# FangjinhuaWang/PatchmatchNet

Hardware: AMD Instinct MI355X
Metric: depth-maps/sec at 1600x1200 N=5 src views (higher is better)
Workload: dtype f32

## Files before the change

### include/pmn_hip.h

```cpp
#ifndef PMN_HIP_H
#define PMN_HIP_H

#include <stdint.h>

#ifdef __cplusplus
extern "C" {
#endif

#define PMN_ABI_VERSION 25
#define PMN_MLP_FLOATS 340
#define PMN_MAX_DEPTH 64
#define PMN_MAX_NEIGHBORS 17
#define PMN_MAX_FUSE_SRC 32
#define PMN_TSDF_MAX_VIEWS 16
#define PMN_TSDF_MARK_SPAN 8
#define PMN_RASTER_MAX_DIM 16384
#define PMN_RASTER_MAX_BOX 64
#define PMN_SPLAT_MAX_RADIUS 32

#define PMN_OK 0
#define PMN_ERR_ARG (-1)
#define PMN_ERR_SHAPE (-2)
#define PMN_ERR_LAUNCH (-3)

int pmn_abi_version(void);

const char *pmn_error_string(int code);

int pmn_nchw_to_nhwc(const float *in, float *out, int B, int C, int h, int w, void *stream);

int pmn_feature_weight(const float *ref_nhwc, const float *eval_offsets, const int *eval_table_host,
                       const float *mlp, int B, int C, int G, int K, int h, int w,
                       float *out_feature_weight, void *stream);

int pmn_init_hypotheses(const float *noise, const float *depth, int depth_shift, const float *depth_min,
                        const float *depth_max, int num_sample, float interval_scale, const float *propa_offsets,
                        const int *propa_table_host, int K, int B, int h, int w, float *depth_sample,
                        float *xnorm, void *stream);

int pmn_warp_correlate(const float *ref_nhwc, const float *src_nhwc, const float *rel_proj,
                       const float *depth_sample, const float *view_weights_in, int vw_shift,
                       const float *similarity_mlp, const float *pixelwise_mlp, int B, int N, int C,
                       int G, int D, int h, int w, int hs, int ws, float *cost_out, float *view_weights_out,
                       int *vw_argmax_out, float *similarity_out, void *stream);

int pmn_warp_correlate_views(const float *ref_nhwc, const void *src_view_table, const float *rel_proj,
                             const float *depth_sample, const float *view_weights_in, int vw_shift,
                             const float *similarity_mlp, const float *pixelwise_mlp, int B, int N, int C,
                             int G, int D, int h, int w, int hs, int ws, float *cost_out, float *view_weights_out,
                             int *vw_argmax_out, float *similarity_out, void *stream);

int pmn_aggregate_regress(const float *cost, const float *depth_sample, const float *xnorm,
                          const float *feature_weight, const float *eval_offsets, const int *eval_table_host,
                          int K, float interval_scale, int is_inverse, int B, int D, int h, int w,
                          float *score_out, float *depth_out, void *stream);

int pmn_confidence(const float *score, int B, int D, int h, int w, int H, int W, float *confidence_out,
                   int *depth_index_out, void *stream);

int pmn_conv2d(const float *in, const float *weights, const float *shift, const float *up, float *out, int N, int H,
               int W, int cin, int cout, int K, int stride, int pad, int dil, int relu, int in_nchw, int out_nchw,
               int up_h, int up_w, void *stream);

int pmn_fpn_tail(const float *x, const float *up, const float *w_in, const float *b_in, const float *w_out, float *out,
                 int N, int H, int W, int cin, int cmid, int cout, void *stream);

int pmn_conv2d_mfma(const float *in, const float *weights, const float *shift, float *out, float *out_b, int N, int H, int W,
                    int cin, int cout, int ca, int K, int stride, int pad, int dil, int relu, int planar, void *stream);


int pmn_conv2d_f16s(const float *in, const void *weights, const float *shift, float *out, int N, int H, int W, int cin, int cout,
                    int k, int stride, int relu, void *stream);

int pmn_conv2d_f16s_pair(const float *in, const void *weights_a, const float *shift_a, const void *weights_b, const float *shift_b,
                         float *out, int N, int H, int W, int channels, int relu, void *stream);

int pmn_offset_heads_f16s(const float *in, const void *weights, const float *shift, float *out_a, float *out_b, int N, int H, int W,
                          int cin, int cout, int ca, int dil, void *stream);

int pmn_fpn_level(const float *x, const float *u, const float *w, const float *b, float *out_a, float *out_b, int N, int H,
                  int W, int cin, int cout, int ca, void *stream);

int pmn_deconv3x3s2(const float *in, const float *weights, const float *shift, float *out, int N, int Hi, int Wi, int cin,
                    int cout, int relu, void *stream);

int pmn_refine_front(const float *img, const float *t2, const float *w0, const float *s0, const float *wd, const float *sd,
                     float *x16, int B, int H, int W, void *stream);
int pmn_refine_tail(const float *x16, const float *w3, const float *s3, const float *wr, const float *dnorm,
                    const float *depth_min, const float *depth_max, float *out, int B, int H, int W, void *stream);

int pmn_refine_fused(const float *img, const float *t2, const float *w0, const float *s0, const float *wd, const float *sd,
                     const void *w3a, const float *s3, const float *wr, const float *dnorm, const float *depth_min,
                     const float *depth_max, float *out, int B, int H, int W, void *stream);

int pmn_stage_projections(const float *intrinsics, const float *extrinsics, int B, int V, int nstages, float scale0,
                          float *rel, void *stream);

int pmn_stem(const float *img, const float *w0, const float *s0, const float *w1, const float *s1, float *out, int N, int H,
             int W, void *stream);

int pmn_stem_f16s(const float *img, const float *w0, const float *s0, const void *w1a, const float *s1, float *out, int N, int H,
                  int W, void *stream);

int pmn_stem_f16s_views(const float *const *img_table, int views, const float *w0, const float *s0, const void *w1a,
                        const float *s1, float *out, int B, int H, int W, void *stream);

int pmn_differentiable_warping(const float *src_nchw, const float *rel_proj, const float *depth, int B, int C,
                               int D, int h, int w, int hs, int ws, float *warped, void *stream);

int pmn_fuse_view(const float *maps, long long slot_stride, int ref_slot, const int *src_slots_host,
                  const int *src_hw_host, int n_src, const float *mats, int H, int W, float geo_pixel_thres, float geo_depth_thres, int geo_mask_thres,
                  float photo_thres, unsigned char *masks, float *xyz, double *depth_avg, int *geo_sum, void *stream);

int pmn_pack_points(const unsigned char *final_mask, const float *xyz, const void *image_hwc, int image_is_float, int H, int W,
                    unsigned char *records, long long capacity_points, long long *cursor, int *view_count, long long *scratch,
                    void *stream);

int pmn_pack_points_normals(const unsigned char *final_mask, const float *xyz, const float *normals_chw, const float *rotation,
                            int rotation_stride, const void *image_hwc, int image_is_float, int H, int W, unsigned char *records,
                            long long capacity_points, long long *cursor, int *view_count, long long *scratch, void *stream);

int pmn_depth_normals(const float *depth, int H, int W, const float *intrinsics_host, int radius, float rel_thres,
                      float *normals_out, void *stream);

int pmn_normalize_depth(const float *depth, const float *depth_min, const float *depth_max, int B, int n, float *out,
                        void *stream);

int pmn_check_f16_domain(const float *x, long long n, int *flag, void *stream);

int pmn_plan_create(void **plan_out);
int pmn_plan_begin(void *plan);
int pmn_plan_end(void *plan);
int pmn_plan_count(const void *plan);
const char *pmn_plan_kernel_name(const void *plan, int index);
int pmn_plan_launch(const void *plan, void *stream);
int pmn_plan_destroy(void *plan);

int pmn_view_scores(const double *cam_centers, const double *xyz, const long long *obs_ptr, const int *obs_pt,
                    const long long *trk_ptr, const int *trk_img, int N, int P, long long n_obs, long long n_trk,
                    double theta0, double sigma1, double sigma2, double *score, void *stream);

#define PMN_METRICS_MAX_STAGES 4
#define PMN_METRICS_MAX_ITERS 5
#define PMN_METRICS_MAX_THRESHOLDS 8
#define PMN_METRICS_COUNT 0
#define PMN_METRICS_ABS 4
#define PMN_METRICS_THR 8
#define PMN_METRICS_SL1 16
#define PMN_METRICS_ROW 36
#define PMN_METRICS_PIXELS_PER_BLOCK 4096
#define PMN_METRICS_MAX_BLOCKS 128
#define PMN_METRICS_BLOCKS(H, W)                                                                                                     \
    ((int)((((long long)(H) * (W) + PMN_METRICS_PIXELS_PER_BLOCK - 1) / PMN_METRICS_PIXELS_PER_BLOCK) > PMN_METRICS_MAX_BLOCKS        \
               ? PMN_METRICS_MAX_BLOCKS                                                                                               \
               : (((long long)(H) * (W) + PMN_METRICS_PIXELS_PER_BLOCK - 1) / PMN_METRICS_PIXELS_PER_BLOCK)))
#define PMN_METRICS_SCRATCH(B, H, W) ((long long)(B) * PMN_METRICS_BLOCKS(H, W) * PMN_METRICS_ROW)
int pmn_depth_metrics(const float *depth_gt, const float *depth_min, const float *const *maps_host, const int *iters_host,
                      const int *hw_host, int stages, const float *thresholds_host, int n_thresholds, int B, int H, int W,
                      double *scratch, long long scratch_doubles, double *rows, void *stream);

int pmn_nn_distance(const float *to_xyz, const long long *to_keys, long long n_to, const double *origin_host, double cell,
                    const int *dims_host, const float *query, const int *order, long long n_from, double max_dist, double *dist,
                    int *index, void *stream);
int pmn_reduce_round(const float *xyz, const long long *keys, long long n, const double *origin_host, double cell,
                     const int *dims_host, double dst, const int *rank, unsigned char *state, unsigned int *counter, void *stream);

int pmn_tsdf_integrate(float *tsdf, float *weight, float *rgb, float *cweight, const int *dims_host, const float *origin_host,
                       float voxel, float trunc, const float *maps, long long slot_stride, const int *slots_host,
                       const int *hw_host, const void *const *masks_host, const void *const *images_host, const float *cams_host,
                       int n_views, void *stream);
int pmn_mt_count(const float *tsdf, const float *weight, const int *dims_host, float min_weight, unsigned char *vertex_mask,
                 unsigned char *cell_triangles, void *stream);
int pmn_mt_emit(const float *tsdf, const float *weight, const float *rgb, const float *cweight, const int *dims_host,
                const float *origin_host, float voxel, float min_weight, const unsigned char *vertex_mask,
                const unsigned char *cell_triangles, const int *vertex_scan, const int *triangle_scan, float *vertices,
                unsigned char *colors, float *normals, int *faces, void *stream);

int pmn_tsdf_mark_blocks(unsigned char *flags, int *overflow, const int *dims_host, const float *origin_host, float voxel, float trunc,
                         const float *maps, long long slot_stride, const int *slots_host, const int *hw_host,
                         const void *const *masks_host, const float *inv_cams_host, int n_views, void *stream);
int pmn_tsdf_integrate_blocks(float *tsdf, float *weight, float *rgb, float *cweight, const int *blocks, int n_blocks,
                              const int *dims_host, const float *origin_host, float voxel, float trunc, const float *maps,
                              long long slot_stride, const int *slots_host, const int *hw_host, const void *const *masks_host,
                              const void *const *images_host, const float *cams_host, int n_views, void *stream);
int pmn_mt_count_blocks(const float *tsdf, const float *weight, const int *table, const int *blocks, int n_blocks,
                        const int *dims_host, float min_weight, unsigned char *vertex_mask, unsigned char *cell_triangles, void *stream);
int pmn_mt_emit_blocks(const float *tsdf, const float *weight, const float *rgb, const float *cweight, const int *table,
                       const int *blocks, int n_blocks, const int *dims_host, const float *origin_host, float voxel, float min_weight,
                       const unsigned char *vertex_mask, const unsigned char *cell_triangles, const int *vertex_scan,
                       const int *triangle_scan, float *vertices, unsigned char *colors, float *normals, int *faces, void *stream);

int pmn_raster_triangles(const float *vertices, int n_vertices, const int *faces, int n_faces, const float *cam_host, int h, int w,
                         long long max_box, unsigned long long *keys, int *counters, int *worklist, void *stream);
int pmn_splat_points(const float *points, long long n_points, const float *cam_host, int h, int w, float radius_px, float radius_world,
                     unsigned long long *keys, int *counters, void *stream);
int pmn_raster_resolve(const unsigned long long *keys, int h, int w, const float *cam_host, const float *vertices, long long n_vertices,
                       const int *faces, long long n_faces, const unsigned char *colors, const float *normals, int shade, float *depth,
                       int *index, unsigned char *rgb, float *normal, void *stream);

#define PMN_ICP_SUMS 17
#define PMN_ICP_LIMBS 5
#define PMN_ICP_BLOCK_POINTS 256
#define PMN_ICP_BLOCKS(n) (((long long)(n) + PMN_ICP_BLOCK_POINTS - 1) / PMN_ICP_BLOCK_POINTS)
#define PMN_ICP_SCRATCH(n) (PMN_ICP_BLOCKS(n) * PMN_ICP_SUMS * PMN_ICP_LIMBS)
#define PMN_VOXEL_LONG_RUN 256
#define PMN_VOXEL_MAX_CHANNELS 8
#define PMN_CROP_MAX_VERTICES 4096
int pmn_icp_accumulate(const float *to_xyz, const long long *to_keys, long long n_to, const double *origin_host, double cell,
                       const int *dims_host, const float *src, const int *order, long long n, const double *pose_host,
                       const double *centre_host, double max_dist, double *scratch, long long scratch_doubles, double *sums,
                       void *stream);
int pmn_voxel_mean(const float *xyz, const float *attr, int channels, long long n, const long long *starts, long long m, float *out_xyz,
                   float *out_attr, void *stream);
int pmn_crop_prism(const float *xyz, long long n, const double *polygon, int k, int axis, double axis_min, double axis_max,
                   const double *pose_host, unsigned char *mask, void *stream);

int pmn_mesh_components(const int *faces, int n_faces, int n_vertices, int *label, int *invalid, void *stream);
int pmn_mesh_face_samples(const float *vertices, int n_vertices, const int *faces, int n_faces, double density, unsigned long long seed,
                          int *counts, int *invalid, void *stream);
int pmn_mesh_sample(const float *vertices, int n_vertices, const int *faces, int n_faces, const unsigned char *colors,
                    const long long *sample_scan, long long n_samples, unsigned long long seed, float *points, int *face,
                    unsigned char *out_colors, void *stream);

#ifdef __cplusplus
}
#endif
#endif
```

### patchmatchnet_amd/_lib.py

```python
from __future__ import annotations

import ctypes
import os
import subprocess
from typing import Optional

_CSRC = os.path.join(os.path.dirname(os.path.abspath(__file__)), "csrc")
LIB_PATH = os.path.join(_CSRC, "libpmn_hip.so")
ABI_VERSION = 25
MLP_FLOATS = 340
MAX_DEPTH = 64
MAX_NEIGHBORS = 17
MAX_FUSE_SRC = 32
TSDF_MAX_VIEWS = 16
TSDF_MARK_SPAN = 8
RASTER_MAX_DIM = 16384
RASTER_MAX_BOX = 64
SPLAT_MAX_RADIUS = 32
ICP_SUMS = 17
ICP_LIMBS = 5
ICP_BLOCK_POINTS = 256
VOXEL_LONG_RUN = 256
VOXEL_MAX_CHANNELS = 8
CROP_MAX_VERTICES = 4096

_fp = ctypes.c_void_p
_ip = ctypes.c_void_p
_hp = ctypes.c_void_p
_i = ctypes.c_int
_f = ctypes.c_float
_s = ctypes.c_void_p

SIGNATURES = {
    "pmn_abi_version": [],
    "pmn_error_string": [_i],
    "pmn_nchw_to_nhwc": [_fp, _fp, _i, _i, _i, _i, _s],
    "pmn_feature_weight": [_fp, _fp, _hp, _fp, _i, _i, _i, _i, _i, _i, _fp, _s],
    "pmn_init_hypotheses": [_fp, _fp, _i, _fp, _fp, _i, _f, _fp, _hp, _i, _i, _i, _i, _fp, _fp, _s],
    "pmn_warp_correlate": [_fp, _fp, _fp, _fp, _fp, _i, _fp, _fp, _i, _i, _i, _i, _i, _i, _i, _i, _i, _fp, _fp, _ip,
                           _fp, _s],
    "pmn_warp_correlate_views": [_fp, _fp, _fp, _fp, _fp, _i, _fp, _fp, _i, _i, _i, _i, _i, _i, _i, _i, _i, _fp, _fp, _ip,
                                 _fp, _s],
    "pmn_aggregate_regress": [_fp, _fp, _fp, _fp, _fp, _hp, _i, _f, _i, _i, _i, _i, _i, _fp, _fp, _s],
    "pmn_confidence": [_fp, _i, _i, _i, _i, _i, _i, _fp, _ip, _s],
    "pmn_conv2d": [_fp, _fp, _fp, _fp, _fp] + [_i] * 14 + [_s],
    "pmn_fpn_tail": [_fp] * 6 + [_i] * 6 + [_s],
    "pmn_fpn_level": [_fp] * 6 + [_i] * 6 + [_s],
    "pmn_conv2d_f16s": [_fp] * 4 + [_i] * 8 + [_s],
    "pmn_offset_heads_f16s": [_fp] * 5 + [_i] * 7 + [_s],
    "pmn_conv2d_f16s_pair": [_fp] * 6 + [_i] * 5 + [_s],
    "pmn_refine_front": [_fp] * 7 + [_i] * 3 + [_s],
    "pmn_refine_tail": [_fp] * 8 + [_i] * 3 + [_s],
    "pmn_refine_fused": [_fp] * 13 + [_i] * 3 + [_s],
    "pmn_conv2d_mfma": [_fp] * 5 + [_i] * 12 + [_s],
    "pmn_deconv3x3s2": [_fp] * 4 + [_i] * 6 + [_s],
    "pmn_stage_projections": [_fp, _fp, _i, _i, _i, _f, _fp, _s],
    "pmn_stem": [_fp] * 6 + [_i] * 3 + [_s],
    "pmn_stem_f16s": [_fp] * 6 + [_i] * 3 + [_s],
    "pmn_stem_f16s_views": [_fp, _i] + [_fp] * 5 + [_i] * 3 + [_s],
    "pmn_differentiable_warping": [_fp, _fp, _fp, _i, _i, _i, _i, _i, _i, _i, _fp, _s],
    "pmn_fuse_view": [_fp, ctypes.c_longlong, _i, _hp, _hp, _i, _fp, _i, _i, _f, _f, _i, _f, _fp, _fp, _fp, _ip, _s],
    "pmn_pack_points": [_fp, _fp, _fp, _i, _i, _i, _fp, ctypes.c_longlong, _fp, _ip, _fp, _s],
    "pmn_pack_points_normals": [_fp, _fp, _fp, _fp, _i, _fp, _i, _i, _i, _fp, ctypes.c_longlong, _fp, _ip, _fp, _s],
    "pmn_depth_normals": [_fp, _i, _i, _hp, _i, _f, _fp, _s],
    "pmn_normalize_depth": [_fp, _fp, _fp, _i, _i, _fp, _s],
    "pmn_check_f16_domain": [_fp, ctypes.c_longlong, _ip, _s],
    "pmn_plan_create": [ctypes.POINTER(ctypes.c_void_p)],
    "pmn_plan_begin": [_hp],
    "pmn_plan_end": [_hp],
    "pmn_plan_count": [_hp],
    "pmn_plan_kernel_name": [_hp, _i],
    "pmn_plan_launch": [_hp, _s],
    "pmn_plan_destroy": [_hp],
    "pmn_view_scores": [_fp] * 6 + [_i, _i, ctypes.c_longlong, ctypes.c_longlong] + [ctypes.c_double] * 3 + [_fp, _s],
    "pmn_depth_metrics": [_fp, _fp, _hp, _hp, _hp, _i, _hp, _i, _i, _i, _i, _fp, ctypes.c_longlong, _fp, _s],
    "pmn_nn_distance": [_fp, _ip, ctypes.c_longlong, _hp, ctypes.c_double, _hp, _fp, _ip, ctypes.c_longlong, ctypes.c_double, _fp, _ip,
                        _s],
    "pmn_reduce_round": [_fp, _ip, ctypes.c_longlong, _hp, ctypes.c_double, _hp, ctypes.c_double, _ip, _ip, _ip, _s],
    "pmn_tsdf_integrate": [_fp] * 4 + [_hp, _hp, _f, _f, _fp, ctypes.c_longlong] + [_hp] * 5 + [_i, _s],
    "pmn_mt_count": [_fp, _fp, _hp, _f, _ip, _ip, _s],
    "pmn_mt_emit": [_fp] * 4 + [_hp, _hp, _f, _f] + [_ip] * 4 + [_fp, _ip, _fp, _ip, _s],
    "pmn_tsdf_mark_blocks": [_ip, _ip, _hp, _hp, _f, _f, _fp, ctypes.c_longlong] + [_hp] * 4 + [_i, _s],
    "pmn_tsdf_integrate_blocks": [_fp] * 4 + [_ip, _i, _hp, _hp, _f, _f, _fp, ctypes.c_longlong] + [_hp] * 5 + [_i, _s],
    "pmn_mt_count_blocks": [_fp, _fp, _ip, _ip, _i, _hp, _f, _ip, _ip, _s],
    "pmn_mt_emit_blocks": [_fp] * 4 + [_ip, _ip, _i, _hp, _hp, _f, _f] + [_ip] * 4 + [_fp, _ip, _fp, _ip, _s],
    "pmn_raster_triangles": [_fp, _i, _ip, _i, _hp, _i, _i, ctypes.c_longlong, _ip, _ip, _ip, _s],
    "pmn_splat_points": [_fp, ctypes.c_longlong, _hp, _i, _i, _f, _f, _ip, _ip, _s],
    "pmn_raster_resolve": [_ip, _i, _i, _hp, _fp, ctypes.c_longlong, _ip, ctypes.c_longlong, _ip, _fp, _i, _fp, _ip, _ip, _fp, _s],
    "pmn_icp_accumulate": [_fp, _ip, ctypes.c_longlong, _hp, ctypes.c_double, _hp, _fp, _ip, ctypes.c_longlong, _hp, _hp, ctypes.c_double,
                           _fp, ctypes.c_longlong, _fp, _s],
    "pmn_voxel_mean": [_fp, _fp, _i, ctypes.c_longlong, _ip, ctypes.c_longlong, _fp, _fp, _s],
    "pmn_crop_prism": [_fp, ctypes.c_longlong, _fp, _i, _i, ctypes.c_double, ctypes.c_double, _hp, _ip, _s],
    "pmn_mesh_components": [_ip, _i, _i, _ip, _ip, _s],
    "pmn_mesh_face_samples": [_fp, _i, _ip, _i, ctypes.c_double, ctypes.c_ulonglong, _ip, _ip, _s],
    "pmn_mesh_sample": [_fp, _i, _ip, _i, _ip, _ip, ctypes.c_longlong, ctypes.c_ulonglong, _fp, _ip, _ip, _s],
}

METRICS_MAX_STAGES = 4
METRICS_MAX_ITERS = 5
METRICS_MAX_THRESHOLDS = 8
METRICS_COUNT, METRICS_ABS, METRICS_THR, METRICS_SL1 = 0, 4, 8, 16
METRICS_ROW = 36
METRICS_PIXELS_PER_BLOCK = 4096
METRICS_MAX_BLOCKS = 128


def metrics_scratch(B: int, H: int, W: int) -> int:
    return B * min(METRICS_MAX_BLOCKS, -(-H * W // METRICS_PIXELS_PER_BLOCK)) * METRICS_ROW

def icp_scratch(n: int) -> int:
    return -(-n // ICP_BLOCK_POINTS) * ICP_SUMS * ICP_LIMBS


EXPERIMENTAL_SIGNATURES = {"pmn_set_tuning": [_i, _i],
                           "pmn_conv3x3_wino": [_fp] * 4 + [_i] * 5 + [_s],
                           "pmn_conv5x5s2_wino": [_fp] * 4 + [_i] * 6 + [_s]}
EXPERIMENTAL_LIB_PATH = os.path.join(_CSRC, "libpmn_hip_experimental.so")


def experimental() -> bool:
    return os.environ.get("PMN_EXPERIMENTAL", "") == "1"


_LIB: Optional[ctypes.CDLL] = None


class PmnError(RuntimeError):
    pass


def build(force: bool = False, verbose: bool = False) -> str:
    args = ["make", "-C", _CSRC, "-j4"] + (["-B"] if force else []) + (["EXPERIMENTAL=1"] if experimental() else [])
    if not verbose:
        args.insert(1, "-s")
    subprocess.check_call(args)
    return LIB_PATH


def lib() -> ctypes.CDLL:
    global _LIB
    if _LIB is None:
        path, sigs = LIB_PATH, SIGNATURES
        if experimental():
            path, sigs = EXPERIMENTAL_LIB_PATH, {**SIGNATURES, **EXPERIMENTAL_SIGNATURES}
        if not os.path.isfile(path):
            raise PmnError(f"{path} not found: build it with `python -c 'import __graft_entry__ as g; g.build()'` "
                           f"or `make -C patchmatchnet_amd/csrc` -- patchmatchnet_amd has no fallback path")
        L = (ctypes.CDLL if os.environ.get("PMN_CTYPES", "") == "cdll" else ctypes.PyDLL)(path)
        for name, argtypes in sigs.items():
            try:
                fn = getattr(L, name)
            except AttributeError as e:
                raise PmnError(f"libpmn_hip.so does not export {name}") from e
            fn.argtypes = argtypes
            fn.restype = ctypes.c_char_p if name in ("pmn_error_string", "pmn_plan_kernel_name") else ctypes.c_int
        if L.pmn_abi_version() != ABI_VERSION:
            raise PmnError(f"libpmn_hip.so ABI {L.pmn_abi_version()} != expected {ABI_VERSION}: rebuild")
        _LIB = L
    return _LIB


def check(code: int, what: str) -> None:
    if code != 0:
        raise PmnError(f"{what} failed: {lib().pmn_error_string(code).decode()} (code {code})")
```

### patchmatchnet_amd/csrc/plan.hip

```cpp
#include <hip/hip_runtime.h>

#include <cstring>
#include <mutex>
#include <new>
#include <vector>

#include "pmn_common.hpp"

struct PmnPlanEntry {
    const void* func;
    dim3 grid, block;
    size_t lds;
    int nargs;
    size_t first_arg;
};

struct PmnPlan {
    uint32_t magic;
    bool recording, poisoned, sealed;
    int device;
    std::vector<PmnPlanEntry> entries;
    std::vector<size_t> arg_offsets;
    std::vector<unsigned char> blob;
    std::vector<void*> argv;
};

static const uint32_t PMN_PLAN_MAGIC = 0x504d4e50u;

thread_local PmnPlan* pmn_tls_plan = nullptr;

static PmnPlan* as_plan(void* p) {
    PmnPlan* plan = static_cast<PmnPlan*>(p);
    return (plan && plan->magic == PMN_PLAN_MAGIC) ? plan : nullptr;
}

int pmn_plan_append(PmnPlan* plan, const void* func, dim3 grid, dim3 block, size_t lds, int nargs, void* const* args,
                    const size_t* sizes, const size_t* aligns) {
    if (!plan || plan->poisoned) return PMN_ERR_ARG;
    try {
        PmnPlanEntry e{func, grid, block, lds, nargs, plan->arg_offsets.size()};
        for (int i = 0; i < nargs; ++i) {
            const size_t al = aligns[i] ? aligns[i] : 1;
            size_t off = (plan->blob.size() + al - 1) / al * al;
            plan->blob.resize(off + sizes[i]);
            std::memcpy(plan->blob.data() + off, args[i], sizes[i]);
            plan->arg_offsets.push_back(off);
        }
        plan->entries.push_back(e);
    } catch (const std::bad_alloc&) {
        plan->poisoned = true;
        return PMN_ERR_ARG;
    }
    return PMN_OK;
}

extern "C" int pmn_plan_create(void** plan_out) {
    if (!plan_out) return PMN_ERR_ARG;
    PmnPlan* plan = new (std::nothrow) PmnPlan();
    if (!plan) return PMN_ERR_ARG;
    plan->magic = PMN_PLAN_MAGIC;
    plan->recording = plan->poisoned = plan->sealed = false;
    plan->device = -1;
    *plan_out = plan;
    return PMN_OK;
}

extern "C" int pmn_plan_begin(void* p) {
    PmnPlan* plan = as_plan(p);
    if (!plan || plan->sealed || plan->recording || pmn_tls_plan != nullptr) return PMN_ERR_ARG;
    if (hipGetDevice(&plan->device) != hipSuccess) plan->device = -1;
    plan->recording = true;
    pmn_tls_plan = plan;
    return PMN_OK;
}

extern "C" int pmn_plan_end(void* p) {
    PmnPlan* plan = as_plan(p);
    if (!plan || !plan->recording || pmn_tls_plan != plan) return PMN_ERR_ARG;
    pmn_tls_plan = nullptr;
    plan->recording = false;
    if (plan->poisoned) return PMN_ERR_ARG;
    try {
        plan->argv.resize(plan->arg_offsets.size());
    } catch (const std::bad_alloc&) {
        plan->poisoned = true;
        return PMN_ERR_ARG;
    }
    for (size_t i = 0; i < plan->arg_offsets.size(); ++i) plan->argv[i] = plan->blob.data() + plan->arg_offsets[i];
    plan->sealed = true;
    return PMN_OK;
}

extern "C" int pmn_plan_count(const void* p) {
    const PmnPlan* plan = as_plan(const_cast<void*>(p));
    if (!plan) return PMN_ERR_ARG;
    return (int)plan->entries.size();
}

extern "C" const char* pmn_plan_kernel_name(const void* p, int index) {
    const PmnPlan* plan = as_plan(const_cast<void*>(p));
    if (!plan || index < 0 || index >= (int)plan->entries.size()) return nullptr;
    return hipKernelNameRefByPtr(plan->entries[index].func, nullptr);
}

extern "C" int pmn_plan_launch(const void* p, void* stream) {
    const PmnPlan* plan = as_plan(const_cast<void*>(p));
    if (!plan || !plan->sealed) return PMN_ERR_ARG;
    if (pmn_tls_plan != nullptr) return PMN_ERR_ARG;
    hipStream_t st = (hipStream_t)stream;
    void* const* argv = plan->argv.data();
    for (const PmnPlanEntry& e : plan->entries) {
        if (hipLaunchKernel(e.func, e.grid, e.block, const_cast<void**>(argv + e.first_arg), e.lds, st) != hipSuccess) {
            (void)hipGetLastError();
            return PMN_ERR_LAUNCH;
        }
    }
    return PMN_OK;
}

extern "C" int pmn_plan_destroy(void* p) {
    PmnPlan* plan = as_plan(p);
    if (!plan) return PMN_ERR_ARG;
    if (pmn_tls_plan == plan) pmn_tls_plan = nullptr;
    plan->magic = 0;
    delete plan;
    return PMN_OK;
}
```

### patchmatchnet_amd/graph.py

```python
from __future__ import annotations

from typing import Dict, List, Optional, Sequence, Tuple

import torch

from ._lib import PmnError


class GraphedForward:

    def __init__(self, model, max_graphs: int = 8, inputs_in_place: bool = False) -> None:
        self.model, self.max_graphs, self.inputs_in_place = model, max_graphs, inputs_in_place
        self.cache: Dict[Tuple, Tuple] = {}
        self.replays = self.captures = self.evictions = 0

    @staticmethod
    def _alias_pattern(images: Sequence[torch.Tensor]) -> Tuple[int, ...]:
        first: Dict[int, int] = {}
        return tuple(first.setdefault(im.data_ptr(), i) for i, im in enumerate(images))

    @classmethod
    def _signature(cls, images: Sequence[torch.Tensor], intrinsics: torch.Tensor, features) -> Tuple:
        feat = None if features is None else tuple(tuple((s, tuple(t.shape)) for s, t in sorted(f.items())) for f in features)
        return (tuple(tuple(i.shape) for i in images), cls._alias_pattern(images), tuple(intrinsics.shape), feat,
                features is not None and cls._table_ok_cached(features))

    _TABLE_OK: Dict[Tuple, bool] = {}

    @classmethod
    def _table_ok_cached(cls, features) -> bool:
        try:
            key = tuple((s, tuple(t.shape), tuple(t.stride()), t.dtype, t.is_cuda) for f in features for s, t in sorted(f.items()))
        except (AttributeError, TypeError):
            return cls._table_ok(features)
        hit = cls._TABLE_OK.get(key)
        if hit is None:
            if len(cls._TABLE_OK) > 64:
                cls._TABLE_OK.clear()
            hit = cls._TABLE_OK[key] = cls._table_ok(features)
        return hit

    def _images_in_place(self, features) -> bool:
        feature = getattr(self.model, "feature", None)
        if not (self.inputs_in_place and features is None and getattr(self.model, "hip_feature_net", False)
                and feature is not None and feature.f16_split):
            return False
        return "conv1_f16s" in feature._packed()

    def _capture(self, images, intrinsics, extrinsics, depth_min, depth_max, features):
        dev = intrinsics.device
        pattern = self._alias_pattern(images)
        in_place = self._images_in_place(features)
        bufs = [torch.empty_like(im) if pattern[i] == i and not (in_place and i) else None for i, im in enumerate(images)]
        static = dict(images=[bufs[pattern[i]] for i in range(len(images))], intrinsics=torch.empty_like(intrinsics),
                      extrinsics=torch.empty_like(extrinsics), depth_min=torch.empty_like(depth_min),
                      depth_max=torch.empty_like(depth_max),
                      noise=torch.empty((images[0].shape[0], 48, images[0].shape[2] // 8, images[0].shape[3] // 8),
                                        dtype=torch.float32, device=dev),
                      features=None, features_nhwc=None)
        if in_place:
            from . import ops
            static["images"] = [bufs[0]] * len(images)
            static["image_bufs"] = bufs
            static["table_all"] = torch.zeros(len(images), dtype=torch.int64, device=dev)
            static["image_table"] = ops.SourceTable(static["table_all"], (len(images),) + tuple(images[0].shape))
            static["table_host"] = []
        if features is not None and self._table_ok(features):
            from . import ops
            B = images[0].shape[0]
            stages = sorted(features[0])
            ref = {s: torch.empty((B,) + tuple(features[0][s].shape[2:]) + (features[0][s].shape[1],), dtype=torch.float32, device=dev)
                   for s in stages}
            static["ref_nhwc"] = ref
            n_src = len(features) - 1
            static["table_all"] = torch.zeros(len(stages) * n_src, dtype=torch.int64, device=dev)
            static["tables"] = {s: ops.SourceTable(static["table_all"][i * n_src:(i + 1) * n_src],
                                                   (n_src, B) + tuple(features[1][s].shape[2:]) + (features[1][s].shape[1],))
                                for i, s in enumerate(stages)}
            static["features"] = [{s: ref[s].permute(0, 3, 1, 2) for s in stages} for _ in range(len(features))]
            static["table_host"] = []
        elif features is not None:
            B = images[0].shape[0]
            stages = sorted(features[0])
            nhwc = {s: torch.empty((len(features) * B,) + tuple(features[0][s].shape[2:]) + (features[0][s].shape[1],),
                                   dtype=torch.float32, device=dev) for s in stages}
            static["features_nhwc"] = nhwc
            static["features"] = [{s: nhwc[s][v * B:(v + 1) * B].permute(0, 3, 1, 2) for s in stages} for v in range(len(features))]
        self._fill(static, images, intrinsics, extrinsics, depth_min, depth_max, features)

        def run():
            return self.model(list(static["images"]), static["intrinsics"], static["extrinsics"], static["depth_min"],
                              static["depth_max"], features=static["features"], features_nhwc=static["features_nhwc"],
                              noise=static["noise"], source_tables=static.get("tables"), ref_nhwc_maps=static.get("ref_nhwc"),
                              image_table=static.get("image_table"))

        rng = torch.cuda.get_rng_state(dev)
        self._draw(static)
        try:
            handle, out = self._record(run, dev)
        finally:
            torch.cuda.set_rng_state(rng, dev)
        return handle, static, out

    def _record(self, run, dev):
        side = torch.cuda.Stream(dev)
        side.wait_stream(torch.cuda.current_stream(dev))
        with torch.cuda.stream(side):
            run()
        torch.cuda.current_stream(dev).wait_stream(side)
        graph = torch.cuda.CUDAGraph()
        with torch.cuda.graph(graph, capture_error_mode="thread_local"):
            depth, confidence, _ = run()
        return graph, (depth, confidence)

    def _replay(self, handle, dev) -> None:
        handle.replay()

    @staticmethod
    def _table_ok(features) -> bool:
        try:
            for s in features[0]:
                shapes = {tuple(f[s].shape) for f in features}
                if len(shapes) != 1:
                    return False
                for f in features:
                    t = f[s]
                    if not (t.is_cuda and t.dtype == torch.float32 and t.permute(0, 2, 3, 1).is_contiguous()):
                        return False
            return len(features) >= 2
        except (AttributeError, KeyError, TypeError):
            return False

    @staticmethod
    def _draw(static) -> None:
        torch.rand(size=tuple(static["noise"].shape), out=static["noise"])

    @staticmethod
    def _stage_addresses(static, addrs) -> None:
        ring = static["table_host"]
        k = static["turn"] = (static.get("turn", -1) + 1) % 8
        if k >= len(ring):
            host = torch.empty(static["table_all"].numel(), dtype=torch.int64).pin_memory()
            ring.append([host, host.numpy(), None])
        host, host_np, ev = ring[k]
        if ev is not None:
            ev.synchronize()
        host_np[:] = addrs
        static["table_all"].copy_(host, non_blocking=True)
        ev = torch.cuda.Event()
        ev.record(torch.cuda.current_stream(static["intrinsics"].device))
        ring[k][2] = ev

    @classmethod
    def _fill(cls, static, images, intrinsics, extrinsics, depth_min, depth_max, features) -> None:
        if "image_table" in static:
            from . import ops
            bufs, addrs, held = static["image_bufs"], [], []
            for i, im in enumerate(images):
                if i == 0 or im.device != static["intrinsics"].device or not ops.SourceTable.image_in_place(im):
                    if bufs[i] is None:
                        bufs[i] = torch.empty(tuple(images[0].shape), dtype=torch.float32, device=static["intrinsics"].device)
                    if bufs[i].data_ptr() != im.data_ptr():
                        bufs[i].copy_(im, non_blocking=True)
                    addrs.append(bufs[i].data_ptr())
                else:
                    im.record_stream(torch.cuda.current_stream(im.device))
                    held.append(im)
                    addrs.append(im.data_ptr())
            static["held_images"] = held
            cls._stage_addresses(static, addrs)
        else:
            done = set()
            for dst, src in zip(static["images"], images):
                if dst.data_ptr() not in done and dst.data_ptr() != src.data_ptr():
                    dst.copy_(src, non_blocking=True)
                done.add(dst.data_ptr())
        static["intrinsics"].copy_(intrinsics, non_blocking=True)
        static["extrinsics"].copy_(extrinsics, non_blocking=True)
        static["depth_min"].copy_(depth_min, non_blocking=True)
        static["depth_max"].copy_(depth_max, non_blocking=True)
        if features is not None and "tables" in static:
            for s, t in features[0].items():
                static["features"][0][s].copy_(t, non_blocking=True)
            cls._stage_addresses(static, [features[1 + v][s].data_ptr() for s in sorted(static["tables"]) for v in range(len(features) - 1)])
        elif features is not None:
            for dst, src in zip(static["features"], features):
                for s, t in src.items():
                    dst[s].copy_(t, non_blocking=True)

    def __call__(self, images: List[torch.Tensor], intrinsics: torch.Tensor, extrinsics: torch.Tensor,
                 depth_min: torch.Tensor, depth_max: torch.Tensor, features: Optional[List[Dict[int, torch.Tensor]]] = None):
        if not intrinsics.is_cuda:
            raise PmnError("GraphedForward replays HIP graphs: the inputs must be on a ROCm device")
        h, w = images[0].shape[-2:]
        if h % 8 or w % 8 or any(tuple(i.shape) != tuple(images[0].shape) for i in images):
            depth, confidence, _ = self.model(images, intrinsics, extrinsics, depth_min, depth_max, features=features)
            return depth, confidence
        key = self._signature(images, intrinsics, features)
        entry = self.cache.pop(key, None)
        if entry is None:
            if len(self.cache) >= self.max_graphs:
                self.cache.pop(next(iter(self.cache)))
                self.evictions += 1
            entry = self._capture(images, intrinsics, extrinsics, depth_min, depth_max, features)
            self.captures += 1
        self.cache[key] = entry
        graph, static, out = entry
        self._fill(static, images, intrinsics, extrinsics, depth_min, depth_max, features)
        self._draw(static)
        self._replay(graph, intrinsics.device)
        self.replays += 1
        return out


class _LibraryLaunchesOnly(torch.utils._python_dispatch.TorchDispatchMode):

    _ALLOC = ("aten.empty.", "aten.empty_strided.", "aten.empty_like.", "aten.new_empty.", "aten.new_empty_strided.", "aten.detach.",
              "aten.alias.", "aten.lift_fresh.", "aten._unsafe_view.", "aten.reshape.", "aten.view.", "aten.sym_size.",
              "aten.sym_stride.", "aten.sym_numel.", "aten.sym_storage_offset.", "aten.is_contiguous.", "aten.size.", "aten.stride.",
              "aten.numel.", "aten.dim.", "aten.is_pinned.", "prim.device.", "prim.dtype.", "prim.layout.", "aten.record_stream.")

    def __torch_dispatch__(self, func, types, args=(), kwargs=None):
        if not (getattr(func, "is_view", False) or (str(func) + ".").startswith(self._ALLOC)):
            raise PmnError(f"PlannedForward: the forward dispatched {func} while it was being recorded -- an operator outside "
                           "libpmn_hip.so cannot be part of a launch plan (it would run once, on uninitialised data, and never "
                           "again); this input signature has to run eagerly or through a path that only calls the library")
        return func(*args, **(kwargs or {}))


class PlannedForward(GraphedForward):

    def __init__(self, model, max_graphs: int = 8, inputs_in_place: bool = False) -> None:
        super().__init__(model, max_graphs=max_graphs, inputs_in_place=inputs_in_place)

    def _record(self, run, dev):
        import ctypes
        from . import _lib
        L = _lib.lib()
        run()
        with torch.cuda.device(dev):
            pool = torch.cuda.MemPool()
            plan = ctypes.c_void_p()
            _lib.check(L.pmn_plan_create(ctypes.byref(plan)), "pmn_plan_create")
            handle = _Plan(plan, pool)
            with torch.cuda.use_mem_pool(pool, device=dev):
                _lib.check(L.pmn_plan_begin(plan), "pmn_plan_begin")
                try:
                    with _LibraryLaunchesOnly():
                        depth, confidence, _ = run()
                finally:
                    rc = L.pmn_plan_end(plan)
                _lib.check(rc, "pmn_plan_end")
        handle.count = L.pmn_plan_count(plan)
        if handle.count <= 0:
            raise PmnError("PlannedForward: the recording pass recorded no launch")
        return handle, (depth, confidence)

    def _replay(self, handle, dev) -> None:
        from . import _lib
        with torch.cuda.device(dev):
            _lib.check(_lib.lib().pmn_plan_launch(handle.plan, torch.cuda.current_stream(dev).cuda_stream), "pmn_plan_launch")


class PlannedValidationForward(PlannedForward):

    def __init__(self, model, thresholds: Sequence[float], max_graphs: int = 8) -> None:
        super().__init__(model, max_graphs=max_graphs)
        self.thresholds = tuple(float(t) for t in thresholds)
        self._truth: Dict[Tuple, Tuple[torch.Tensor, torch.Tensor]] = {}
        self._current: Optional[Tuple[torch.Tensor, torch.Tensor]] = None

    def __call__(self, images: List[torch.Tensor], intrinsics: torch.Tensor, extrinsics: torch.Tensor,
                 depth_min: torch.Tensor, depth_max: torch.Tensor, depth_gt: torch.Tensor):
        h, w = images[0].shape[-2:]
        if h % 8 or w % 8:
            raise PmnError(f"PlannedValidationForward: {h}x{w} images -- the stage maps are down-samplings of the ground truth only "
                           "when height and width are multiples of 8")
        key = (tuple(depth_gt.shape), depth_gt.device)
        bufs = self._truth.get(key)
        if bufs is None:
            bufs = self._truth[key] = (torch.empty(tuple(depth_gt.shape), dtype=torch.float32, device=depth_gt.device),
                                       torch.empty(tuple(depth_min.shape), dtype=torch.float32, device=depth_gt.device))
        bufs[0].copy_(depth_gt, non_blocking=True)
        bufs[1].copy_(depth_min, non_blocking=True)
        self._current = bufs
        return super().__call__(images, intrinsics, extrinsics, depth_min, depth_max)

    def _record(self, run, dev):
        from . import ops
        depth_gt, depth_min = self._current
        held = {}

        def run_scored():
            depth, confidence, maps = run()
            held["rows"] = ops.depth_metrics(depth_gt, depth_min, maps, self.thresholds)
            return depth, confidence, maps

        handle, (depth, confidence) = super()._record(run_scored, dev)
        return handle, (depth, confidence, held["rows"])


class _Plan:

    def __init__(self, plan, pool) -> None:
        self.plan, self.pool, self.count = plan, pool, 0

    def kernel_names(self) -> List[str]:
        from . import _lib
        L = _lib.lib()
        return [(L.pmn_plan_kernel_name(self.plan, i) or b"?").decode() for i in range(self.count)]

    def __del__(self):
        try:
            from . import _lib
            if self.plan:
                _lib.lib().pmn_plan_destroy(self.plan)
                self.plan = None
        except Exception:
            pass
```

### patchmatchnet_amd/net.py

```python
from __future__ import annotations

from typing import Dict, List, Optional, Tuple

import warnings

import numpy as np
import torch
import torch.nn as nn
import torch.nn.functional as F

from . import _lib, ops, params
from ._lib import PmnError
from .module import ConvBnReLU
from .patchmatch import PatchMatch


class FeatureNet(nn.Module):

    def __init__(self) -> None:
        super().__init__()
        spec = [(3, 8, 3, 1, 1), (8, 8, 3, 1, 1), (8, 16, 5, 2, 2), (16, 16, 3, 1, 1), (16, 16, 3, 1, 1),
                (16, 32, 5, 2, 2), (32, 32, 3, 1, 1), (32, 32, 3, 1, 1), (32, 64, 5, 2, 2), (64, 64, 3, 1, 1),
                (64, 64, 3, 1, 1)]
        for i, (cin, cout, k, s, p) in enumerate(spec):
            setattr(self, f"conv{i}", ConvBnReLU(cin, cout, k, s, p))
        self.output1 = nn.Conv2d(64, 64, 1, bias=False)
        self.inner1 = nn.Conv2d(32, 64, 1, bias=True)
        self.inner2 = nn.Conv2d(16, 64, 1, bias=True)
        self.output2 = nn.Conv2d(64, 32, 1, bias=False)
        self.output3 = nn.Conv2d(64, 16, 1, bias=False)
        self.f16_split = True
        self.f16_domain_error: Optional[str] = None
        self.fold_fpn = True
        self.fuse_conv34 = True
        self.fpn8_valu = False
        self.layer_hook = None

    _SPEC = [(3, 1, 1), (3, 1, 1), (5, 2, 2), (3, 1, 1), (3, 1, 1), (5, 2, 2), (3, 1, 1), (3, 1, 1), (5, 2, 2), (3, 1, 1),
             (3, 1, 1)]

    def _packed(self):
        srcs = [p for p in self.parameters()] + [b for b in self.buffers() if b.dtype.is_floating_point]
        key = params.versions(srcs)
        if getattr(self, "_pack_key", None) != key:
            dev = self.output1.weight.device
            pk = {}
            f16_ok, self.f16_domain_error = True, None
            for i in range(11):
                m = getattr(self, f"conv{i}")
                w, s = params.pack_conv(m.conv.weight, bn=(m.bn.weight, m.bn.bias, m.bn.running_mean, m.bn.running_var),
                                        eps=m.bn.eps)
                pk[f"conv{i}"] = (torch.from_numpy(w).to(dev), torch.from_numpy(s).to(dev))
                cv = m.conv
                if (cv.kernel_size[0], cv.stride[0], cv.in_channels, cv.out_channels) in ops.F16S_SHAPES and f16_ok:
                    try:
                        w, s = params.pack_conv_f16s(cv.weight, bn=(m.bn.weight, m.bn.bias, m.bn.running_mean, m.bn.running_var),
                                                     eps=m.bn.eps)
                        pk[f"conv{i}_f16s"] = (torch.from_numpy(w).to(dev), torch.from_numpy(s).to(dev))
                    except params.F16DomainError as e:
                        f16_ok, self.f16_domain_error = False, f"conv{i}: {e}"
            m1 = self.conv1
            try:
                w, s = params.pack_stem_conv1_f16s(m1.conv.weight, bn=(m1.bn.weight, m1.bn.bias, m1.bn.running_mean, m1.bn.running_var),
                                                  eps=m1.bn.eps)
                pk["conv1_f16s"] = (torch.from_numpy(w).to(dev), torch.from_numpy(s).to(dev))
            except params.F16DomainError as e:
                f16_ok, self.f16_domain_error = False, f"conv1: {e}"
            if not f16_ok:
                for k in [k for k in pk if k.endswith("_f16s")]:
                    del pk[k]
                warnings.warn("FeatureNet: " + self.f16_domain_error + " -- using the fp32 kernels (pmn_stem / pmn_conv2d) instead of "
                              "the fp16-split matrix-core kernels", RuntimeWarning, stacklevel=2)
            for name in ("output1", "inner1", "inner2", "output2", "output3"):
                m = getattr(self, name)
                w, s = params.pack_conv(m.weight, bias=m.bias)
                pk[name] = (torch.from_numpy(w).to(dev), torch.from_numpy(s).to(dev))
            fold = params.fold_fpn(self.output1.weight, self.inner1.weight, self.inner1.bias, self.inner2.weight,
                                   self.inner2.bias, self.output2.weight, self.output3.weight)
            for lvl, (w, b) in fold.items():
                pk[f"fpn{lvl}"] = (torch.from_numpy(w).to(dev), torch.from_numpy(b).to(dev))
            w8 = torch.from_numpy(np.ascontiguousarray(fold[8][0].T))[:, :, None, None]
            w, s = params.pack_conv_mfma(w8, bias=torch.from_numpy(fold[8][1]))
            pk["fpn8_mfma"] = (torch.from_numpy(w).to(dev), torch.from_numpy(s).to(dev))
            self._pack, self._pack_key = pk, key
        return self._pack

    def forward_hip(self, x, image_table: Optional["ops.SourceTable"] = None) -> Dict[int, torch.Tensor]:
        pk = self._packed()
        imgs = list(x) if isinstance(x, (list, tuple)) else [x]
        B, _, H, W = imgs[0].shape
        in_place = image_table is not None
        if in_place and not (self.f16_split and "conv1_f16s" in pk):
            raise PmnError("image_table: only the fp16-split stem (FeatureNet.f16_split, weights inside its domain) reads images in place")
        if in_place:
            t = ops.stem_f16s_views(image_table, *pk["conv0"], *pk["conv1_f16s"])
        else:
            t = torch.empty((B * len(imgs), H, W, 8), dtype=torch.float32, device=imgs[0].device)
        for i, im in enumerate(() if in_place else imgs):
            if self.f16_split and "conv1_f16s" in pk:
                ops.stem_f16s(im.contiguous(), *pk["conv0"], *pk["conv1_f16s"], out=t[i * B:(i + 1) * B])
            else:
                ops.stem(im.contiguous(), *pk["conv0"], *pk["conv1"], out=t[i * B:(i + 1) * B])
        feats = {}
        for i, (k, s, p) in enumerate(self._SPEC):
            if i < 2:
                continue
            if i == 4 and self.f16_split and self.fuse_conv34 and "conv3_f16s" in pk and "conv4_f16s" in pk:
                continue
            if i == 3 and self.f16_split and self.fuse_conv34 and "conv3_f16s" in pk and "conv4_f16s" in pk:
                t = ops.conv2d_f16s_pair(t, *pk["conv3_f16s"], *pk["conv4_f16s"], relu=True)
                feats[4] = t
            elif self.f16_split and f"conv{i}_f16s" in pk:
                t = ops.conv2d_f16s(t, *pk[f"conv{i}_f16s"], k, s, relu=True)
            elif self.layer_hook is not None and (hooked := self.layer_hook(i, t)) is not None:
                t = hooked
            else:
                w, sh = pk[f"conv{i}"]
                t = ops.conv2d(t, w, sh, getattr(self, f"conv{i}").conv.out_channels, k, s, p, relu=True)
            if i in (4, 7, 10):
                feats[i] = t
        half, quarter, eighth = feats[4], feats[7], feats[10]
        if self.fold_fpn:
            if self.fpn8_valu:
                f3, u8 = ops.fpn_level(eighth, None, *pk["fpn8"], ca=64)
            else:
                f3, u8 = ops.pointwise_split_mfma(eighth, *pk["fpn8_mfma"], cout=112, ca=64)
            f2, u4 = ops.fpn_level(quarter, u8, *pk["fpn4"], ca=32)
            f1, _ = ops.fpn_level(half, u4, *pk["fpn2"], ca=16)
            return {3: f3, 2: f2, 1: f1}
        out = {3: ops.conv2d(eighth, *pk["output1"], 64, 1)}
        top = ops.conv2d(quarter, *pk["inner1"], 64, 1, up=eighth)
        out[2] = ops.conv2d(top, *pk["output2"], 32, 1)
        out[1] = ops.fpn_tail(half, top, pk["inner2"][0], pk["inner2"][1], pk["output3"][0])
        return out

    def forward(self, x: torch.Tensor) -> Dict[int, torch.Tensor]:
        half = self.conv4(self.conv3(self.conv2(self.conv1(self.conv0(x)))))
        quarter = self.conv7(self.conv6(self.conv5(half)))
        eighth = self.conv10(self.conv9(self.conv8(quarter)))
        out: Dict[int, torch.Tensor] = {3: self.output1(eighth)}
        top = F.interpolate(eighth, scale_factor=2.0, mode="bilinear", align_corners=False) + self.inner1(quarter)
        out[2] = self.output2(top)
        top = F.interpolate(top, scale_factor=2.0, mode="bilinear", align_corners=False) + self.inner2(half)
        out[1] = self.output3(top)
        return out


class Refinement(nn.Module):

    def __init__(self) -> None:
        super().__init__()
        self.conv0 = ConvBnReLU(in_channels=3, out_channels=8)
        self.conv1 = ConvBnReLU(in_channels=1, out_channels=8)
        self.conv2 = ConvBnReLU(in_channels=8, out_channels=8)
        self.deconv = nn.ConvTranspose2d(8, 8, kernel_size=3, padding=1, output_padding=1, stride=2, bias=False)
        self.bn = nn.BatchNorm2d(8)
        self.conv3 = ConvBnReLU(in_channels=16, out_channels=8)
        self.res = nn.Conv2d(8, 1, kernel_size=3, padding=1, bias=False)
        self.f16_split = True
        self.f16_domain_error: Optional[str] = None
        self.research = dict(layers=False)

    def _packed(self):
        srcs = [p for p in self.parameters()] + [b for b in self.buffers() if b.dtype.is_floating_point]
        key = params.versions(srcs)
        if getattr(self, "_pack_key", None) != key:
            dev = self.res.weight.device

            def bn_of(m):
                return (m.weight, m.bias, m.running_mean, m.running_var)

            pk = {}
            for name in ("conv0", "conv1", "conv2", "conv3"):
                m = getattr(self, name)
                w, s = params.pack_conv(m.conv.weight, bn=bn_of(m.bn), eps=m.bn.eps)
                pk[name] = (torch.from_numpy(w).to(dev), torch.from_numpy(s).to(dev))
            w, s = params.pack_deconv(self.deconv.weight, bn=bn_of(self.bn), eps=self.bn.eps)
            pk["deconv"] = (torch.from_numpy(w).to(dev), torch.from_numpy(s).to(dev))
            w, s = params.pack_conv(self.res.weight)
            pk["res"] = (torch.from_numpy(w).to(dev), torch.from_numpy(s).to(dev))
            pk["tail"] = tuple(torch.from_numpy(a).to(dev) for a in params.pack_refine_tail(
                self.conv3.conv.weight, bn_of(self.conv3.bn), self.res.weight, eps=self.conv3.bn.eps))
            self.f16_domain_error = None
            try:
                w, s = params.pack_refine_conv3_f16s(self.conv3.conv.weight, bn_of(self.conv3.bn), eps=self.conv3.bn.eps)
                pk["conv3_f16s"] = (torch.from_numpy(w).to(dev), torch.from_numpy(s).to(dev))
            except params.F16DomainError as e:
                self.f16_domain_error = f"conv3: {e}"
                warnings.warn("Refinement: " + self.f16_domain_error + " -- using the fp32 kernels (pmn_refine_front / pmn_refine_tail)",
                              RuntimeWarning, stacklevel=2)
            self._pack, self._pack_key = pk, key
        return self._pack

    def forward_hip(self, img: torch.Tensor, depth_0: torch.Tensor, depth_min: torch.Tensor, depth_max: torch.Tensor
                    ) -> torch.Tensor:
        pk = self._packed()
        b = depth_min.size()[0]
        if not self.research["layers"]:
            d = ops.normalize_depth(depth_0, depth_min, depth_max)
        else:
            lo = depth_min.view(b, 1, 1, 1)
            span = (depth_max - depth_min).view(b, 1, 1, 1)
            d = ((depth_0 - lo) / span).contiguous()
        t = ops.conv2d(d, *pk["conv1"], 8, 3, 1, 1, relu=True, in_nchw=True)
        t = ops.conv2d(t, *pk["conv2"], 8, 3, 1, 1, relu=True)
        if not self.research["layers"]:
            if self.f16_split and "conv3_f16s" in pk:
                return ops.refine_fused(img.contiguous(), t, *pk["conv0"], *pk["deconv"], *pk["conv3_f16s"], pk["tail"][2], d,
                                        depth_min.float().contiguous(), depth_max.float().contiguous())
            x16 = ops.refine_front(img.contiguous(), t, *pk["conv0"], *pk["deconv"])
            return ops.refine_tail(x16, *pk["tail"], d, depth_min.float().contiguous(), depth_max.float().contiguous())
        img_feat = ops.conv2d(img.contiguous(), *pk["conv0"], 8, 3, 1, 1, relu=True, in_nchw=True)
        up = ops.deconv3x3s2(t, *pk["deconv"], relu=True)
        t = ops.conv2d(torch.cat((up, img_feat), dim=3), *pk["conv3"], 8, 3, 1, 1, relu=True)
        res = ops.conv2d(t, *pk["res"], 1, 3, 1, 1, out_nchw=True)
        d = F.interpolate(d, scale_factor=2.0, mode="nearest") + res
        return d * span + lo

    def forward(self, img: torch.Tensor, depth_0: torch.Tensor, depth_min: torch.Tensor, depth_max: torch.Tensor
                ) -> torch.Tensor:
        b = depth_min.size()[0]
        lo = depth_min.view(b, 1, 1, 1)
        span = (depth_max - depth_min).view(b, 1, 1, 1)
        d = (depth_0 - lo) / span
        img_feat = self.conv0(img)
        up = F.relu(self.bn(self.deconv(self.conv2(self.conv1(d)))), inplace=True)
        res = self.res(self.conv3(torch.cat((up, img_feat), dim=1)))
        d = F.interpolate(d, scale_factor=2.0, mode="nearest") + res
        return d * span + lo


class PatchmatchNet(nn.Module):

    def __init__(self, patchmatch_interval_scale: List[float], propagation_range: List[int],
                 patchmatch_iteration: List[int], patchmatch_num_sample: List[int], propagate_neighbors: List[int],
                 evaluate_neighbors: List[int]) -> None:
        super().__init__()
        self.stages = 4
        self.feature = FeatureNet()
        self.patchmatch_num_sample = patchmatch_num_sample
        num_features = [16, 32, 64]
        self.propagate_neighbors = propagate_neighbors
        self.evaluate_neighbors = evaluate_neighbors
        self.G = [4, 8, 8]
        for i in range(self.stages - 1):
            setattr(self, f"patchmatch_{i + 1}", PatchMatch(
                propagation_out_range=propagation_range[i], patchmatch_iteration=patchmatch_iteration[i],
                patchmatch_num_sample=patchmatch_num_sample[i], patchmatch_interval_scale=patchmatch_interval_scale[i],
                num_feature=num_features[i], G=self.G[i], propagate_neighbors=self.propagate_neighbors[i],
                evaluate_neighbors=evaluate_neighbors[i], stage=i + 1))
        self.upsample_net = Refinement()
        self.batch_feature_extraction = True
        self.hip_feature_net = True
        self.hip_projections = True

    def load_state_dict(self, state_dict, strict: bool = True, **kw):
        if any(k.startswith("module.") for k in state_dict):
            state_dict = {(k[len("module."):] if k.startswith("module.") else k): v for k, v in state_dict.items()}
        return super().load_state_dict(state_dict, strict=strict, **kw)

    @staticmethod
    def scripted_module_config(archive) -> Dict[str, list]:
        stages = [getattr(archive, f"patchmatch_{i}") for i in (1, 2, 3)]
        return dict(patchmatch_interval_scale=[float(s.patchmatch_interval_scale) for s in stages],
                    propagation_range=[int(s.dilation) for s in stages],
                    patchmatch_iteration=[int(s.patchmatch_iteration) for s in stages],
                    patchmatch_num_sample=[int(x) for x in archive.patchmatch_num_sample],
                    propagate_neighbors=[int(s.propagate_neighbors) for s in stages],
                    evaluate_neighbors=[int(s.evaluate_neighbors) for s in stages])

    @classmethod
    def from_scripted_module(cls, path: str) -> "PatchmatchNet":
        archive = torch.jit.load(path, map_location="cpu")
        model = cls(**cls.scripted_module_config(archive))
        model.load_state_dict({k: v.detach().clone() for k, v in archive.state_dict().items()}, strict=True)
        return model

    def extract_features(self, images: List[torch.Tensor], stacked: Optional[dict] = None,
                         image_table: Optional["ops.SourceTable"] = None) -> List[Dict[int, torch.Tensor]]:
        same = all(im.shape == images[0].shape for im in images)
        B = images[0].shape[0]
        if image_table is not None and not (self.hip_feature_net and same and images[0].is_cuda and self.feature.f16_split):
            raise PmnError("image_table needs the HIP FeatureNet (f16_split) and same-size images on a ROCm device")
        if self.hip_feature_net and same and images[0].is_cuda:
            f = self.feature.forward_hip(images, image_table=image_table)
            if stacked is not None:
                stacked.update({("nhwc", s): t for s, t in f.items()})
            return [{s: t[i * B:(i + 1) * B].permute(0, 3, 1, 2) for s, t in f.items()} for i in range(len(images))]
        if self.hip_feature_net and images[0].is_cuda:
            outs = [self.feature.forward_hip(im) for im in images]
            return [{s: t.permute(0, 3, 1, 2) for s, t in f.items()} for f in outs]
        if self.batch_feature_extraction and same and len(images) > 1:
            f = self.feature(torch.cat(images, dim=0))
            if stacked is not None:
                stacked.update(f)
            return [{s: t[i * B:(i + 1) * B] for s, t in f.items()} for i in range(len(images))]
        return [self.feature(im) for im in images]

    def forward(self, images: List[torch.Tensor], intrinsics: torch.Tensor, extrinsics: torch.Tensor,
                depth_min: torch.Tensor, depth_max: torch.Tensor, noise: Optional[torch.Tensor] = None,
                features: Optional[List[Dict[int, torch.Tensor]]] = None, debug: Optional[dict] = None,
                features_nhwc: Optional[Dict[int, torch.Tensor]] = None, source_tables: Optional[Dict[int, "ops.SourceTable"]] = None,
                ref_nhwc_maps: Optional[Dict[int, torch.Tensor]] = None, image_table: Optional["ops.SourceTable"] = None
                ) -> Tuple[torch.Tensor, torch.Tensor, Dict[int, List[torch.Tensor]]]:
        assert len(images) == intrinsics.size()[1], "Different number of images and intrinsic matrices"
        assert len(images) == extrinsics.size()[1], "Different number of images and extrinsic matrices"
        if self.training:
            raise PmnError("patchmatchnet_amd.PatchmatchNet is inference-only: call .eval() (the HIP kernels have no "
                           "backward pass)")
        images, intrinsics, orig_height, orig_width = adjust_image_dims(images, intrinsics)
        ref_image = images[0]
        _, _, ref_height, ref_width = ref_image.size()

        stacked: Dict[int, torch.Tensor] = {}
        if features is None:
            features = self.extract_features(images, stacked, image_table)
        elif features_nhwc is not None:
            stacked.update({("nhwc", st): t for st, t in features_nhwc.items()})
        ref_feature, src_features = features[0], features[1:]
        batch = ref_image.shape[0]

        depth_min = depth_min.float()
        depth_max = depth_max.float()
        device = intrinsics.device
        depth = torch.empty(0, device=device)
        score = torch.empty(0, device=device)
        view_weights = torch.empty(0, device=device)
        depth_patchmatch: Dict[int, List[torch.Tensor]] = {}

        scale = 0.125
        depth_shift, vw_shift = 0, 0
        rel_all = ops.stage_projections(intrinsics, extrinsics, self.stages - 1, scale) if self.hip_projections else None
        for stage in range(self.stages - 1, 0, -1):
            if rel_all is None:
                intrinsics_l = intrinsics.clone()
                intrinsics_l[:, :, :2] *= scale
                proj = extrinsics.clone()
                proj[:, :, :3, :4] = torch.matmul(intrinsics_l, extrinsics[:, :, :3, :4])
                proj_l = torch.unbind(proj, 1)
                ref_proj, src_proj = proj_l[0], proj_l[1:]
            else:
                ref_proj, src_proj = extrinsics[:, 0], [extrinsics[:, i] for i in range(1, extrinsics.shape[1])]
            scale *= 2.0

            dbg = [] if debug is not None else None
            pm: PatchMatch = getattr(self, f"patchmatch_{stage}")
            ref_nhwc = src_nhwc = None
            if ("nhwc", stage) in stacked:
                allv = stacked[("nhwc", stage)]
            elif stage in stacked:
                allv = ops.nchw_to_nhwc(stacked[stage].contiguous())
            else:
                allv = None
            if source_tables is not None:
                ref_nhwc, src_nhwc = ref_nhwc_maps[stage], source_tables[stage]
            elif allv is not None:
                ref_nhwc = allv[:batch]
                src_nhwc = allv[batch:].view(len(src_features), batch, *allv.shape[1:])
            depths, score, view_weights = pm(
                ref_feature=ref_feature[stage], src_features=[f[stage] for f in src_features], ref_proj=ref_proj,
                src_projs=list(src_proj), depth_min=depth_min, depth_max=depth_max, depth=depth,
                view_weights=view_weights, depth_shift=depth_shift, vw_shift=vw_shift,
                noise=noise if stage == self.stages - 1 else None, debug=dbg, ref_nhwc=ref_nhwc, src_nhwc=src_nhwc,
                rel_proj=None if rel_all is None else rel_all[self.stages - 1 - stage])
            if debug is not None:
                debug[stage] = dbg
            depth_patchmatch[stage] = depths
            depth = depths[-1].detach()
            if stage > 1:
                depth_shift = 1
                vw_shift = vw_shift + 1 if view_weights.shape[-1] != depths[-1].shape[-1] else 1

        if self.hip_feature_net and ref_image.is_cuda:
            depth = self.upsample_net.forward_hip(ref_image, depth, depth_min, depth_max)
        else:
            depth = self.upsample_net(ref_image, depth, depth_min, depth_max)
        if ref_width != orig_width or ref_height != orig_height:
            depth = F.interpolate(depth, size=[orig_height, orig_width], mode="bilinear", align_corners=False)
        depth_patchmatch[0] = [depth]

        confidence, _ = ops.confidence(score.contiguous(), orig_height, orig_width)
        return depth, confidence, depth_patchmatch


def adjust_image_dims(images: List[torch.Tensor], intrinsics: torch.Tensor
                      ) -> Tuple[List[torch.Tensor], torch.Tensor, int, int]:
    _, _, ref_height, ref_width = images[0].size()
    for i in range(len(images)):
        _, _, height, width = images[i].size()
        new_height = int(round(height / 8)) * 8
        new_width = int(round(width / 8)) * 8
        if new_width != width or new_height != height:
            intrinsics[:, i, 0] *= new_width / width
            intrinsics[:, i, 1] *= new_height / height
            images[i] = F.interpolate(images[i], size=[new_height, new_width], mode="bilinear", align_corners=False)
    return images, intrinsics, ref_height, ref_width
```

### patchmatchnet_amd/ops.py

```python
from __future__ import annotations

import ctypes
from typing import List, Optional, Sequence, Tuple

import numpy as np
import torch

from . import _lib
from ._lib import PmnError, check


_TIMING = None
_TIMING_ON = True


def enable_kernel_timing() -> None:
    global _TIMING, _TIMING_ON
    _TIMING, _TIMING_ON = [], True


def pause_kernel_timing(paused: bool) -> None:
    global _TIMING_ON
    _TIMING_ON = not paused


def disable_kernel_timing():
    global _TIMING
    rec, _TIMING = _TIMING, None
    if not rec:
        return []
    torch.cuda.synchronize()
    return [(s.elapsed_time(e), nbytes, tag) for s, e, nbytes, tag in rec]


TUNE_WINDOW_BYTES, TUNE_FLAGS, TUNE_WINDOW_BYTES_PIXELWISE, TUNE_ABLATE = 0, 1, 2, 3
TUNE_LANE_WINDOW_BYTES, TUNE_LANE_ABLATE, TUNE_LANE_WAVES_PER_SIMD = 4, 5, 6
TUNE_TILE_WINDOW_BYTES = 10
FLAG_WINDOWED, FLAG_NO_ROTATION, FLAG_STREAM_PIXELWISE, FLAG_STREAM_VIEWS, FLAG_WIN_V1, FLAG_TILE, FLAG_MFMA = 1, 2, 4, 8, 16, 32, 64
DEFAULT_FLAGS = 0


def set_tuning(key: int, value: int) -> None:
    if not _lib.experimental():
        raise PmnError("pmn_set_tuning exists only in libpmn_hip_experimental.so: build with `make -C patchmatchnet_amd/csrc "
                       "EXPERIMENTAL=1` and run with PMN_EXPERIMENTAL=1")
    check(_lib.lib().pmn_set_tuning(int(key), int(value)), "pmn_set_tuning")


import os as _os

F16_DOMAIN_CHECK = _os.environ.get("PMN_CHECK_F16_DOMAIN", "") == "1"
_F16_FLAGS = {}


def _f16_domain_probe(*tensors: Optional[torch.Tensor]) -> None:
    if not F16_DOMAIN_CHECK:
        return
    for t in tensors:
        if t is None or not t.is_cuda or t.numel() == 0:
            continue
        flag = _F16_FLAGS.get(t.device)
        if flag is None:
            flag = _F16_FLAGS[t.device] = torch.zeros(1, dtype=torch.int32, device=t.device)
        with torch.cuda.device(t.device):
            check(_lib.lib().pmn_check_f16_domain(t.data_ptr(), t.numel(), flag.data_ptr(), _stream(t)), "pmn_check_f16_domain")


def f16_domain_check(reset: bool = True) -> None:
    bad = [str(d) for d, f in _F16_FLAGS.items() if int(f.item()) != 0]
    if reset:
        for f in _F16_FLAGS.values():
            f.zero_()
    if bad:
        raise PmnError("an activation outside the fp16-split kernels' domain (|x| >= 65504 or not finite) reached pmn_*_f16s on " +
                       ", ".join(bad) + ": the outputs contain inf / NaN where an fp32 convolution is finite -- set f16_split = False on "
                       "FeatureNet / Refinement / PatchMatch for this checkpoint or input range (include/pmn_hip.h)")


def _dev(t: torch.Tensor, name: str) -> torch.Tensor:
    if not isinstance(t, torch.Tensor):
        raise PmnError(f"{name}: expected a torch.Tensor")
    if not t.is_cuda:
        raise PmnError(f"{name}: tensor is on {t.device}; patchmatchnet_amd runs only on a ROCm GPU (no CPU fallback)")
    if t.dtype != torch.float32:
        raise PmnError(f"{name}: expected float32, got {t.dtype}")
    if not t.is_contiguous():
        raise PmnError(f"{name}: tensor must be contiguous")
    return t


def _dlast(t: torch.Tensor, name: str) -> torch.Tensor:
    if not isinstance(t, torch.Tensor) or not t.is_cuda or t.dtype != torch.float32:
        raise PmnError(f"{name}: expected a float32 tensor on a ROCm GPU (no CPU fallback)")
    if t.permute(0, 2, 3, 1).is_contiguous():
        return t
    return t.permute(0, 2, 3, 1).contiguous().permute(0, 3, 1, 2)


def _dev_as(t: torch.Tensor, name: str, dtype: torch.dtype) -> torch.Tensor:
    if not isinstance(t, torch.Tensor) or not t.is_cuda:
        raise PmnError(f"{name}: expected a tensor on a ROCm GPU (no CPU fallback)")
    if t.dtype != dtype or not t.is_contiguous():
        raise PmnError(f"{name}: expected a contiguous {dtype} tensor")
    return t


def _ptr(t: Optional[torch.Tensor]) -> Optional[int]:
    return None if t is None else t.data_ptr()


def _stream(t: torch.Tensor) -> int:
    return torch.cuda.current_stream(t.device).cuda_stream


def _host_f32(a: np.ndarray, n: int, name: str):
    a = np.ascontiguousarray(a, np.float32)
    if a.size != n:
        raise PmnError(f"{name}: expected {n} floats, got {a.size}")
    return a, a.ctypes.data_as(ctypes.c_void_p)


def _host_i32(a: np.ndarray, n: int, name: str):
    a = np.ascontiguousarray(a, np.int32)
    if a.size != n:
        raise PmnError(f"{name}: expected {n} ints, got {a.size}")
    return a, a.ctypes.data_as(ctypes.c_void_p)


def nchw_to_nhwc(x: torch.Tensor, out: Optional[torch.Tensor] = None) -> torch.Tensor:
    if out is None and isinstance(x, torch.Tensor) and x.is_cuda and x.dtype == torch.float32 and not x.is_contiguous():
        v = x.permute(0, 2, 3, 1)
        if v.is_contiguous():
            return v
        x = x.contiguous()
    _dev(x, "x")
    B, C, h, w = x.shape
    if out is None:
        out = torch.empty((B, h, w, C), dtype=torch.float32, device=x.device)
    else:
        _dev(out, "out")
        if tuple(out.shape) != (B, h, w, C):
            raise PmnError("nchw_to_nhwc: bad output shape")
    with torch.cuda.device(x.device):
        check(_lib.lib().pmn_nchw_to_nhwc(x.data_ptr(), out.data_ptr(), B, C, h, w, _stream(x)), "pmn_nchw_to_nhwc")
    return out


def stack_sources_nhwc(src_features: Sequence[torch.Tensor]) -> torch.Tensor:
    buf, sizes = stack_sources_padded(src_features)
    if any(sz != sizes[0] for sz in sizes):
        raise PmnError("all source feature maps of one stage must share a shape (stack_sources_padded handles mixed sizes)")
    return buf


def stack_sources_padded(src_features: Sequence[torch.Tensor]):
    if len(src_features) == 0:
        raise PmnError("at least one source view is required")
    B, C = src_features[0].shape[:2]
    sizes = [(int(f.shape[2]), int(f.shape[3])) for f in src_features]
    if any(tuple(f.shape[:2]) != (B, C) for f in src_features):
        raise PmnError("source feature maps of one stage must share batch size and channels")
    hs, ws = max(h for h, _ in sizes), max(w for _, w in sizes)
    mixed = any(sz != (hs, ws) for sz in sizes)
    alloc = torch.zeros if mixed else torch.empty
    buf = alloc((len(src_features), B, hs, ws, C), dtype=torch.float32, device=src_features[0].device)
    for i, f in enumerate(src_features):
        v = f.permute(0, 2, 3, 1)
        if sizes[i] != (hs, ws):
            _dev(f.contiguous(), "src_feature")
            buf[i][:, :sizes[i][0], :sizes[i][1], :].copy_(v)
        elif f.is_cuda and f.dtype == torch.float32 and v.is_contiguous():
            buf[i].copy_(v)
        else:
            nchw_to_nhwc(f.contiguous(), buf[i])
    return buf, sizes


def rescale_projection_rows(rel_proj: torch.Tensor, sizes, padded_hw) -> torch.Tensor:
    HS, WS = padded_hw
    if all(sz == (HS, WS) for sz in sizes):
        return rel_proj
    out = rel_proj.clone()
    for v, (h_v, w_v) in enumerate(sizes):
        if (h_v, w_v) != (HS, WS):
            out[:, v, 0, :] *= (w_v - 1) / (WS - 1)
            out[:, v, 1, :] *= (h_v - 1) / (HS - 1)
    return out.contiguous()


def _mlp_dev(t: torch.Tensor, name: str) -> torch.Tensor:
    _dev(t, name)
    if t.numel() != _lib.MLP_FLOATS:
        raise PmnError(f"{name}: expected a packed MLP block of {_lib.MLP_FLOATS} floats")
    return t


def feature_weight(ref_nhwc: torch.Tensor, eval_offsets: torch.Tensor, table: np.ndarray, mlp: torch.Tensor,
                   G: int) -> torch.Tensor:
    _dev(ref_nhwc, "ref_nhwc")
    _dev(eval_offsets, "eval_offsets")
    B, h, w, C = ref_nhwc.shape
    K = eval_offsets.shape[1] // 2
    if tuple(eval_offsets.shape) != (B, 2 * K, h, w):
        raise PmnError("feature_weight: eval_offsets must be [B,2K,h,w]")
    tab, tab_p = _host_i32(table, 2 * K, "table")
    _mlp_dev(mlp, "mlp")
    out = torch.empty((B, K, h, w), dtype=torch.float32, device=ref_nhwc.device)
    with torch.cuda.device(ref_nhwc.device):
        check(_lib.lib().pmn_feature_weight(ref_nhwc.data_ptr(), eval_offsets.data_ptr(), tab_p, mlp.data_ptr(), B, C, G,
                                            K, h, w,
                                            out.data_ptr(), _stream(out)), "pmn_feature_weight")
    return out


def init_hypotheses(noise: Optional[torch.Tensor], depth: Optional[torch.Tensor], depth_shift: int,
                    depth_min: torch.Tensor, depth_max: torch.Tensor, num_sample: int, interval_scale: float,
                    propa_offsets: Optional[torch.Tensor], table: Optional[np.ndarray], h: int, w: int
                    ) -> Tuple[torch.Tensor, torch.Tensor]:
    _dev(depth_min, "depth_min")
    _dev(depth_max, "depth_max")
    B = depth_min.shape[0]
    dev = depth_min.device
    if noise is not None:
        _dev(noise, "noise")
        if tuple(noise.shape) != (B, 48, h, w):
            raise PmnError("init_hypotheses: noise must be [B,48,h,w]")
        D0 = 48
    else:
        if depth is None:
            raise PmnError("init_hypotheses: need noise or depth")
        _dev(depth, "depth")
        if tuple(depth.shape) != (B, 1, h >> depth_shift, w >> depth_shift):
            raise PmnError(f"init_hypotheses: depth must be [B,1,{h >> depth_shift},{w >> depth_shift}], "
                           f"got {tuple(depth.shape)}")
        D0 = num_sample
    K = 0
    tab_p = None
    tab = None
    if propa_offsets is not None:
        _dev(propa_offsets, "propa_offsets")
        K = propa_offsets.shape[1] // 2
        if tuple(propa_offsets.shape) != (B, 2 * K, h, w):
            raise PmnError("init_hypotheses: propa_offsets must be [B,2K,h,w]")
        tab, tab_p = _host_i32(table, 2 * K, "table")
    D = D0 + K
    ds = torch.empty((B, D, h, w), dtype=torch.float32, device=dev)
    xn = torch.empty((B, h, w, D), dtype=torch.float32, device=dev).permute(0, 3, 1, 2)
    with torch.cuda.device(dev):
        check(_lib.lib().pmn_init_hypotheses(_ptr(noise), _ptr(depth) if noise is None else None, depth_shift,
                                             depth_min.data_ptr(), depth_max.data_ptr(), num_sample,
                                             float(interval_scale), _ptr(propa_offsets), tab_p, K, B, h, w,
                                             ds.data_ptr(), xn.data_ptr(), _stream(ds)), "pmn_init_hypotheses")
    del tab
    return ds, xn


class SourceTable:

    def __init__(self, table: torch.Tensor, shape) -> None:
        if table.dtype != torch.int64 or not table.is_cuda or table.numel() != int(shape[0]):
            raise PmnError("SourceTable: int64 device tensor with one address per source view")
        self.table, self.shape, self.device = table, tuple(int(x) for x in shape), table.device

    @staticmethod
    def image_in_place(im: torch.Tensor) -> bool:
        return bool(im.is_cuda and im.dtype == torch.float32 and im.is_contiguous() and im.data_ptr() % 16 == 0)

    @staticmethod
    def addresses(maps) -> list:
        out = []
        for m in maps:
            if not (m.is_cuda and m.dtype == torch.float32 and m.is_contiguous()):
                raise PmnError("SourceTable: dense float32 channels-last device maps")
            out.append(m.data_ptr())
        return out


def warp_correlate(ref_nhwc: torch.Tensor, src_nhwc, rel_proj: torch.Tensor, depth_sample: torch.Tensor,
                   view_weights: Optional[torch.Tensor], vw_shift: int, similarity_mlp: torch.Tensor,
                   pixelwise_mlp: Optional[torch.Tensor], G: int, want_similarity: bool = False,
                   want_argmax: bool = False):
    _dev(ref_nhwc, "ref_nhwc")
    table = src_nhwc if isinstance(src_nhwc, SourceTable) else None
    if table is None:
        _dev(src_nhwc, "src_nhwc")
    _dev(rel_proj, "rel_proj")
    _dev(depth_sample, "depth_sample")
    B, h, w, C = ref_nhwc.shape
    N, Bs, hs, ws, Cs = src_nhwc.shape
    D = depth_sample.shape[1]
    if Bs != B or Cs != C or tuple(depth_sample.shape) != (B, D, h, w) or tuple(rel_proj.shape) != (B, N, 4, 4):
        raise PmnError("warp_correlate: inconsistent shapes")
    dev = ref_nhwc.device
    sim_p = _mlp_dev(similarity_mlp, "similarity_mlp").data_ptr()
    pix_p, vw_out, argmax = None, None, None
    if view_weights is not None:
        _dev(view_weights, "view_weights")
        if tuple(view_weights.shape) != (B, N, h >> vw_shift, w >> vw_shift):
            raise PmnError("Patchmatch Evaluation: Different number of images and view weights")
    else:
        if pixelwise_mlp is None:
            raise PmnError("warp_correlate: pixelwise_mlp required when view_weights is None")
        pix_p = _mlp_dev(pixelwise_mlp, "pixelwise_mlp").data_ptr()
        vw_out = torch.empty((B, N, h, w), dtype=torch.float32, device=dev)
        if want_argmax:
            argmax = torch.empty((B, N, h, w), dtype=torch.int32, device=dev)
    cost = torch.empty((B, h, w, D), dtype=torch.float32, device=dev).permute(0, 3, 1, 2)
    sim = torch.empty((B, G, D, h, w), dtype=torch.float32, device=dev) if want_similarity else None
    with torch.cuda.device(dev):
        if _TIMING is not None and _TIMING_ON:
            ev0, ev1 = torch.cuda.Event(enable_timing=True), torch.cuda.Event(enable_timing=True)
            ev0.record()
        fn = _lib.lib().pmn_warp_correlate if table is None else _lib.lib().pmn_warp_correlate_views
        check(fn(ref_nhwc.data_ptr(), (src_nhwc if table is None else table.table).data_ptr(), rel_proj.data_ptr(),
                 depth_sample.data_ptr(), _ptr(view_weights), vw_shift, sim_p, pix_p, B, N, C,
                 G, D, h, w, hs, ws, cost.data_ptr(), _ptr(vw_out), _ptr(argmax), _ptr(sim),
                 _stream(cost)), "pmn_warp_correlate")
        if _TIMING is not None and _TIMING_ON:
            ev1.record()
            _TIMING.append((ev0, ev1, 4 * B * h * w * ((1 + N) * C + D + N + G * D),
                            f"C{C}_D{D}_{h}x{w}_N{N}_{'vw' if view_weights is not None else 'pixelwise'}"))
    return cost, (view_weights if view_weights is not None else vw_out), argmax, sim


def aggregate_regress(cost: torch.Tensor, depth_sample: torch.Tensor, xnorm: torch.Tensor, feature_weight_: torch.Tensor,
                      eval_offsets: torch.Tensor, table: np.ndarray, interval_scale: float, is_inverse: bool
                      ) -> Tuple[torch.Tensor, torch.Tensor]:
    for n, t in (("depth_sample", depth_sample), ("feature_weight", feature_weight_), ("eval_offsets", eval_offsets)):
        _dev(t, n)
    cost, xnorm = _dlast(cost, "cost"), _dlast(xnorm, "xnorm")
    B, D, h, w = cost.shape
    K = feature_weight_.shape[1]
    if tuple(depth_sample.shape) != (B, D, h, w) or tuple(xnorm.shape) != (B, D, h, w) or \
            tuple(feature_weight_.shape) != (B, K, h, w) or tuple(eval_offsets.shape) != (B, 2 * K, h, w):
        raise PmnError("aggregate_regress: inconsistent shapes")
    tab, tab_p = _host_i32(table, 2 * K, "table")
    score = torch.empty((B, D, h, w), dtype=torch.float32, device=cost.device)
    depth = torch.empty((B, h, w), dtype=torch.float32, device=cost.device)
    with torch.cuda.device(cost.device):
        check(_lib.lib().pmn_aggregate_regress(cost.data_ptr(), depth_sample.data_ptr(), xnorm.data_ptr(),
                                               feature_weight_.data_ptr(), eval_offsets.data_ptr(), tab_p, K,
                                               float(interval_scale), 1 if is_inverse else 0, B, D, h, w,
                                               score.data_ptr(), depth.data_ptr(), _stream(cost)),
              "pmn_aggregate_regress")
    return score, depth


def confidence(score: torch.Tensor, H: int, W: int, want_index: bool = False):
    _dev(score, "score")
    B, D, h, w = score.shape
    conf = torch.empty((B, H, W), dtype=torch.float32, device=score.device)
    idx = torch.empty((B, h, w), dtype=torch.int32, device=score.device) if want_index else None
    with torch.cuda.device(score.device):
        check(_lib.lib().pmn_confidence(score.data_ptr(), B, D, h, w, H, W, conf.data_ptr(), _ptr(idx), _stream(score)),
              "pmn_confidence")
    return conf, idx


def relative_projection(src_projs: Sequence[torch.Tensor], ref_proj: torch.Tensor) -> torch.Tensor:
    inv = torch.inverse(ref_proj)
    return torch.matmul(torch.stack(list(src_projs), dim=1), inv.unsqueeze(1)).contiguous()


def differentiable_warping(src_fea: torch.Tensor, src_proj: torch.Tensor, ref_proj: torch.Tensor,
                           depth_samples: torch.Tensor) -> torch.Tensor:
    src_fea = _dev(src_fea.contiguous(), "src_fea")
    depth_samples = _dev(depth_samples.contiguous(), "depth_samples")
    B, C, hs, ws = src_fea.shape
    _, D, h, w = depth_samples.shape
    proj = torch.matmul(src_proj, torch.inverse(ref_proj)).contiguous()
    _dev(proj, "proj")
    out = torch.empty((B, C, D, h, w), dtype=torch.float32, device=src_fea.device)
    with torch.cuda.device(src_fea.device):
        check(_lib.lib().pmn_differentiable_warping(src_fea.data_ptr(), proj.data_ptr(), depth_samples.data_ptr(), B, C,
                                                    D, h, w, hs, ws, out.data_ptr(), _stream(out)),
              "pmn_differentiable_warping")
    return out


def stage_projections(intrinsics: torch.Tensor, extrinsics: torch.Tensor, nstages: int = 3, scale0: float = 0.125
                      ) -> torch.Tensor:
    intrinsics = _dev(intrinsics.float().contiguous(), "intrinsics")
    extrinsics = _dev(extrinsics.float().contiguous(), "extrinsics")
    B, V = intrinsics.shape[:2]
    rel = torch.empty((nstages, B, V - 1, 4, 4), dtype=torch.float32, device=intrinsics.device)
    with torch.cuda.device(rel.device):
        check(_lib.lib().pmn_stage_projections(intrinsics.data_ptr(), extrinsics.data_ptr(), B, V, nstages, float(scale0),
                                               rel.data_ptr(), _stream(rel)), "pmn_stage_projections")
    return rel


def normalize_depth(depth: torch.Tensor, depth_min: torch.Tensor, depth_max: torch.Tensor) -> torch.Tensor:
    depth = _dev(depth.contiguous(), "depth")
    lo, hi = _dev(depth_min.float().contiguous(), "depth_min"), _dev(depth_max.float().contiguous(), "depth_max")
    B = depth.shape[0]
    if lo.numel() != B or hi.numel() != B:
        raise PmnError("normalize_depth: depth_min / depth_max must hold one value per batch element")
    out = torch.empty_like(depth)
    with torch.cuda.device(depth.device):
        check(_lib.lib().pmn_normalize_depth(depth.data_ptr(), lo.data_ptr(), hi.data_ptr(), B, depth.numel() // B, out.data_ptr(),
                                             _stream(out)), "pmn_normalize_depth")
    return out


def conv2d(x: torch.Tensor, weights: torch.Tensor, shift: torch.Tensor, cout: int, K: int, stride: int = 1, pad: int = 0,
           dil: int = 1, relu: bool = False, up: Optional[torch.Tensor] = None, in_nchw: bool = False,
           out_nchw: bool = False, out: Optional[torch.Tensor] = None) -> torch.Tensor:
    _dev(x, "x")
    _dev(weights, "weights")
    _dev(shift, "shift")
    if in_nchw:
        N, cin, H, W = x.shape
    else:
        N, H, W, cin = x.shape
    if tuple(weights.shape[:3]) != (K, K, cin) or shift.numel() != weights.shape[3]:
        raise PmnError("conv2d: packed weights do not match the input")
    Ho = (H + 2 * pad - dil * (K - 1) - 1) // stride + 1
    Wo = (W + 2 * pad - dil * (K - 1) - 1) // stride + 1
    shape = (N, cout, Ho, Wo) if out_nchw else (N, Ho, Wo, cout)
    if out is None:
        out = torch.empty(shape, dtype=torch.float32, device=x.device)
    else:
        _dev(out, "out")
        if tuple(out.shape) != shape:
            raise PmnError("conv2d: bad `out` shape")
    up_h = up_w = 0
    if up is not None:
        _dev(up, "up")
        if tuple(up.shape) != (N, Ho // 2, Wo // 2, cout) or Ho % 2 or Wo % 2:
            raise PmnError("conv2d: `up` must be [N,Ho/2,Wo/2,cout]")
        up_h, up_w = up.shape[1], up.shape[2]
    with torch.cuda.device(x.device):
        check(_lib.lib().pmn_conv2d(x.data_ptr(), weights.data_ptr(), shift.data_ptr(), _ptr(up), out.data_ptr(), N, H, W,
                                    cin, cout, K, stride, pad, dil, 1 if relu else 0, 1 if in_nchw else 0,
                                    1 if out_nchw else 0, up_h, up_w, _stream(x)), "pmn_conv2d")
    return out


def fpn_tail(x: torch.Tensor, up: torch.Tensor, w_in: torch.Tensor, b_in: torch.Tensor, w_out: torch.Tensor) -> torch.Tensor:
    for n_, t_ in (("x", x), ("up", up), ("w_in", w_in), ("b_in", b_in), ("w_out", w_out)):
        _dev(t_, n_)
    N, H, W, cin = x.shape
    cmid, cout = up.shape[3], w_out.shape[3]
    if tuple(up.shape) != (N, H // 2, W // 2, cmid) or tuple(w_in.shape) != (1, 1, cin, cmid) or \
            tuple(w_out.shape) != (1, 1, cmid, cout):
        raise PmnError("fpn_tail: inconsistent shapes")
    out = torch.empty((N, H, W, cout), dtype=torch.float32, device=x.device)
    with torch.cuda.device(x.device):
        check(_lib.lib().pmn_fpn_tail(x.data_ptr(), up.data_ptr(), w_in.data_ptr(), b_in.data_ptr(), w_out.data_ptr(),
                                      out.data_ptr(), N, H, W, cin, cmid, cout, _stream(x)), "pmn_fpn_tail")
    return out


MFMA_CONV_SHAPES = {(64, 64, 3, 1), (32, 32, 3, 1), (32, 64, 5, 2), (16, 32, 5, 2)}
MFMA_HEAD_SHAPES = {(64, 2), (32, 4), (16, 6)}


def conv2d_mfma(x: torch.Tensor, weights: torch.Tensor, shift: torch.Tensor, K: int, stride: int = 1, pad: int = 0,
                relu: bool = True) -> torch.Tensor:
    for n_, t_ in (("x", x), ("weights", weights), ("shift", shift)):
        _dev(t_, n_)
    N, H, W, cin = x.shape
    cout = shift.shape[0]
    if tuple(weights.shape) != (K * K, cin // 8, cout // 32, 64, 4):
        raise PmnError("conv2d_mfma: weights are not in pack_conv_mfma layout for this input")
    Ho, Wo = (H + 2 * pad - K) // stride + 1, (W + 2 * pad - K) // stride + 1
    out = torch.empty((N, Ho, Wo, cout), dtype=torch.float32, device=x.device)
    with torch.cuda.device(x.device):
        check(_lib.lib().pmn_conv2d_mfma(x.data_ptr(), weights.data_ptr(), shift.data_ptr(), out.data_ptr(), None, N, H, W,
                                         cin, cout, cout, K, stride, pad, 1, 1 if relu else 0, 0, _stream(x)),
              "pmn_conv2d_mfma")
    return out


def conv3x3_wino(x: torch.Tensor, weights: torch.Tensor, shift: torch.Tensor, relu: bool = True) -> torch.Tensor:
    if not _lib.experimental():
        raise PmnError("conv3x3_wino: research build only (make -C patchmatchnet_amd/csrc EXPERIMENTAL=1, PMN_EXPERIMENTAL=1)")
    for n_, t_ in (("x", x), ("weights", weights), ("shift", shift)):
        _dev(t_, n_)
    N, H, W, C = x.shape
    if tuple(weights.shape) != (C // 16, 16, C // 16, 64, 4) or tuple(shift.shape) != (C,):
        raise PmnError("conv3x3_wino: weights are not in pack_conv_wino layout for this input")
    out = torch.empty((N, H, W, C), dtype=torch.float32, device=x.device)
    with torch.cuda.device(x.device):
        check(_lib.lib().pmn_conv3x3_wino(x.data_ptr(), weights.data_ptr(), shift.data_ptr(), out.data_ptr(), N, H, W, C,
                                          1 if relu else 0, _stream(x)), "pmn_conv3x3_wino")
    return out


def conv5x5s2_wino(x: torch.Tensor, weights: torch.Tensor, shift: torch.Tensor, relu: bool = True) -> torch.Tensor:
    if not _lib.experimental():
        raise PmnError("conv5x5s2_wino: research build only (make -C patchmatchnet_amd/csrc EXPERIMENTAL=1, PMN_EXPERIMENTAL=1)")
    for n_, t_ in (("x", x), ("weights", weights), ("shift", shift)):
        _dev(t_, n_)
    N, H, W, cin = x.shape
    cout = shift.shape[0]
    if tuple(weights.shape) != (cin // 8, 49, cout // 16, 64, 2):
        raise PmnError("conv5x5s2_wino: weights are not in pack_conv5x5s2_wino layout for this input")
    out = torch.empty((N, (H - 1) // 2 + 1, (W - 1) // 2 + 1, cout), dtype=torch.float32, device=x.device)
    with torch.cuda.device(x.device):
        check(_lib.lib().pmn_conv5x5s2_wino(x.data_ptr(), weights.data_ptr(), shift.data_ptr(), out.data_ptr(), N, H, W, cin,
                                            cout, 1 if relu else 0, _stream(x)), "pmn_conv5x5s2_wino")
    return out


F16S_SHAPES = {(3, 1, 16, 16), (3, 1, 32, 32), (3, 1, 64, 64), (5, 2, 8, 16), (5, 2, 16, 32), (5, 2, 32, 64)}


def conv2d_f16s(x: torch.Tensor, weights: torch.Tensor, shift: torch.Tensor, k: int, stride: int, relu: bool = True) -> torch.Tensor:
    _dev(x, "x")
    _f16_domain_probe(x)
    _dev(shift, "shift")
    if not isinstance(weights, torch.Tensor) or not weights.is_cuda or weights.dtype != torch.float16 or not weights.is_contiguous():
        raise PmnError("conv2d_f16s: weights must be a contiguous float16 tensor on a ROCm GPU (params.pack_conv_f16s)")
    N, H, W, cin = x.shape
    cout = shift.shape[0]
    if (k, stride, cin, cout) not in F16S_SHAPES:
        raise PmnError(f"conv2d_f16s: unsupported layer (k={k}, stride={stride}, cin={cin}, cout={cout})")
    from . import params as _params
    cc = _params.f16s_chunk(cin, k)
    if tuple(weights.shape) != (cin // cc, (k * k * (cc // 8) + 3) // 4, cout // 16, 2, 64, 8):
        raise PmnError("conv2d_f16s: weights are not in pack_conv_f16s layout for this input")
    out = torch.empty((N, (H - 1) // stride + 1, (W - 1) // stride + 1, cout), dtype=torch.float32, device=x.device)
    with torch.cuda.device(x.device):
        check(_lib.lib().pmn_conv2d_f16s(x.data_ptr(), weights.data_ptr(), shift.data_ptr(), out.data_ptr(), N, H, W, cin, cout, k,
                                         stride, 1 if relu else 0, _stream(x)), "pmn_conv2d_f16s")
    return out


def conv2d_f16s_pair(x: torch.Tensor, weights_a: torch.Tensor, shift_a: torch.Tensor, weights_b: torch.Tensor, shift_b: torch.Tensor,
                     relu: bool = True) -> torch.Tensor:
    _dev(x, "x")
    _f16_domain_probe(x)
    N, H, W, C = x.shape
    for w_, s_ in ((weights_a, shift_a), (weights_b, shift_b)):
        _dev(s_, "shift")
        if not isinstance(w_, torch.Tensor) or not w_.is_cuda or w_.dtype != torch.float16 or not w_.is_contiguous() or \
                tuple(w_.shape) != (1, 5, 1, 2, 64, 8) or s_.numel() != 16:
            raise PmnError("conv2d_f16s_pair: weights must be params.pack_conv_f16s of a (3, 1, 16, 16) layer on a ROCm GPU")
    if C != 16:
        raise PmnError("conv2d_f16s_pair: 16-channel layers only")
    out = torch.empty((N, H, W, 16), dtype=torch.float32, device=x.device)
    with torch.cuda.device(x.device):
        check(_lib.lib().pmn_conv2d_f16s_pair(x.data_ptr(), weights_a.data_ptr(), shift_a.data_ptr(), weights_b.data_ptr(), shift_b.data_ptr(),
                                              out.data_ptr(), N, H, W, 16, 1 if relu else 0, _stream(x)), "pmn_conv2d_f16s_pair")
    return out


def pointwise_split_mfma(x: torch.Tensor, weights: torch.Tensor, shift: torch.Tensor, cout: int, ca: int):
    for n_, t_ in (("x", x), ("weights", weights), ("shift", shift)):
        _dev(t_, n_)
    N, H, W, cin = x.shape
    coutp = shift.shape[0]
    if tuple(weights.shape) != (1, cin // 8, coutp // 32, 64, 4) or not 0 < ca < cout <= coutp:
        raise PmnError("pointwise_split_mfma: weights are not in pack_conv_mfma layout for this input")
    out_a = torch.empty((N, H, W, ca), dtype=torch.float32, device=x.device)
    out_b = torch.empty((N, H, W, cout - ca), dtype=torch.float32, device=x.device)
    with torch.cuda.device(x.device):
        check(_lib.lib().pmn_conv2d_mfma(x.data_ptr(), weights.data_ptr(), shift.data_ptr(), out_a.data_ptr(), out_b.data_ptr(),
                                         N, H, W, cin, cout, ca, 1, 1, 0, 1, 0, 0, _stream(x)), "pmn_conv2d_mfma")
    return out_a, out_b


def offset_heads_mfma(x: torch.Tensor, weights: torch.Tensor, shift: torch.Tensor, cout: int, ca: int, dil: int):
    for n_, t_ in (("x", x), ("weights", weights), ("shift", shift)):
        _dev(t_, n_)
    N, H, W, cin = x.shape
    coutp = shift.shape[0]
    if tuple(weights.shape) != (9, cin // 8, coutp // 32, 64, 4) or not 0 < ca <= cout <= coutp:
        raise PmnError("offset_heads_mfma: weights are not in pack_conv_mfma layout for this input")
    out_a = torch.empty((N, ca, H, W), dtype=torch.float32, device=x.device)
    out_b = torch.empty((N, cout - ca, H, W), dtype=torch.float32, device=x.device) if ca < cout else None
    with torch.cuda.device(x.device):
        check(_lib.lib().pmn_conv2d_mfma(x.data_ptr(), weights.data_ptr(), shift.data_ptr(), out_a.data_ptr(), _ptr(out_b), N,
                                         H, W, cin, cout, ca, 3, 1, dil, dil, 0, 1, _stream(x)), "pmn_conv2d_mfma")
    return out_a, out_b


F16S_HEAD_SHAPES = {(64, 2), (32, 4), (16, 6)}


def offset_heads_f16s(x: torch.Tensor, weights: torch.Tensor, shift: torch.Tensor, cout: int, ca: int, dil: int):
    _dev(x, "x")
    _f16_domain_probe(x)
    _dev(shift, "shift")
    N, H, W, cin = x.shape
    coutp = shift.shape[0]
    if not isinstance(weights, torch.Tensor) or not weights.is_cuda or weights.dtype != torch.float16 or not weights.is_contiguous() \
            or tuple(weights.shape) != (cin // 16, (9 * 2 + 3) // 4, coutp // 16, 2, 64, 8) or not 0 < ca <= cout <= coutp \
            or coutp != (cout + 15) // 16 * 16:
        raise PmnError("offset_heads_f16s: weights are not in pack_offset_heads_f16s layout for this input")
    out_a = torch.empty((N, ca, H, W), dtype=torch.float32, device=x.device)
    out_b = torch.empty((N, cout - ca, H, W), dtype=torch.float32, device=x.device) if ca < cout else None
    with torch.cuda.device(x.device):
        check(_lib.lib().pmn_offset_heads_f16s(x.data_ptr(), weights.data_ptr(), shift.data_ptr(), out_a.data_ptr(), _ptr(out_b), N,
                                               H, W, cin, cout, ca, dil, _stream(x)), "pmn_offset_heads_f16s")
    return out_a, out_b


def fpn_level(x: torch.Tensor, u: Optional[torch.Tensor], w: torch.Tensor, b: torch.Tensor, ca: int):
    for n_, t_ in (("x", x), ("w", w), ("b", b)):
        _dev(t_, n_)
    N, H, W, cin = x.shape
    cout = w.shape[1]
    if tuple(w.shape) != (cin, cout) or tuple(b.shape) != (cout,) or not 0 < ca <= cout:
        raise PmnError("fpn_level: inconsistent shapes")
    if u is not None:
        _dev(u, "u")
        if tuple(u.shape) != (N, H // 2, W // 2, cout) or H % 2 or W % 2:
            raise PmnError("fpn_level: `u` must be [N,H/2,W/2,cout]")
    out_a = torch.empty((N, H, W, ca), dtype=torch.float32, device=x.device)
    out_b = torch.empty((N, H, W, cout - ca), dtype=torch.float32, device=x.device) if ca < cout else None
    with torch.cuda.device(x.device):
        check(_lib.lib().pmn_fpn_level(x.data_ptr(), _ptr(u), w.data_ptr(), b.data_ptr(), out_a.data_ptr(), _ptr(out_b),
                                       N, H, W, cin, cout, ca, _stream(x)), "pmn_fpn_level")
    return out_a, out_b


def refine_front(img: torch.Tensor, t2: torch.Tensor, w0: torch.Tensor, s0: torch.Tensor, wd: torch.Tensor,
                 sd: torch.Tensor) -> torch.Tensor:
    for n_, t_ in (("img", img), ("t2", t2), ("w0", w0), ("s0", s0), ("wd", wd), ("sd", sd)):
        _dev(t_, n_)
    B, c, H, W = img.shape
    if c != 3 or H % 2 or W % 2 or tuple(t2.shape) != (B, H // 2, W // 2, 8) or tuple(w0.shape) != (3, 3, 3, 8) or \
            tuple(wd.shape) != (3, 3, 8, 8):
        raise PmnError("refine_front: inconsistent shapes")
    out = torch.empty((B, H, W, 16), dtype=torch.float32, device=img.device)
    with torch.cuda.device(img.device):
        check(_lib.lib().pmn_refine_front(img.data_ptr(), t2.data_ptr(), w0.data_ptr(), s0.data_ptr(), wd.data_ptr(),
                                          sd.data_ptr(), out.data_ptr(), B, H, W, _stream(img)), "pmn_refine_front")
    return out


def refine_tail(x16: torch.Tensor, w3: torch.Tensor, s3: torch.Tensor, wr: torch.Tensor, dnorm: torch.Tensor,
                depth_min: torch.Tensor, depth_max: torch.Tensor) -> torch.Tensor:
    for n_, t_ in (("x16", x16), ("w3", w3), ("s3", s3), ("wr", wr), ("dnorm", dnorm), ("depth_min", depth_min),
                   ("depth_max", depth_max)):
        _dev(t_, n_)
    B, H, W, c = x16.shape
    if c != 16 or H % 2 or W % 2 or tuple(dnorm.shape) != (B, 1, H // 2, W // 2) or tuple(w3.shape) != (2, 3, 3, 16, 4) or \
            tuple(wr.shape) != (3, 3, 8) or depth_min.numel() != B or depth_max.numel() != B:
        raise PmnError("refine_tail: inconsistent shapes")
    out = torch.empty((B, 1, H, W), dtype=torch.float32, device=x16.device)
    with torch.cuda.device(x16.device):
        check(_lib.lib().pmn_refine_tail(x16.data_ptr(), w3.data_ptr(), s3.data_ptr(), wr.data_ptr(), dnorm.data_ptr(),
                                         depth_min.data_ptr(), depth_max.data_ptr(), out.data_ptr(), B, H, W, _stream(x16)),
              "pmn_refine_tail")
    return out


def refine_fused(img: torch.Tensor, t2: torch.Tensor, w0: torch.Tensor, s0: torch.Tensor, wd: torch.Tensor, sd: torch.Tensor,
                 w3a: torch.Tensor, s3: torch.Tensor, wr: torch.Tensor, dnorm: torch.Tensor, depth_min: torch.Tensor,
                 depth_max: torch.Tensor) -> torch.Tensor:
    for n_, t_ in (("img", img), ("t2", t2), ("w0", w0), ("s0", s0), ("wd", wd), ("sd", sd), ("s3", s3), ("wr", wr), ("dnorm", dnorm),
                   ("depth_min", depth_min), ("depth_max", depth_max)):
        _dev(t_, n_)
    if not isinstance(w3a, torch.Tensor) or not w3a.is_cuda or w3a.dtype != torch.float16 or tuple(w3a.shape) != (5, 2, 64, 8) \
            or not w3a.is_contiguous():
        raise PmnError("refine_fused: w3a must be the float16 [5,2,64,8] tensor of params.pack_refine_conv3_f16s on a ROCm GPU")
    B, c, H, W = img.shape
    if c != 3 or H % 2 or W % 2 or tuple(t2.shape) != (B, H // 2, W // 2, 8) or tuple(dnorm.shape) != (B, 1, H // 2, W // 2) or \
            tuple(w0.shape) != (3, 3, 3, 8) or tuple(wd.shape) != (3, 3, 8, 8) or tuple(wr.shape) != (3, 3, 8) or s3.numel() != 8 or \
            depth_min.numel() != B or depth_max.numel() != B:
        raise PmnError("refine_fused: inconsistent shapes")
    _f16_domain_probe(img, t2)
    out = torch.empty((B, 1, H, W), dtype=torch.float32, device=img.device)
    with torch.cuda.device(img.device):
        check(_lib.lib().pmn_refine_fused(img.data_ptr(), t2.data_ptr(), w0.data_ptr(), s0.data_ptr(), wd.data_ptr(), sd.data_ptr(),
                                          w3a.data_ptr(), s3.data_ptr(), wr.data_ptr(), dnorm.data_ptr(), depth_min.data_ptr(),
                                          depth_max.data_ptr(), out.data_ptr(), B, H, W, _stream(img)), "pmn_refine_fused")
    return out


def deconv3x3s2(x: torch.Tensor, weights: torch.Tensor, shift: torch.Tensor, relu: bool = True) -> torch.Tensor:
    _dev(x, "x")
    _dev(weights, "weights")
    _dev(shift, "shift")
    N, Hi, Wi, cin = x.shape
    cout = weights.shape[3]
    out = torch.empty((N, 2 * Hi, 2 * Wi, cout), dtype=torch.float32, device=x.device)
    with torch.cuda.device(x.device):
        check(_lib.lib().pmn_deconv3x3s2(x.data_ptr(), weights.data_ptr(), shift.data_ptr(), out.data_ptr(), N, Hi, Wi, cin,
                                         cout, 1 if relu else 0, _stream(x)), "pmn_deconv3x3s2")
    return out


def stem(img: torch.Tensor, w0: torch.Tensor, s0: torch.Tensor, w1: torch.Tensor, s1: torch.Tensor,
         out: Optional[torch.Tensor] = None) -> torch.Tensor:
    for n_, t_ in (("img", img), ("w0", w0), ("s0", s0), ("w1", w1), ("s1", s1)):
        _dev(t_, n_)
    N, c, H, W = img.shape
    if c != 3 or tuple(w0.shape) != (3, 3, 3, 8) or tuple(w1.shape) != (3, 3, 8, 8):
        raise PmnError("stem: expects a 3-channel image and 3->8->8 weights")
    if out is None:
        out = torch.empty((N, H, W, 8), dtype=torch.float32, device=img.device)
    else:
        _dev(out, "out")
        if tuple(out.shape) != (N, H, W, 8):
            raise PmnError("stem: bad `out` shape")
    with torch.cuda.device(img.device):
        check(_lib.lib().pmn_stem(img.data_ptr(), w0.data_ptr(), s0.data_ptr(), w1.data_ptr(), s1.data_ptr(), out.data_ptr(),
                                  N, H, W, _stream(img)), "pmn_stem")
    return out


def stem_f16s(img: torch.Tensor, w0: torch.Tensor, s0: torch.Tensor, w1a: torch.Tensor, s1: torch.Tensor,
              out: Optional[torch.Tensor] = None) -> torch.Tensor:
    for n_, t_ in (("img", img), ("w0", w0), ("s0", s0), ("s1", s1)):
        _dev(t_, n_)
    if not isinstance(w1a, torch.Tensor) or not w1a.is_cuda or w1a.dtype != torch.float16 or tuple(w1a.shape) != (3, 2, 64, 8) \
            or not w1a.is_contiguous():
        raise PmnError("stem_f16s: w1a must be the float16 [3,2,64,8] tensor of params.pack_stem_conv1_f16s on a ROCm GPU")
    N, c, H, W = img.shape
    if c != 3 or tuple(w0.shape) != (3, 3, 3, 8):
        raise PmnError("stem_f16s: expects a 3-channel image and 3->8 conv0 weights")
    _f16_domain_probe(img)
    if out is None:
        out = torch.empty((N, H, W, 8), dtype=torch.float32, device=img.device)
    else:
        _dev(out, "out")
        if tuple(out.shape) != (N, H, W, 8):
            raise PmnError("stem_f16s: bad `out` shape")
    with torch.cuda.device(img.device):
        check(_lib.lib().pmn_stem_f16s(img.data_ptr(), w0.data_ptr(), s0.data_ptr(), w1a.data_ptr(), s1.data_ptr(), out.data_ptr(),
                                       N, H, W, _stream(img)), "pmn_stem_f16s")
    return out


def stem_f16s_views(images: "SourceTable", w0: torch.Tensor, s0: torch.Tensor, w1a: torch.Tensor, s1: torch.Tensor) -> torch.Tensor:
    for n_, t_ in (("w0", w0), ("s0", s0), ("s1", s1)):
        _dev(t_, n_)
    if not isinstance(images, SourceTable) or len(images.shape) != 5 or images.shape[2] != 3:
        raise PmnError("stem_f16s_views: a SourceTable of shape (views, B, 3, H, W)")
    if not isinstance(w1a, torch.Tensor) or not w1a.is_cuda or w1a.dtype != torch.float16 or tuple(w1a.shape) != (3, 2, 64, 8) \
            or not w1a.is_contiguous() or tuple(w0.shape) != (3, 3, 3, 8):
        raise PmnError("stem_f16s_views: 3->8 conv0 weights and the float16 [3,2,64,8] tensor of params.pack_stem_conv1_f16s")
    V, B, _, H, W = images.shape
    out = torch.empty((V * B, H, W, 8), dtype=torch.float32, device=images.device)
    with torch.cuda.device(images.device):
        check(_lib.lib().pmn_stem_f16s_views(images.table.data_ptr(), V, w0.data_ptr(), s0.data_ptr(), w1a.data_ptr(), s1.data_ptr(),
                                             out.data_ptr(), B, H, W, _stream(out)), "pmn_stem_f16s_views")
    return out


def fuse_view(maps: torch.Tensor, ref_slot: int, src_slots: Sequence[int], mats: torch.Tensor, geo_pixel_thres: float,
              geo_depth_thres: float, geo_mask_thres: int, photo_thres: float, want_depth_avg: bool = False,
              want_geo_sum: bool = False, sizes: Optional[Sequence[Tuple[int, int]]] = None):
    _dev(maps, "maps")
    _dev(mats, "mats")
    if sizes is None:
        if maps.dim() != 4 or maps.shape[1] != 2:
            raise PmnError("fuse_view: maps must be [V,2,H,W] (or [V,F] flat slots with sizes=)")
        V, _, H, W = maps.shape
        stride = 2 * H * W
        sizes = [(H, W)] * V
    else:
        if maps.dim() != 2 or len(sizes) != maps.shape[0]:
            raise PmnError("fuse_view: with sizes= maps must be [V,F] flat slots and sizes must have V entries")
        V, stride = maps.shape
        if any(h < 1 or w < 1 or 2 * h * w > stride for h, w in sizes):
            raise PmnError("fuse_view: a view's maps do not fit its slot")
    n = len(src_slots)
    if n > _lib.MAX_FUSE_SRC:
        raise PmnError(f"fuse_view: at most {_lib.MAX_FUSE_SRC} source views per reference view")
    if not 0 <= ref_slot < V or any(not 0 <= s < V for s in src_slots):
        raise PmnError("fuse_view: slot out of range")
    if mats.numel() != 48 + 64 * n:
        raise PmnError("fuse_view: mats must hold 48 + 64 * n_src floats (fusion.camera_block)")
    H, W = sizes[ref_slot]
    slots, slots_p = _host_i32(np.asarray(list(src_slots) if n else [0], np.int32), max(n, 1), "src_slots")
    hw, hw_p = _host_i32(np.asarray([x for s in src_slots for x in sizes[s]] if n else [0, 0], np.int32), max(2 * n, 2), "src_hw")
    masks = torch.empty((3, H, W), dtype=torch.uint8, device=maps.device)
    xyz = torch.empty((H, W, 3), dtype=torch.float32, device=maps.device)
    davg = torch.empty((H, W), dtype=torch.float64, device=maps.device) if want_depth_avg else None
    gsum = torch.empty((H, W), dtype=torch.int32, device=maps.device) if want_geo_sum else None
    with torch.cuda.device(maps.device):
        check(_lib.lib().pmn_fuse_view(maps.data_ptr(), int(stride), int(ref_slot), slots_p, hw_p, n, mats.data_ptr(), H, W,
                                       float(geo_pixel_thres), float(geo_depth_thres), int(geo_mask_thres), float(photo_thres),
                                       masks.data_ptr(), xyz.data_ptr(), _ptr(davg), _ptr(gsum), _stream(maps)),
              "pmn_fuse_view")
    del slots, hw
    return masks, xyz, davg, gsum


def depth_normals(depth: torch.Tensor, intrinsics, radius: int = 2, rel_thres: float = 0.01) -> torch.Tensor:
    _dev(depth, "depth")
    if depth.dim() not in (2, 3) or depth.numel() == 0:
        raise PmnError("depth_normals: depth must be [H,W] or [B,H,W], H, W >= 1")
    if isinstance(radius, bool) or not isinstance(radius, (int, np.integer)) or not 1 <= int(radius) <= 3:
        raise PmnError("depth_normals: radius must be 1, 2 or 3")
    with np.errstate(over="ignore"):
        rel_thres = float(np.float32(rel_thres))
    if not (np.isfinite(rel_thres) and rel_thres > 0.0):
        raise PmnError("depth_normals: rel_thres must be a positive finite float32")
    K = np.ascontiguousarray((intrinsics.detach().cpu().numpy() if isinstance(intrinsics, torch.Tensor) else np.asarray(intrinsics)),
                             np.float32)
    batched = depth.dim() == 3
    B = depth.shape[0] if batched else 1
    if tuple(K.shape) != ((B, 3, 3) if batched else (3, 3)):
        raise PmnError("depth_normals: intrinsics must be [3,3] for a [H,W] map, [B,3,3] for [B,H,W] maps")
    if not np.isfinite(K).all():
        raise PmnError("depth_normals: intrinsics must be finite")
    K = K.reshape(B, 9)
    H, W = depth.shape[-2:]
    out = torch.empty((B, 3, H, W), dtype=torch.float32, device=depth.device)
    with torch.cuda.device(depth.device):
        for b in range(B):
            k, k_p = _host_f32(K[b], 9, "intrinsics")
            check(_lib.lib().pmn_depth_normals((depth[b] if batched else depth).data_ptr(), H, W, k_p, int(radius), rel_thres,
                                               out[b].data_ptr(), _stream(depth)), "pmn_depth_normals")
            del k
    return out if batched else out[0]



def _colour_planes(tsdf, rgb, cweight, what, layout):
    if (rgb is None) != (cweight is None):
        raise PmnError(f"{what}: rgb and cweight come together or not at all")
    if rgb is not None:
        _dev(rgb, "rgb")
        _dev(cweight, "cweight")
        if tuple(rgb.shape) != (3,) + tuple(tsdf.shape) or cweight.shape != tsdf.shape or rgb.device != tsdf.device or \
                cweight.device != tsdf.device:
            raise PmnError(f"{what}: {layout}")


def _volume_planes(tsdf, weight, rgb, cweight, what):
    _dev(tsdf, "tsdf")
    _dev(weight, "weight")
    if tsdf.dim() != 3 or tsdf.numel() == 0 or weight.shape != tsdf.shape or weight.device != tsdf.device:
        raise PmnError(f"{what}: tsdf and weight must be [nz,ny,nx] planes of one volume on one device")
    _colour_planes(tsdf, rgb, cweight, what, "rgb must be [3,nz,ny,nx] and cweight [nz,ny,nx] on the volume's device")
    nz, ny, nx = tsdf.shape
    if nz > 65535 or tsdf.numel() > 2 ** 31 - 1:
        raise PmnError(f"{what}: a volume holds at most 2^31 - 1 samples and 65535 planes")
    return _host_i32(np.asarray([nx, ny, nz]), 3, "dims")


def _positive_f32(v, what):
    with np.errstate(over="ignore"):
        v = float(np.float32(v))
    if not (np.isfinite(v) and v > 0.0):
        raise PmnError(f"{what} must be a positive finite float32")
    return v


def _placement(origin, voxel, trunc, what):
    org, org_p = _host_f32(np.asarray(origin, np.float32), 3, "origin")
    if not np.isfinite(org).all():
        raise PmnError(f"{what}: origin must be finite")
    return org, org_p, _positive_f32(voxel, f"{what}: voxel"), None if trunc is None else _positive_f32(trunc, f"{what}: trunc")


def _view_args(maps, slots, sizes, cams, masks, images, dev, what):
    _dev(maps, "maps")
    if maps.dim() < 2 or maps.device != dev:
        raise PmnError(f"{what}: maps must be [S,...] slots on the volume's device")
    S, stride = maps.shape[0], maps[0].numel()
    V = len(slots)
    if not 1 <= V <= _lib.TSDF_MAX_VIEWS:
        raise PmnError(f"{what}: 1 .. {_lib.TSDF_MAX_VIEWS} views per launch, got {V}")
    if len(sizes) != V or any(not 0 <= int(s) < S for s in slots) or any(h < 1 or w < 1 or h * w > stride for h, w in sizes):
        raise PmnError(f"{what}: a slot is out of range or a view's depth map does not fit its slot")
    cam = np.ascontiguousarray(np.asarray(cams, np.float32).reshape(-1))
    if cam.size != 21 * V or not np.isfinite(cam).all():
        raise PmnError(f"{what}: cams must hold 21 finite floats per view (K, then the upper 3x4 of the extrinsic)")

    def table(items, shape_of, name):
        if items is None:
            return None, None
        if len(items) != V:
            raise PmnError(f"{what}: {name} must have one entry (a tensor or None) per view")
        arr = (ctypes.c_void_p * V)()
        for n, t in enumerate(items):
            if t is None:
                continue
            if not isinstance(t, torch.Tensor) or not t.is_cuda or t.device != dev or t.dtype != torch.uint8 or \
                    not t.is_contiguous() or tuple(t.shape) != shape_of(*sizes[n]):
                raise PmnError(f"{what}: {name}[{n}] must be a contiguous uint8 tensor {shape_of(*sizes[n])} on the volume's device "
                               f"(no CPU fallback)")
            arr[n] = t.data_ptr()
        return arr, ctypes.cast(arr, ctypes.c_void_p)

    m_arr, m_p = table(masks, lambda h, w: (h, w), "masks")
    i_arr, i_p = table(images, lambda h, w: (h, w, 3), "images")
    sl, sl_p = _host_i32(np.asarray(list(slots)), V, "slots")
    hw, hw_p = _host_i32(np.asarray([x for s in sizes for x in s]), 2 * V, "sizes")
    return V, int(stride), cam, (m_arr, i_arr, sl, hw), sl_p, hw_p, m_p, i_p


def tsdf_integrate(tsdf: torch.Tensor, weight: torch.Tensor, rgb: Optional[torch.Tensor], cweight: Optional[torch.Tensor], origin,
                   voxel: float, trunc: float, maps: torch.Tensor, slots: Sequence[int], sizes: Sequence[Tuple[int, int]], cams,
                   masks: Optional[Sequence[Optional[torch.Tensor]]] = None,
                   images: Optional[Sequence[Optional[torch.Tensor]]] = None) -> None:
    dims, dims_p = _volume_planes(tsdf, weight, rgb, cweight, "tsdf_integrate")
    org, org_p, voxel, trunc = _placement(origin, voxel, trunc, "tsdf_integrate")
    V, stride, cam, keep, sl_p, hw_p, m_p, i_p = _view_args(maps, slots, sizes, cams, masks, images, tsdf.device, "tsdf_integrate")
    with torch.cuda.device(tsdf.device):
        check(_lib.lib().pmn_tsdf_integrate(tsdf.data_ptr(), weight.data_ptr(), _ptr(rgb), _ptr(cweight), dims_p, org_p, voxel, trunc,
                                            maps.data_ptr(), stride, sl_p, hw_p, m_p, i_p, cam.ctypes.data_as(ctypes.c_void_p), V,
                                            _stream(tsdf)), "pmn_tsdf_integrate")
    del dims, org, keep


def _popcount_u8(m: torch.Tensor) -> torch.Tensor:
    m = m - ((m >> 1) & 0x55)
    m = (m & 0x33) + ((m >> 2) & 0x33)
    return (m + (m >> 4)) & 0x0F


def _mt_extract(what, tsdf, color, normals, count, emit):
    dev = tsdf.device
    vmask = torch.empty(tsdf.shape, dtype=torch.uint8, device=dev)
    ntri = torch.empty(tsdf.shape, dtype=torch.uint8, device=dev)
    with torch.cuda.device(dev):
        count(vmask, ntri)
        vcount = _popcount_u8(vmask)
        totals = torch.stack((vcount.sum(dtype=torch.int64), ntri.sum(dtype=torch.int64))).tolist()
        nv, nt = int(totals[0]), int(totals[1])
        if nv > 2 ** 31 - 1 or nt > 2 ** 31 - 1:
            raise PmnError(f"{what}: {nv} vertices / {nt} triangles do not fit int32 indices; use a larger voxel")
        vscan = torch.cumsum(vcount.reshape(-1), 0, dtype=torch.int32)
        tscan = torch.cumsum(ntri.reshape(-1), 0, dtype=torch.int32)
        del vcount
        vertices = torch.empty((nv, 3), dtype=torch.float32, device=dev)
        faces = torch.empty((nt, 3), dtype=torch.int32, device=dev)
        colors = torch.empty((nv, 3), dtype=torch.uint8, device=dev) if color else None
        nrm = torch.empty((nv, 3), dtype=torch.float32, device=dev) if normals else None
        if nv:
            emit(vmask, ntri, vscan, tscan, vertices, colors, nrm, faces)
    return vertices, faces, colors, nrm


def mt_extract(tsdf: torch.Tensor, weight: torch.Tensor, origin, voxel: float, min_weight: float = 1.0,
               rgb: Optional[torch.Tensor] = None, cweight: Optional[torch.Tensor] = None, normals: bool = True):
    dims, dims_p = _volume_planes(tsdf, weight, rgb, cweight, "mt_extract")
    org, org_p, voxel, _ = _placement(origin, voxel, None, "mt_extract")
    min_weight = float(np.float32(min_weight))
    if not np.isfinite(min_weight):
        raise PmnError("mt_extract: min_weight must be finite")
    L, planes, stream = _lib.lib(), (tsdf.data_ptr(), weight.data_ptr()), _stream(tsdf)

    def count(vmask, ntri):
        check(L.pmn_mt_count(*planes, dims_p, min_weight, vmask.data_ptr(), ntri.data_ptr(), stream), "pmn_mt_count")

    def emit(vmask, ntri, vscan, tscan, vertices, colors, nrm, faces):
        check(L.pmn_mt_emit(*planes, _ptr(rgb), _ptr(cweight), dims_p, org_p, voxel, min_weight, vmask.data_ptr(), ntri.data_ptr(),
                            vscan.data_ptr(), tscan.data_ptr(), vertices.data_ptr(), _ptr(colors), _ptr(nrm), faces.data_ptr(), stream),
              "pmn_mt_emit")

    out = _mt_extract("mt_extract", tsdf, rgb is not None, normals, count, emit)
    del dims, org
    return out



SPARSE_BLOCK = 8
SPARSE_MAX_AXIS = 2 ** 19
SPARSE_MAX_TABLE = 2 ** 28
SPARSE_MAX_BLOCKS = (2 ** 31 - 1) // SPARSE_BLOCK ** 3


def sparse_blocks(dims) -> Tuple[int, int, int]:
    nx, ny, nz = (int(d) for d in dims)
    nb = tuple(-(-n // SPARSE_BLOCK) for n in (nx, ny, nz))
    if min(nx, ny, nz) < 2 or max(nx, ny, nz) >= SPARSE_MAX_AXIS or nb[0] * nb[1] * nb[2] > SPARSE_MAX_TABLE:
        raise PmnError(f"sparse volume: dims {nx} x {ny} x {nz} must be 2 .. {SPARSE_MAX_AXIS - 1} per axis and at most "
                       f"{SPARSE_MAX_TABLE} blocks of {SPARSE_BLOCK}^3 samples")
    return nb


def _grid_args(dims, origin, voxel, trunc, what):
    nb = sparse_blocks(dims)
    d, d_p = _host_i32(np.asarray([int(x) for x in dims]), 3, "dims")
    org, org_p, voxel, trunc = _placement(origin, voxel, trunc, what)
    return nb, (d, org), d_p, org_p, voxel, trunc


def inverse_cameras(cams) -> np.ndarray:
    cams = np.asarray(cams, np.float32).reshape(-1, 21).astype(np.float64)
    out = np.empty((len(cams), 21), np.float32)
    for n, c in enumerate(cams):
        E = np.eye(4)
        E[:3] = c[9:].reshape(3, 4)
        try:
            with np.errstate(all="ignore"):
                out[n, :9] = np.linalg.inv(c[:9].reshape(3, 3)).reshape(9)
                out[n, 9:] = np.linalg.inv(E)[:3].reshape(12)
        except np.linalg.LinAlgError as e:
            raise PmnError(f"tsdf_mark_blocks: camera {n} is singular") from e
    if not np.isfinite(out).all():
        raise PmnError("tsdf_mark_blocks: a camera has no finite float32 inverse")
    return out


def tsdf_mark_blocks(flags: torch.Tensor, overflow: torch.Tensor, dims, origin, voxel: float, trunc: float, maps: torch.Tensor,
                     slots: Sequence[int], sizes: Sequence[Tuple[int, int]], cams,
                     masks: Optional[Sequence[Optional[torch.Tensor]]] = None) -> None:
    _dev_as(flags, "flags", torch.uint8)
    _dev_as(overflow, "overflow", torch.int32)
    nb, keep, dims_p, org_p, voxel, trunc = _grid_args(dims, origin, voxel, trunc, "tsdf_mark_blocks")
    if tuple(flags.shape) != nb[::-1]:
        raise PmnError(f"tsdf_mark_blocks: flags must be a contiguous uint8 tensor {nb[::-1]} (nbz, nby, nbx)")
    if overflow.numel() != 1 or overflow.device != flags.device:
        raise PmnError("tsdf_mark_blocks: overflow must be one int32 on the flags' device")
    V, stride, cam, keep2, sl_p, hw_p, m_p, _ = _view_args(maps, slots, sizes, cams, masks, None, flags.device, "tsdf_mark_blocks")
    inv = np.ascontiguousarray(inverse_cameras(cam).reshape(-1))
    with torch.cuda.device(flags.device):
        check(_lib.lib().pmn_tsdf_mark_blocks(flags.data_ptr(), overflow.data_ptr(), dims_p, org_p, voxel, trunc, maps.data_ptr(), stride,
                                              sl_p, hw_p, m_p, inv.ctypes.data_as(ctypes.c_void_p), V, _stream(flags)),
              "pmn_tsdf_mark_blocks")
    del keep, keep2


def _pool_planes(tsdf, weight, rgb, cweight, blocks, what):
    _dev(tsdf, "tsdf")
    _dev(weight, "weight")
    _dev_as(blocks, "blocks", torch.int32)
    B = tsdf.shape[0] if tsdf.dim() == 4 else 0
    shape = (B,) + (SPARSE_BLOCK,) * 3
    if not 1 <= B <= SPARSE_MAX_BLOCKS or tuple(tsdf.shape) != shape or tuple(weight.shape) != shape or weight.device != tsdf.device:
        raise PmnError(f"{what}: tsdf and weight must be [B,8,8,8] pool planes on one device, 1 <= B <= {SPARSE_MAX_BLOCKS}")
    _colour_planes(tsdf, rgb, cweight, what, "rgb must be [3,B,8,8,8] and cweight [B,8,8,8] on the pool's device")
    if tuple(blocks.shape) != (B,) or blocks.device != tsdf.device:
        raise PmnError(f"{what}: blocks must be a contiguous int32 [B] tensor on the pool's device")
    return B


def tsdf_integrate_blocks(tsdf: torch.Tensor, weight: torch.Tensor, rgb: Optional[torch.Tensor], cweight: Optional[torch.Tensor],
                          blocks: torch.Tensor, dims, origin, voxel: float, trunc: float, maps: torch.Tensor, slots: Sequence[int],
                          sizes: Sequence[Tuple[int, int]], cams, masks: Optional[Sequence[Optional[torch.Tensor]]] = None,
                          images: Optional[Sequence[Optional[torch.Tensor]]] = None) -> None:
    B = _pool_planes(tsdf, weight, rgb, cweight, blocks, "tsdf_integrate_blocks")
    nb, keep, dims_p, org_p, voxel, trunc = _grid_args(dims, origin, voxel, trunc, "tsdf_integrate_blocks")
    V, stride, cam, keep2, sl_p, hw_p, m_p, i_p = _view_args(maps, slots, sizes, cams, masks, images, tsdf.device, "tsdf_integrate_blocks")
    with torch.cuda.device(tsdf.device):
        check(_lib.lib().pmn_tsdf_integrate_blocks(tsdf.data_ptr(), weight.data_ptr(), _ptr(rgb), _ptr(cweight), blocks.data_ptr(), B,
                                                   dims_p, org_p, voxel, trunc, maps.data_ptr(), stride, sl_p, hw_p, m_p, i_p,
                                                   cam.ctypes.data_as(ctypes.c_void_p), V, _stream(tsdf)), "pmn_tsdf_integrate_blocks")
    del keep, keep2


def mt_extract_blocks(tsdf: torch.Tensor, weight: torch.Tensor, table: torch.Tensor, blocks: torch.Tensor, dims, origin, voxel: float,
                      min_weight: float = 1.0, rgb: Optional[torch.Tensor] = None, cweight: Optional[torch.Tensor] = None,
                      normals: bool = True):
    B = _pool_planes(tsdf, weight, rgb, cweight, blocks, "mt_extract_blocks")
    nb, keep, dims_p, org_p, voxel, _ = _grid_args(dims, origin, voxel, None, "mt_extract_blocks")
    _dev_as(table, "table", torch.int32)
    if tuple(table.shape) != nb[::-1] or table.device != tsdf.device:
        raise PmnError(f"mt_extract_blocks: table must be a contiguous int32 tensor {nb[::-1]} (nbz, nby, nbx) on the pool's device")
    min_weight = float(np.float32(min_weight))
    if not (np.isfinite(min_weight) and min_weight > 0):
        raise PmnError("mt_extract_blocks: min_weight must be positive and finite")
    L, planes, lists, stream = _lib.lib(), (tsdf.data_ptr(), weight.data_ptr()), (table.data_ptr(), blocks.data_ptr(), B), _stream(tsdf)

    def count(vmask, ntri):
        check(L.pmn_mt_count_blocks(*planes, *lists, dims_p, min_weight, vmask.data_ptr(), ntri.data_ptr(), stream), "pmn_mt_count_blocks")

    def emit(vmask, ntri, vscan, tscan, vertices, colors, nrm, faces):
        check(L.pmn_mt_emit_blocks(*planes, _ptr(rgb), _ptr(cweight), *lists, dims_p, org_p, voxel, min_weight, vmask.data_ptr(),
                                   ntri.data_ptr(), vscan.data_ptr(), tscan.data_ptr(), vertices.data_ptr(), _ptr(colors), _ptr(nrm),
                                   faces.data_ptr(), stream), "pmn_mt_emit_blocks")

    out = _mt_extract("mt_extract_blocks", tsdf, rgb is not None, normals, count, emit)
    del keep
    return out



def _raster_common(keys: torch.Tensor, counters: torch.Tensor, cam, what: str):
    if not isinstance(keys, torch.Tensor) or not keys.is_cuda:
        raise PmnError(f"{what}: keys must be a tensor on a ROCm GPU (no CPU fallback)")
    if keys.dtype != torch.int64 or keys.dim() != 2 or not keys.is_contiguous() or keys.numel() == 0:
        raise PmnError(f"{what}: keys must be a contiguous [h,w] int64 tensor (the uint64 keys' bits)")
    h, w = keys.shape
    if h > _lib.RASTER_MAX_DIM or w > _lib.RASTER_MAX_DIM:
        raise PmnError(f"{what}: a view is at most {_lib.RASTER_MAX_DIM} pixels per side")
    if not isinstance(counters, torch.Tensor) or counters.device != keys.device or counters.dtype != torch.int32 or \
            counters.numel() != 4 or not counters.is_contiguous():
        raise PmnError(f"{what}: counters must be 4 int32 on the keys' device")
    cam = np.ascontiguousarray(np.asarray(cam, np.float32).reshape(-1))
    if cam.size != 21 or not np.isfinite(cam).all():
        raise PmnError(f"{what}: cam must hold 21 finite floats (K, then the upper 3x4 of the extrinsic)")
    return h, w, cam


def _raster_array(t, dtype, keys, name, what, rows=None):
    if not isinstance(t, torch.Tensor) or not t.is_cuda or t.device != keys.device or t.dtype != dtype or t.dim() != 2 or \
            t.shape[1] != 3 or not t.is_contiguous() or t.shape[0] < 1 or (rows is not None and t.shape[0] != rows):
        raise PmnError(f"{what}: {name} must be a contiguous [{'n' if rows is None else rows},3] {dtype} tensor on the keys' device "
                       f"(no CPU fallback)")
    return t


def raster_triangles(vertices: torch.Tensor, faces: torch.Tensor, cam, keys: torch.Tensor, counters: torch.Tensor,
                     worklist: torch.Tensor, max_box: int = 0) -> None:
    h, w, cam = _raster_common(keys, counters, cam, "raster_triangles")
    _raster_array(vertices, torch.float32, keys, "vertices", "raster_triangles")
    _raster_array(faces, torch.int32, keys, "faces", "raster_triangles")
    if vertices.shape[0] > 2 ** 31 - 1 or faces.shape[0] > 2 ** 31 - 1:
        raise PmnError("raster_triangles: at most 2^31 - 1 vertices and faces")
    if not isinstance(worklist, torch.Tensor) or worklist.device != keys.device or worklist.dtype != torch.int32 or \
            not worklist.is_contiguous() or worklist.numel() < faces.shape[0]:
        raise PmnError("raster_triangles: worklist must hold one int32 per face on the keys' device")
    if int(max_box) < 0:
        raise PmnError("raster_triangles: max_box must be >= 0")
    with torch.cuda.device(keys.device):
        check(_lib.lib().pmn_raster_triangles(vertices.data_ptr(), vertices.shape[0], faces.data_ptr(), faces.shape[0],
                                              cam.ctypes.data_as(ctypes.c_void_p), h, w, int(max_box), keys.data_ptr(),
                                              counters.data_ptr(), worklist.data_ptr(), _stream(keys)), "pmn_raster_triangles")


def splat_points(points: torch.Tensor, cam, keys: torch.Tensor, counters: torch.Tensor, radius_px: float = 0.0,
                 radius_world: float = 0.0) -> None:
    h, w, cam = _raster_common(keys, counters, cam, "splat_points")
    _raster_array(points, torch.float32, keys, "points", "splat_points")
    if points.shape[0] > 2 ** 31 - 1:
        raise PmnError("splat_points: at most 2^31 - 1 points (the index plane is int32)")
    with np.errstate(over="ignore"):
        radius_px, radius_world = float(np.float32(radius_px)), float(np.float32(radius_world))
    if not (0.0 <= radius_px <= _lib.SPLAT_MAX_RADIUS) or not (np.isfinite(radius_world) and radius_world >= 0.0) or \
            (radius_px > 0.0 and radius_world > 0.0):
        raise PmnError(f"splat_points: radius_px must be 0 .. {_lib.SPLAT_MAX_RADIUS}, radius_world >= 0 and finite, and only one "
                       f"of them non-zero")
    with torch.cuda.device(keys.device):
        check(_lib.lib().pmn_splat_points(points.data_ptr(), points.shape[0], cam.ctypes.data_as(ctypes.c_void_p), h, w, radius_px,
                                          radius_world, keys.data_ptr(), counters.data_ptr(), _stream(keys)), "pmn_splat_points")


def raster_resolve(keys: torch.Tensor, cam, vertices: torch.Tensor, faces: Optional[torch.Tensor], depth: torch.Tensor,
                   index: torch.Tensor, colors: Optional[torch.Tensor] = None, normals: Optional[torch.Tensor] = None,
                   shade: bool = False, rgb: Optional[torch.Tensor] = None, normal: Optional[torch.Tensor] = None) -> None:
    if not isinstance(keys, torch.Tensor) or not keys.is_cuda or keys.dtype != torch.int64 or keys.dim() != 2 or \
            not keys.is_contiguous() or keys.numel() == 0:
        raise PmnError("raster_resolve: keys must be a contiguous [h,w] int64 tensor on a ROCm GPU (no CPU fallback)")
    h, w = keys.shape
    cam = np.ascontiguousarray(np.asarray(cam, np.float32).reshape(-1))
    if cam.size != 21 or not np.isfinite(cam).all():
        raise PmnError("raster_resolve: cam must hold 21 finite floats (K, then the upper 3x4 of the extrinsic)")
    _raster_array(vertices, torch.float32, keys, "vertices", "raster_resolve")
    nv = vertices.shape[0]
    if faces is not None:
        _raster_array(faces, torch.int32, keys, "faces", "raster_resolve")
    if colors is not None:
        _raster_array(colors, torch.uint8, keys, "colors", "raster_resolve", nv)
    if normals is not None:
        _raster_array(normals, torch.float32, keys, "normals", "raster_resolve", nv)

    def plane(t, dtype, shape, name):
        if not isinstance(t, torch.Tensor) or t.device != keys.device or t.dtype != dtype or tuple(t.shape) != shape or \
                not t.is_contiguous():
            raise PmnError(f"raster_resolve: {name} must be a contiguous {shape} {dtype} tensor on the keys' device")
        return t

    plane(depth, torch.float32, (h, w), "depth")
    plane(index, torch.int32, (h, w), "index")
    if rgb is not None:
        plane(rgb, torch.uint8, (h, w, 3), "rgb")
    if normal is not None:
        plane(normal, torch.float32, (h, w, 3), "normal")
    with torch.cuda.device(keys.device):
        check(_lib.lib().pmn_raster_resolve(keys.data_ptr(), h, w, cam.ctypes.data_as(ctypes.c_void_p), vertices.data_ptr(), nv,
                                            _ptr(faces), 0 if faces is None else faces.shape[0], _ptr(colors), _ptr(normals),
                                            1 if shade else 0, depth.data_ptr(), index.data_ptr(), _ptr(rgb), _ptr(normal),
                                            _stream(keys)), "pmn_raster_resolve")


class PointPacker:

    def __init__(self, capacity: int, device, max_views: int = 1024, normals: bool = False) -> None:
        self.capacity = int(capacity)
        self.normals = bool(normals)
        self.record_size = 27 if self.normals else 15
        self.records = torch.empty((self.record_size * self.capacity,), dtype=torch.uint8, device=device)
        self.cursor = torch.zeros((1,), dtype=torch.int64, device=device)
        self.view_counts = torch.zeros((max_views,), dtype=torch.int32, device=device)
        self.scratch = None
        self.n = 0

    def reset(self) -> None:
        self.cursor.zero_()
        self.n = 0

    def append(self, final_mask: torch.Tensor, xyz: torch.Tensor, image_hwc: torch.Tensor,
               normals_chw: Optional[torch.Tensor] = None, rotation: Optional[torch.Tensor] = None) -> None:
        _dev(xyz, "xyz")
        if self.normals != (normals_chw is not None) or self.normals != (rotation is not None):
            raise PmnError("pack_points: a packer built with normals=True takes normals_chw and rotation with every view, "
                           "one built without takes neither")
        for t, name in ((final_mask, "final_mask"), (image_hwc, "image_hwc")):
            if not isinstance(t, torch.Tensor) or t.device != self.records.device:
                raise PmnError(f"pack_points: {name} must be a tensor on {self.records.device} (no CPU fallback)")
        H, W = final_mask.shape
        if final_mask.dtype != torch.uint8 or not final_mask.is_contiguous():
            raise PmnError("pack_points: final_mask must be contiguous uint8 [H,W]")
        if tuple(xyz.shape) != (H, W, 3) or xyz.dtype != torch.float32 or not xyz.is_contiguous():
            raise PmnError("pack_points: xyz must be contiguous float32 [H,W,3]")
        if tuple(image_hwc.shape) != (H, W, 3) or image_hwc.dtype not in (torch.uint8, torch.float32) or not image_hwc.is_contiguous():
            raise PmnError("pack_points: image must be contiguous uint8 or float32 [H,W,3]")
        if self.n >= self.view_counts.numel():
            raise PmnError("pack_points: more views than the packer was sized for")
        nb = (H * W + 1023) // 1024
        if self.scratch is None or self.scratch.numel() < nb:
            self.scratch = torch.empty((nb,), dtype=torch.int64, device=self.records.device)
        if self.normals:
            for t, name in ((normals_chw, "normals_chw"), (rotation, "rotation")):
                if not isinstance(t, torch.Tensor) or t.device != self.records.device or t.dtype != torch.float32:
                    raise PmnError(f"pack_points: {name} must be a float32 tensor on {self.records.device} (no CPU fallback)")
            if tuple(normals_chw.shape) != (3, H, W) or not normals_chw.is_contiguous():
                raise PmnError("pack_points: normals_chw must be contiguous float32 [3,H,W]")
            if tuple(rotation.shape) not in ((3, 3), (4, 4)) or rotation.stride(1) != 1 or rotation.stride(0) < 3:
                raise PmnError("pack_points: rotation must be float32 [3,3] or [4,4] with unit column stride")
            with torch.cuda.device(self.records.device):
                check(_lib.lib().pmn_pack_points_normals(final_mask.data_ptr(), xyz.data_ptr(), normals_chw.data_ptr(),
                                                         rotation.data_ptr(), int(rotation.stride(0)), image_hwc.data_ptr(),
                                                         1 if image_hwc.dtype == torch.float32 else 0, H, W, self.records.data_ptr(),
                                                         self.capacity, self.cursor.data_ptr(), self.view_counts[self.n:].data_ptr(),
                                                         self.scratch.data_ptr(), _stream(self.records)), "pmn_pack_points_normals")
            self.n += 1
            return
        with torch.cuda.device(self.records.device):
            check(_lib.lib().pmn_pack_points(final_mask.data_ptr(), xyz.data_ptr(), image_hwc.data_ptr(),
                                             1 if image_hwc.dtype == torch.float32 else 0, H, W, self.records.data_ptr(),
                                             self.capacity, self.cursor.data_ptr(), self.view_counts[self.n:].data_ptr(),
                                             self.scratch.data_ptr(), _stream(self.records)), "pmn_pack_points")
        self.n += 1

    def counts(self):
        c = self.view_counts[:self.n].cpu().tolist()
        if any(x < 0 for x in c):
            raise PmnError("pack_points: the record buffer is too small for this scan")
        return c


def view_scores(cam_centers: torch.Tensor, xyz: torch.Tensor, obs_ptr: torch.Tensor, obs_pt: torch.Tensor, trk_ptr: torch.Tensor,
                trk_img: torch.Tensor, theta0: float, sigma1: float, sigma2: float, out: Optional[torch.Tensor] = None) -> torch.Tensor:
    specs = ((cam_centers, "cam_centers", torch.float64), (xyz, "xyz", torch.float64), (obs_ptr, "obs_ptr", torch.int64),
             (obs_pt, "obs_pt", torch.int32), (trk_ptr, "trk_ptr", torch.int64), (trk_img, "trk_img", torch.int32))
    for t, name, dtype in specs:
        if not isinstance(t, torch.Tensor):
            raise PmnError(f"{name}: expected a torch.Tensor")
        if not t.is_cuda:
            raise PmnError(f"{name}: tensor is on {t.device}; patchmatchnet_amd runs only on a ROCm GPU (no CPU fallback)")
        if t.dtype != dtype:
            raise PmnError(f"{name}: expected {dtype}, got {t.dtype}")
        if not t.is_contiguous():
            raise PmnError(f"{name}: tensor must be contiguous")
        if t.device != cam_centers.device:
            raise PmnError(f"{name}: every input must be on {cam_centers.device}")
    if cam_centers.dim() != 2 or cam_centers.shape[1] != 3 or cam_centers.shape[0] < 1:
        raise PmnError("view_scores: cam_centers must be [N,3] with N >= 1")
    if xyz.dim() != 2 or xyz.shape[1] != 3:
        raise PmnError("view_scores: xyz must be [P,3]")
    N, P = int(cam_centers.shape[0]), int(xyz.shape[0])
    if obs_ptr.shape != (N + 1,) or trk_ptr.shape != (P + 1,) or obs_pt.dim() != 1 or trk_img.dim() != 1:
        raise PmnError("view_scores: obs_ptr must be [N+1], trk_ptr [P+1], obs_pt and trk_img 1-D")
    if N >= 2 ** 31 or P >= 2 ** 31:
        raise PmnError("view_scores: more than 2^31 - 1 images or points")
    if out is None:
        out = torch.empty((N, N), dtype=torch.float64, device=cam_centers.device)
    elif not (out.is_cuda and out.dtype == torch.float64 and out.is_contiguous() and out.shape == (N, N)
              and out.device == cam_centers.device):
        raise PmnError("view_scores: out must be a contiguous float64 [N,N] tensor on the inputs' device")
    with torch.cuda.device(cam_centers.device):
        check(_lib.lib().pmn_view_scores(cam_centers.data_ptr(), _ptr(xyz) if P else None, obs_ptr.data_ptr(),
                                         obs_pt.data_ptr() if obs_pt.numel() else None, trk_ptr.data_ptr(),
                                         trk_img.data_ptr() if trk_img.numel() else None, N, P, int(obs_pt.numel()),
                                         int(trk_img.numel()), float(theta0), float(sigma1), float(sigma2), out.data_ptr(),
                                         _stream(cam_centers)),
              "pmn_view_scores")
    return out


def depth_metrics(depth_gt: torch.Tensor, depth_min: torch.Tensor, depth_patchmatch, thresholds: Sequence[float] = (1.0, 2.0, 4.0, 8.0),
                  out: Optional[torch.Tensor] = None, scratch: Optional[torch.Tensor] = None) -> torch.Tensor:
    _dev(depth_gt, "depth_gt")
    _dev(depth_min, "depth_min")
    if depth_gt.dim() == 4 and depth_gt.shape[1] == 1:
        depth_gt = depth_gt.view(depth_gt.shape[0], depth_gt.shape[2], depth_gt.shape[3])
    if depth_gt.dim() != 3:
        raise PmnError(f"depth_metrics: depth_gt must be [B,H,W] or [B,1,H,W], got {tuple(depth_gt.shape)}")
    B, H, W = (int(x) for x in depth_gt.shape)
    if tuple(depth_min.shape) != (B,):
        raise PmnError(f"depth_metrics: depth_min must be [{B}], got {tuple(depth_min.shape)}")
    stages = [depth_patchmatch[s] for s in sorted(depth_patchmatch)] if isinstance(depth_patchmatch, dict) else list(depth_patchmatch)
    if isinstance(depth_patchmatch, dict) and sorted(depth_patchmatch) != list(range(len(stages))):
        raise PmnError(f"depth_metrics: depth_patchmatch must hold stages 0..n-1, got {sorted(depth_patchmatch)}")
    if not 1 <= len(stages) <= _lib.METRICS_MAX_STAGES:
        raise PmnError(f"depth_metrics: 1 to {_lib.METRICS_MAX_STAGES} stages, got {len(stages)}")
    thresholds = [float(t) for t in thresholds]
    if len(thresholds) > _lib.METRICS_MAX_THRESHOLDS:
        raise PmnError(f"depth_metrics: at most {_lib.METRICS_MAX_THRESHOLDS} thresholds, got {len(thresholds)}")
    maps, iters, hw = [], [], []
    for s, ms in enumerate(stages):
        ms = list(ms)
        if not 1 <= len(ms) <= _lib.METRICS_MAX_ITERS:
            raise PmnError(f"depth_metrics: stage {s} has {len(ms)} maps; 1 to {_lib.METRICS_MAX_ITERS} are supported")
        shape = None
        for k, m in enumerate(ms):
            _dev(m, f"depth_patchmatch[{s}][{k}]")
            if m.device != depth_gt.device:
                raise PmnError(f"depth_patchmatch[{s}][{k}]: on {m.device}, the ground truth on {depth_gt.device}")
            sh = tuple(m.shape)
            if len(sh) == 4 and sh[1] == 1:
                sh = (sh[0], sh[2], sh[3])
            if len(sh) != 3 or sh[0] != B or (shape is not None and sh != shape):
                raise PmnError(f"depth_metrics: depth_patchmatch[{s}][{k}] is {tuple(m.shape)}; expected [{B},1,h,w] like the stage's "
                               "other maps")
            shape = sh
            maps.append(m.data_ptr())
        if shape[1:] != (H >> s, W >> s) or min(shape[1:]) < 1:
            raise PmnError(f"depth_metrics: the stage-{s} maps are {shape[1]}x{shape[2]}, the nearest down-sampling of the {H}x{W} "
                           f"ground truth is {H >> s}x{W >> s} (the model's stage maps match it only when H and W are multiples of "
                           f"{1 << (len(stages) - 1)})")
        iters.append(len(ms))
        hw += [shape[1], shape[2]]
    if out is None:
        out = torch.empty((B, _lib.METRICS_ROW), dtype=torch.float64, device=depth_gt.device)
    elif not (out.is_cuda and out.dtype == torch.float64 and out.is_contiguous() and tuple(out.shape) == (B, _lib.METRICS_ROW)
              and out.device == depth_gt.device):
        raise PmnError(f"depth_metrics: out must be a contiguous float64 [{B},{_lib.METRICS_ROW}] tensor on the ground truth's device")
    need = _lib.metrics_scratch(B, H, W)
    if scratch is None:
        scratch = torch.empty(need, dtype=torch.float64, device=depth_gt.device)
    elif not (scratch.is_cuda and scratch.dtype == torch.float64 and scratch.is_contiguous() and scratch.numel() >= need
              and scratch.device == depth_gt.device):
        raise PmnError(f"depth_metrics: scratch must be a contiguous float64 tensor of at least {need} elements on the same device")
    maps_h = (ctypes.c_void_p * len(maps))(*maps)
    iters_h = (ctypes.c_int * len(iters))(*iters)
    hw_h = (ctypes.c_int * len(hw))(*hw)
    thr_h = (ctypes.c_float * max(len(thresholds), 1))(*thresholds)
    with torch.cuda.device(depth_gt.device):
        check(_lib.lib().pmn_depth_metrics(depth_gt.data_ptr(), depth_min.data_ptr(), ctypes.cast(maps_h, ctypes.c_void_p),
                                           ctypes.cast(iters_h, ctypes.c_void_p), ctypes.cast(hw_h, ctypes.c_void_p), len(stages),
                                           ctypes.cast(thr_h, ctypes.c_void_p), len(thresholds), B, H, W, scratch.data_ptr(),
                                           int(scratch.numel()), out.data_ptr(), _stream(depth_gt)),
              "pmn_depth_metrics")
    return out
```

### patchmatchnet_amd/patchmatch.py

```python
from __future__ import annotations

from typing import List, Optional, Tuple

import numpy as np
import torch
import torch.nn as nn

import warnings

from . import _lib, ops, params
from ._lib import PmnError
from .module import ConvBnReLU3D, is_empty


class _PointwiseMLP(nn.Module):

    _last = "similarity"

    def __init__(self, G: int) -> None:
        super().__init__()
        self.G = G
        self.conv0 = ConvBnReLU3D(in_channels=G, out_channels=16, kernel_size=1, stride=1, pad=0)
        self.conv1 = ConvBnReLU3D(in_channels=16, out_channels=8, kernel_size=1, stride=1, pad=0)
        self._packed: Optional[np.ndarray] = None
        self._packed_key = None
        self._packed_dev: Optional[torch.Tensor] = None

    def _sources(self) -> List[torch.Tensor]:
        last = getattr(self, self._last)
        return [self.conv0.conv.weight, *self.conv0.bn_tensors(), self.conv1.conv.weight, *self.conv1.bn_tensors(),
                last.weight, last.bias]

    def packed(self) -> np.ndarray:
        key = params.versions(self._sources())
        if self._packed is None or key != self._packed_key:
            last = getattr(self, self._last)
            self._packed = params.pack_mlp(self.conv0.conv.weight, self.conv0.bn_tensors(), self.conv1.conv.weight,
                                           self.conv1.bn_tensors(), last.weight, last.bias)
            self._packed_key = key
            self._packed_dev = None
        return self._packed

    def packed_device(self) -> torch.Tensor:
        blk = self.packed()
        dev = self.conv0.conv.weight.device
        if self._packed_dev is None or self._packed_dev.device != dev:
            self._packed_dev = torch.from_numpy(blk).to(dev)
        return self._packed_dev


class PixelwiseNet(_PointwiseMLP):

    _last = "conv2"

    def __init__(self, G: int) -> None:
        super().__init__(G)
        self.conv2 = nn.Conv3d(in_channels=8, out_channels=1, kernel_size=1, stride=1, padding=0)
        self.output = nn.Sigmoid()


class SimilarityNet(_PointwiseMLP):

    def __init__(self, G: int) -> None:
        super().__init__(G)
        self.similarity = nn.Conv3d(in_channels=8, out_channels=1, kernel_size=1, stride=1, padding=0)


class FeatureWeightNet(_PointwiseMLP):

    def __init__(self, neighbors: int = 9, G: int = 8) -> None:
        super().__init__(G)
        self.neighbors = neighbors
        self.similarity = nn.Conv3d(in_channels=8, out_channels=1, kernel_size=1, stride=1, padding=0)
        self.output = nn.Sigmoid()

    def forward(self, ref_nhwc: torch.Tensor, eval_offsets: torch.Tensor, table: np.ndarray) -> torch.Tensor:
        return ops.feature_weight(ref_nhwc, eval_offsets, table, self.packed_device(), self.G)


class DepthInitialization(nn.Module):

    def __init__(self, patchmatch_num_sample: int = 1) -> None:
        super().__init__()
        self.patchmatch_num_sample = patchmatch_num_sample

    def forward(self, min_depth: torch.Tensor, max_depth: torch.Tensor, height: int, width: int,
                depth_interval_scale: float, device: torch.device, depth: torch.Tensor) -> torch.Tensor:
        noise = None
        if is_empty(depth):
            noise = torch.rand(size=(min_depth.size()[0], 48, height, width), device=device)
        ds, _ = ops.init_hypotheses(noise, None if noise is not None else depth.detach().contiguous(), 0,
                                    min_depth.float().contiguous(), max_depth.float().contiguous(),
                                    self.patchmatch_num_sample, depth_interval_scale, None, None, height, width)
        return ds


class Propagation(nn.Module):

    def __init__(self) -> None:
        super().__init__()


class Evaluation(nn.Module):

    def __init__(self, G: int = 8) -> None:
        super().__init__()
        self.G = G
        self.pixel_wise_net = PixelwiseNet(self.G)
        self.softmax = nn.LogSoftmax(dim=1)
        self.similarity_net = SimilarityNet(self.G)

    def forward(self, ref_feature: torch.Tensor, src_features: List[torch.Tensor], ref_proj: torch.Tensor,
                src_projs: List[torch.Tensor], depth_sample: torch.Tensor, grid: Optional[torch.Tensor],
                weight: Optional[torch.Tensor], view_weights: torch.Tensor, is_inverse: bool, *,
                fused: Optional[dict] = None, debug: Optional[dict] = None) -> Tuple[torch.Tensor, torch.Tensor, torch.Tensor]:
        N = len(src_features) if src_features is not None else fused["src_nhwc"].shape[0]
        if src_features is not None and src_projs is not None and len(src_features) != len(src_projs):
            raise AssertionError("Patchmatch Evaluation: Different number of images and projection matrices")
        have_vw = not is_empty(view_weights)
        if have_vw and view_weights.size()[1] != N:
            raise AssertionError("Patchmatch Evaluation: Different number of images and view weights")
        f = fused or {}
        ref_nhwc = f.get("ref_nhwc")
        src_nhwc = f.get("src_nhwc")
        rel_proj = f.get("rel_proj")
        if ref_nhwc is None:
            ref_nhwc = ops.nchw_to_nhwc(ref_feature.detach())
        if rel_proj is None:
            rel_proj = ops.relative_projection(src_projs, ref_proj)
        if src_nhwc is None:
            src_nhwc, sizes = ops.stack_sources_padded([s.detach() for s in src_features])
            rel_proj = ops.rescale_projection_rows(rel_proj, sizes, tuple(src_nhwc.shape[2:4]))
        depth_sample = depth_sample.contiguous()
        cost, vw, argmax, sim = ops.warp_correlate(
            ref_nhwc, src_nhwc, rel_proj.contiguous(), depth_sample, view_weights.contiguous() if have_vw else None,
            int(f.get("vw_shift", 0)), self.similarity_net.packed_device(),
            None if have_vw else self.pixel_wise_net.packed_device(), self.G,
            want_similarity=debug is not None, want_argmax=debug is not None and not have_vw)
        if fused is not None and grid is None:
            score, depth = ops.aggregate_regress(cost, depth_sample, f["xnorm"], f["feature_weight"], f["eval_offsets"],
                                                 f["table"], f["interval_scale"], is_inverse)
        else:
            if grid is None or weight is None:
                raise PmnError("Evaluation.forward needs grid and weight (reference signature) or the fused-form arguments")
            B, D, h, w = depth_sample.shape
            K = grid.shape[1] // h
            sampled = torch.nn.functional.grid_sample(cost.contiguous(), grid, mode="bilinear", padding_mode="border",
                                                      align_corners=False).view(B, D, K, h, w)
            score = torch.sum(sampled * weight, dim=2)
            score = torch.exp(self.softmax(score))
            if is_inverse:
                index = torch.arange(0, D, 1, device=score.device).view(1, D, 1, 1)
                index = torch.sum(index * score, dim=1)
                inv_min = 1.0 / depth_sample[:, -1, :, :]
                inv_max = 1.0 / depth_sample[:, 0, :, :]
                depth = 1.0 / (inv_max + index / (D - 1) * (inv_min - inv_max))
            else:
                depth = torch.sum(depth_sample * score, dim=1)
        if debug is not None:
            debug.update(cost=cost, similarity=sim, view_weight_argmax=argmax)
        return depth, score, vw.detach()


class PatchMatch(nn.Module):

    def __init__(self, propagation_out_range: int = 2, patchmatch_iteration: int = 2, patchmatch_num_sample: int = 16,
                 patchmatch_interval_scale: float = 0.025, num_feature: int = 64, G: int = 8,
                 propagate_neighbors: int = 16, evaluate_neighbors: int = 9, stage: int = 3) -> None:
        super().__init__()
        self.patchmatch_iteration = patchmatch_iteration
        self.patchmatch_interval_scale = patchmatch_interval_scale
        self.propa_num_feature = num_feature
        self.G = G
        self.stage = stage
        self.dilation = propagation_out_range
        self.propagate_neighbors = propagate_neighbors
        self.evaluate_neighbors = evaluate_neighbors
        if propagate_neighbors not in (0, 4, 8, 16) or evaluate_neighbors not in (9, 17):
            raise NotImplementedError

        self.depth_initialization = DepthInitialization(patchmatch_num_sample)
        self.propagation = Propagation()
        self.evaluation = Evaluation(self.G)
        self.propa_conv = nn.Conv2d(num_feature, max(2 * propagate_neighbors, 1), kernel_size=3, stride=1,
                                    padding=self.dilation, dilation=self.dilation, bias=True)
        nn.init.constant_(self.propa_conv.weight, 0.0)
        nn.init.constant_(self.propa_conv.bias, 0.0)
        self.eval_conv = nn.Conv2d(num_feature, 2 * evaluate_neighbors, kernel_size=3, stride=1, padding=self.dilation,
                                   dilation=self.dilation, bias=True)
        nn.init.constant_(self.eval_conv.weight, 0.0)
        nn.init.constant_(self.eval_conv.bias, 0.0)
        self.feature_weight_net = FeatureWeightNet(evaluate_neighbors, self.G)

        self.hip_offset_heads = True
        self.f16_split = True
        self.f16_domain_error: Optional[str] = None
        self.heads_hook = None
        self._heads = None
        self._heads_key = None
        self._ptable = params.propagation_table(propagate_neighbors, self.dilation) if propagate_neighbors > 0 else None
        self._etable = params.evaluation_table(evaluate_neighbors, self.dilation)

    def _packed_heads(self):
        srcs = [self.propa_conv.weight, self.propa_conv.bias, self.eval_conv.weight, self.eval_conv.bias]
        key = params.versions(srcs)
        if self._heads is None or key != self._heads_key:
            dev = self.eval_conv.weight.device
            pk = {}
            for name, m in (("propa", self.propa_conv), ("eval", self.eval_conv)):
                w, s = params.pack_conv(m.weight, bias=m.bias)
                pk[name] = (torch.from_numpy(w).to(dev), torch.from_numpy(s).to(dev))
            self.f16_domain_error = None
            for name, mods in (("both", (self.propa_conv, self.eval_conv)), ("eval_only", (self.eval_conv,))):
                wcat = torch.cat([m.weight.detach() for m in mods], 0)
                bcat = torch.cat([m.bias.detach() for m in mods], 0)
                rows = wcat.shape[0]
                if (self.eval_conv.in_channels, self.dilation) in ops.F16S_HEAD_SHAPES and (rows + 15) // 16 * 16 in (32, 48, 64):
                    try:
                        w, s = params.pack_offset_heads_f16s(wcat, bcat)
                        pk["f16s_" + name] = (torch.from_numpy(w).to(dev), torch.from_numpy(s).to(dev))
                    except params.F16DomainError as e:
                        self.f16_domain_error = f"offset heads: {e}"
            if self.f16_domain_error is not None:
                warnings.warn(f"PatchMatch stage {self.stage}: " + self.f16_domain_error + " -- using pmn_conv2d (fp32)", RuntimeWarning,
                              stacklevel=2)
            self._heads, self._heads_key = pk, key
        return self._heads

    def forward(self, ref_feature: torch.Tensor, src_features: List[torch.Tensor], ref_proj: torch.Tensor,
                src_projs: List[torch.Tensor], depth_min: torch.Tensor, depth_max: torch.Tensor, depth: torch.Tensor,
                view_weights: torch.Tensor, depth_shift: int = 0, vw_shift: int = 0, noise: Optional[torch.Tensor] = None,
                debug: Optional[list] = None, ref_nhwc: Optional[torch.Tensor] = None,
                src_nhwc: Optional[torch.Tensor] = None, rel_proj: Optional[torch.Tensor] = None
                ) -> Tuple[List[torch.Tensor], torch.Tensor, torch.Tensor]:
        if len(src_features) != len(src_projs):
            raise AssertionError("Patchmatch Evaluation: Different number of images and projection matrices")
        if not ref_feature.is_cuda:
            raise PmnError("patchmatchnet_amd.PatchMatch runs on a ROCm GPU only (no CPU fallback)")
        device = ref_feature.device
        batch, _, height, width = ref_feature.size()

        propagate_any = self.propagate_neighbors > 0 and not (self.stage == 1 and self.patchmatch_iteration == 1)
        if ref_nhwc is None:
            ref_nhwc = ops.nchw_to_nhwc(ref_feature.detach())
        if self.hip_offset_heads:
            pk = self._packed_heads()
            fkey = "f16s_both" if propagate_any else "f16s_eval_only"
            if self.f16_split and fkey in pk:
                n_p, n_e = (2 * self.propagate_neighbors if propagate_any else 0), 2 * self.evaluate_neighbors
                a_, b_ = ops.offset_heads_f16s(ref_nhwc, *pk[fkey], n_p + n_e, n_p if propagate_any else n_e, self.dilation)
                propa_offsets, eval_offsets = (a_, b_) if propagate_any else (None, a_)
            elif self.heads_hook is not None and (hooked := self.heads_hook(self, ref_nhwc, propagate_any)) is not None:
                propa_offsets, eval_offsets = hooked
            else:
                propa_offsets = ops.conv2d(ref_nhwc, *pk["propa"], 2 * self.propagate_neighbors, 3, 1, self.dilation,
                                           self.dilation, out_nchw=True) if propagate_any else None
                eval_offsets = ops.conv2d(ref_nhwc, *pk["eval"], 2 * self.evaluate_neighbors, 3, 1, self.dilation,
                                          self.dilation, out_nchw=True)
        else:
            ref_feature = ref_feature.contiguous()
            propa_offsets = self.propa_conv(ref_feature).contiguous() if propagate_any else None
            eval_offsets = self.eval_conv(ref_feature).contiguous()
        if rel_proj is None:
            rel_proj = ops.relative_projection(src_projs, ref_proj)
        if src_nhwc is None:
            src_nhwc, sizes = ops.stack_sources_padded([f.detach() for f in src_features])
            rel_proj = ops.rescale_projection_rows(rel_proj, sizes, tuple(src_nhwc.shape[2:4]))
        rel_proj = rel_proj.contiguous()
        depth_min = depth_min.float().contiguous()
        depth_max = depth_max.float().contiguous()

        feature_weight = self.feature_weight_net(ref_nhwc, eval_offsets, self._etable)

        depth_sample = depth
        cur_shift = depth_shift
        score = torch.empty(0, device=device)
        depth_samples: List[torch.Tensor] = []
        for it in range(1, self.patchmatch_iteration + 1):
            is_inverse = self.stage == 1 and it == self.patchmatch_iteration
            first_random = is_empty(depth_sample)
            if first_random and noise is None:
                noise = torch.rand(size=(batch, 48, height, width), device=device)
            propagate = self.propagate_neighbors > 0 and not (self.stage == 1 and it == self.patchmatch_iteration)
            hyp, xnorm = ops.init_hypotheses(
                noise.contiguous() if first_random else None,
                None if first_random else depth_sample.detach().contiguous(), cur_shift, depth_min, depth_max,
                self.depth_initialization.patchmatch_num_sample, self.patchmatch_interval_scale,
                propa_offsets if propagate else None, self._ptable if propagate else None, height, width)
            rec = {} if debug is not None else None
            had_view_weights = not is_empty(view_weights)
            d, score, view_weights = self.evaluation(
                ref_feature=ref_feature, src_features=src_features, ref_proj=ref_proj, src_projs=src_projs, depth_sample=hyp,
                grid=None, weight=None, view_weights=view_weights, is_inverse=is_inverse,
                fused=dict(xnorm=xnorm, eval_offsets=eval_offsets, table=self._etable, feature_weight=feature_weight,
                           interval_scale=self.patchmatch_interval_scale, vw_shift=vw_shift, ref_nhwc=ref_nhwc,
                           src_nhwc=src_nhwc, rel_proj=rel_proj), debug=rec)
            if not had_view_weights:
                vw_shift = 0
            if rec is not None:
                rec.update(depth_sample=hyp, xnorm=xnorm, feature_weight=feature_weight, score=score, depth=d,
                           view_weights=view_weights, eval_offsets=eval_offsets, propa_offsets=propa_offsets)
                debug.append(rec)
            depth_sample = d.unsqueeze(1)
            cur_shift = 0
            depth_samples.append(depth_sample)
        return depth_samples, score, view_weights
```

Before: 384.7.

## Fork launch plan so finer FPN levels run on a side stream concurrently

The recorded launch plan gains fork/switch/join markers that split entries into pre, side, main and post parts. Replay launches the side branch on a second stream, synchronised with events, so work such as the finer FPN levels and the per-stage offset-head precompute can overlap with the coarse-stage patchmatch. Read/write ranges and fresh allocations are tracked during recording so buffers stay alive and branches can be checked for independence. This adds event and stream overhead and the risk of hazards if the branch split is wrong.

```diff
diff --git a/include/pmn_hip.h b/include/pmn_hip.h
--- a/include/pmn_hip.h
+++ b/include/pmn_hip.h
@@ -128,6 +128,10 @@
 
 int pmn_check_f16_domain(const float *x, long long n, int *flag, void *stream);
 
+#define PMN_PLAN_PART_PRE 0
+#define PMN_PLAN_PART_SIDE 1
+#define PMN_PLAN_PART_MAIN 2
+#define PMN_PLAN_PART_POST 3
 int pmn_plan_create(void **plan_out);
 int pmn_plan_begin(void *plan);
 int pmn_plan_end(void *plan);
@@ -135,6 +139,11 @@
 const char *pmn_plan_kernel_name(const void *plan, int index);
 int pmn_plan_launch(const void *plan, void *stream);
 int pmn_plan_destroy(void *plan);
+int pmn_plan_fork(void *plan);
+int pmn_plan_switch(void *plan, int branch);
+int pmn_plan_join(void *plan);
+int pmn_plan_entry_branch(const void *plan, int index);
+int pmn_plan_launch_part(const void *plan, int part, void *stream);
 
 int pmn_view_scores(const double *cam_centers, const double *xyz, const long long *obs_ptr, const int *obs_pt,
                     const long long *trk_ptr, const int *trk_img, int N, int P, long long n_obs, long long n_trk,
diff --git a/patchmatchnet_amd/_lib.py b/patchmatchnet_amd/_lib.py
--- a/patchmatchnet_amd/_lib.py
+++ b/patchmatchnet_amd/_lib.py
@@ -72,6 +72,11 @@
     "pmn_plan_kernel_name": [_hp, _i],
     "pmn_plan_launch": [_hp, _s],
     "pmn_plan_destroy": [_hp],
+    "pmn_plan_fork": [_hp],
+    "pmn_plan_switch": [_hp, _i],
+    "pmn_plan_join": [_hp],
+    "pmn_plan_entry_branch": [_hp, _i],
+    "pmn_plan_launch_part": [_hp, _i, _s],
     "pmn_view_scores": [_fp] * 6 + [_i, _i, ctypes.c_longlong, ctypes.c_longlong] + [ctypes.c_double] * 3 + [_fp, _s],
     "pmn_depth_metrics": [_fp, _fp, _hp, _hp, _hp, _i, _hp, _i, _i, _i, _i, _fp, ctypes.c_longlong, _fp, _s],
     "pmn_nn_distance": [_fp, _ip, ctypes.c_longlong, _hp, ctypes.c_double, _hp, _fp, _ip, ctypes.c_longlong, ctypes.c_double, _fp, _ip,
@@ -95,6 +100,8 @@
     "pmn_mesh_face_samples": [_fp, _i, _ip, _i, ctypes.c_double, ctypes.c_ulonglong, _ip, _ip, _s],
     "pmn_mesh_sample": [_fp, _i, _ip, _i, _ip, _ip, ctypes.c_longlong, ctypes.c_ulonglong, _fp, _ip, _ip, _s],
 }
+
+PLAN_PART_PRE, PLAN_PART_SIDE, PLAN_PART_MAIN, PLAN_PART_POST = 0, 1, 2, 3
 
 METRICS_MAX_STAGES = 4
 METRICS_MAX_ITERS = 5
diff --git a/patchmatchnet_amd/csrc/plan.hip b/patchmatchnet_amd/csrc/plan.hip
--- a/patchmatchnet_amd/csrc/plan.hip
+++ b/patchmatchnet_amd/csrc/plan.hip
@@ -1,11 +1,19 @@
+#ifdef PMN_PLAN_HOST_STUBS
+#include PMN_PLAN_HOST_STUBS
+#else
 #include <hip/hip_runtime.h>
+#endif
 
 #include <cstring>
 #include <mutex>
 #include <new>
 #include <vector>
 
+#ifndef PMN_PLAN_HOST_STUBS
 #include "pmn_common.hpp"
+#endif
+
+enum { PMN_ENTRY_LAUNCH = 0, PMN_ENTRY_FORK = 1, PMN_ENTRY_JOIN = 2 };
 
 struct PmnPlanEntry {
     const void* func;
@@ -13,11 +21,15 @@
     size_t lds;
     int nargs;
     size_t first_arg;
+    int kind;
+    int branch;
 };
 
 struct PmnPlan {
     uint32_t magic;
     bool recording, poisoned, sealed;
+    bool forked, joined;
+    int branch;
     int device;
     std::vector<PmnPlanEntry> entries;
     std::vector<size_t> arg_offsets;
@@ -38,7 +50,7 @@
                     const size_t* sizes, const size_t* aligns) {
     if (!plan || plan->poisoned) return PMN_ERR_ARG;
     try {
-        PmnPlanEntry e{func, grid, block, lds, nargs, plan->arg_offsets.size()};
+        PmnPlanEntry e{func, grid, block, lds, nargs, plan->arg_offsets.size(), PMN_ENTRY_LAUNCH, plan->branch};
         for (int i = 0; i < nargs; ++i) {
             const size_t al = aligns[i] ? aligns[i] : 1;
             size_t off = (plan->blob.size() + al - 1) / al * al;
@@ -60,6 +72,8 @@
     if (!plan) return PMN_ERR_ARG;
     plan->magic = PMN_PLAN_MAGIC;
     plan->recording = plan->poisoned = plan->sealed = false;
+    plan->forked = plan->joined = false;
+    plan->branch = 0;
     plan->device = -1;
     *plan_out = plan;
     return PMN_OK;
@@ -79,6 +93,7 @@
     if (!plan || !plan->recording || pmn_tls_plan != plan) return PMN_ERR_ARG;
     pmn_tls_plan = nullptr;
     plan->recording = false;
+    if (plan->forked && !plan->joined) plan->poisoned = true;
     if (plan->poisoned) return PMN_ERR_ARG;
     try {
         plan->argv.resize(plan->arg_offsets.size());
@@ -91,6 +106,52 @@
     return PMN_OK;
 }
 
+static PmnPlan* recording_plan(void* p) {
+    PmnPlan* plan = as_plan(p);
+    return (plan && plan->recording && pmn_tls_plan == plan && !plan->poisoned) ? plan : nullptr;
+}
+
+static int append_marker(PmnPlan* plan, int kind) {
+    try {
+        plan->entries.push_back(PmnPlanEntry{nullptr, dim3(), dim3(), 0, 0, plan->arg_offsets.size(), kind, 0});
+    } catch (const std::bad_alloc&) {
+        plan->poisoned = true;
+        return PMN_ERR_ARG;
+    }
+    return PMN_OK;
+}
+
+extern "C" int pmn_plan_fork(void* p) {
+    PmnPlan* plan = recording_plan(p);
+    if (!plan || plan->forked) return PMN_ERR_ARG;
+    if (append_marker(plan, PMN_ENTRY_FORK) != PMN_OK) return PMN_ERR_ARG;
+    plan->forked = true;
+    plan->branch = 0;
+    return PMN_OK;
+}
+
+extern "C" int pmn_plan_switch(void* p, int branch) {
+    PmnPlan* plan = recording_plan(p);
+    if (!plan || !plan->forked || plan->joined || (branch != 0 && branch != 1)) return PMN_ERR_ARG;
+    plan->branch = branch;
+    return PMN_OK;
+}
+
+extern "C" int pmn_plan_join(void* p) {
+    PmnPlan* plan = recording_plan(p);
+    if (!plan || !plan->forked || plan->joined) return PMN_ERR_ARG;
+    if (append_marker(plan, PMN_ENTRY_JOIN) != PMN_OK) return PMN_ERR_ARG;
+    plan->joined = true;
+    plan->branch = 0;
+    return PMN_OK;
+}
+
+extern "C" int pmn_plan_entry_branch(const void* p, int index) {
+    const PmnPlan* plan = as_plan(const_cast<void*>(p));
+    if (!plan || index < 0 || index >= (int)plan->entries.size()) return PMN_ERR_ARG;
+    return plan->entries[index].branch;
+}
+
 extern "C" int pmn_plan_count(const void* p) {
     const PmnPlan* plan = as_plan(const_cast<void*>(p));
     if (!plan) return PMN_ERR_ARG;
@@ -100,16 +161,25 @@
 extern "C" const char* pmn_plan_kernel_name(const void* p, int index) {
     const PmnPlan* plan = as_plan(const_cast<void*>(p));
     if (!plan || index < 0 || index >= (int)plan->entries.size()) return nullptr;
-    return hipKernelNameRefByPtr(plan->entries[index].func, nullptr);
-}
-
-extern "C" int pmn_plan_launch(const void* p, void* stream) {
-    const PmnPlan* plan = as_plan(const_cast<void*>(p));
-    if (!plan || !plan->sealed) return PMN_ERR_ARG;
+    const PmnPlanEntry& e = plan->entries[index];
+    if (e.kind != PMN_ENTRY_LAUNCH) return e.kind == PMN_ENTRY_FORK ? "<fork>" : "<join>";
+    return hipKernelNameRefByPtr(e.func, nullptr);
+}
+
+static int launch_entries(const void* p, int part, void* stream) {
+    const PmnPlan* plan = as_plan(const_cast<void*>(p));
+    if (!plan || !plan->sealed || part > 3) return PMN_ERR_ARG;
     if (pmn_tls_plan != nullptr) return PMN_ERR_ARG;
     hipStream_t st = (hipStream_t)stream;
     void* const* argv = plan->argv.data();
+    int region = 0;
     for (const PmnPlanEntry& e : plan->entries) {
+        if (e.kind != PMN_ENTRY_LAUNCH) {
+            region = e.kind == PMN_ENTRY_FORK ? 1 : 2;
+            continue;
+        }
+        const int mine = region == 0 ? 0 : region == 2 ? 3 : (e.branch == 1 ? 1 : 2);
+        if (part >= 0 && part != mine) continue;
         if (hipLaunchKernel(e.func, e.grid, e.block, const_cast<void**>(argv + e.first_arg), e.lds, st) != hipSuccess) {
             (void)hipGetLastError();
             return PMN_ERR_LAUNCH;
@@ -118,6 +188,13 @@
     return PMN_OK;
 }
 
+extern "C" int pmn_plan_launch(const void* p, void* stream) { return launch_entries(p, -1, stream); }
+
+extern "C" int pmn_plan_launch_part(const void* p, int part, void* stream) {
+    if (part < 0) return PMN_ERR_ARG;
+    return launch_entries(p, part, stream);
+}
+
 extern "C" int pmn_plan_destroy(void* p) {
     PmnPlan* plan = as_plan(p);
     if (!plan) return PMN_ERR_ARG;
diff --git a/patchmatchnet_amd/graph.py b/patchmatchnet_amd/graph.py
--- a/patchmatchnet_amd/graph.py
+++ b/patchmatchnet_amd/graph.py
@@ -225,13 +225,20 @@
             raise PmnError(f"PlannedForward: the forward dispatched {func} while it was being recorded -- an operator outside "
                            "libpmn_hip.so cannot be part of a launch plan (it would run once, on uninitialised data, and never "
                            "again); this input signature has to run eagerly or through a path that only calls the library")
-        return func(*args, **(kwargs or {}))
+        out = func(*args, **(kwargs or {}))
+        from . import ops
+        ops._hold(out, fresh=not getattr(func, "is_view", False) and str(func).startswith("aten.") and
+                  (str(func) + ".").startswith(self._FRESH))
+        return out
+
+    _FRESH = ("aten.empty.", "aten.empty_strided.", "aten.empty_like.", "aten.new_empty.", "aten.new_empty_strided.")
 
 
 class PlannedForward(GraphedForward):
 
-    def __init__(self, model, max_graphs: int = 8, inputs_in_place: bool = False) -> None:
+    def __init__(self, model, max_graphs: int = 8, inputs_in_place: bool = False, fork: bool = True) -> None:
         super().__init__(model, max_graphs=max_graphs, inputs_in_place=inputs_in_place)
+        self.fork = fork
 
     def _record(self, run, dev):
         import ctypes
@@ -243,14 +250,18 @@
             plan = ctypes.c_void_p()
             _lib.check(L.pmn_plan_create(ctypes.byref(plan)), "pmn_plan_create")
             handle = _Plan(plan, pool)
+            from . import ops
             with torch.cuda.use_mem_pool(pool, device=dev):
                 _lib.check(L.pmn_plan_begin(plan), "pmn_plan_begin")
+                region = ops.begin_plan_recording(plan)
                 try:
                     with _LibraryLaunchesOnly():
                         depth, confidence, _ = run()
                 finally:
+                    ops.end_plan_recording()
                     rc = L.pmn_plan_end(plan)
                 _lib.check(rc, "pmn_plan_end")
+            handle.forked, handle.held_bytes = region.forked, region.held_bytes
         handle.count = L.pmn_plan_count(plan)
         if handle.count <= 0:
             raise PmnError("PlannedForward: the recording pass recorded no launch")
@@ -258,8 +269,23 @@
 
     def _replay(self, handle, dev) -> None:
         from . import _lib
+        L = _lib.lib()
         with torch.cuda.device(dev):
-            _lib.check(_lib.lib().pmn_plan_launch(handle.plan, torch.cuda.current_stream(dev).cuda_stream), "pmn_plan_launch")
+            cur = torch.cuda.current_stream(dev)
+            if not (handle.forked and self.fork):
+                _lib.check(L.pmn_plan_launch(handle.plan, cur.cuda_stream), "pmn_plan_launch")
+                return
+            if handle.side is None:
+                handle.side, handle.at_fork, handle.at_join = torch.cuda.Stream(dev), torch.cuda.Event(), torch.cuda.Event()
+            side = handle.side
+            _lib.check(L.pmn_plan_launch_part(handle.plan, _lib.PLAN_PART_PRE, cur.cuda_stream), "pmn_plan_launch_part")
+            handle.at_fork.record(cur)
+            side.wait_event(handle.at_fork)
+            _lib.check(L.pmn_plan_launch_part(handle.plan, _lib.PLAN_PART_SIDE, side.cuda_stream), "pmn_plan_launch_part")
+            _lib.check(L.pmn_plan_launch_part(handle.plan, _lib.PLAN_PART_MAIN, cur.cuda_stream), "pmn_plan_launch_part")
+            handle.at_join.record(side)
+            cur.wait_event(handle.at_join)
+            _lib.check(L.pmn_plan_launch_part(handle.plan, _lib.PLAN_PART_POST, cur.cuda_stream), "pmn_plan_launch_part")
 
 
 class PlannedValidationForward(PlannedForward):
@@ -304,11 +330,18 @@
 
     def __init__(self, plan, pool) -> None:
         self.plan, self.pool, self.count = plan, pool, 0
+        self.forked, self.held_bytes = False, 0
+        self.side = self.at_fork = self.at_join = None
 
     def kernel_names(self) -> List[str]:
         from . import _lib
         L = _lib.lib()
         return [(L.pmn_plan_kernel_name(self.plan, i) or b"?").decode() for i in range(self.count)]
+
+    def entry_branches(self) -> List[int]:
+        from . import _lib
+        L = _lib.lib()
+        return [L.pmn_plan_entry_branch(self.plan, i) for i in range(self.count)]
 
     def __del__(self):
         try:
diff --git a/patchmatchnet_amd/net.py b/patchmatchnet_amd/net.py
--- a/patchmatchnet_amd/net.py
+++ b/patchmatchnet_amd/net.py
@@ -85,7 +85,8 @@
             self._pack, self._pack_key = pk, key
         return self._pack
 
-    def forward_hip(self, x, image_table: Optional["ops.SourceTable"] = None) -> Dict[int, torch.Tensor]:
+    def forward_hip(self, x, image_table: Optional["ops.SourceTable"] = None, pending: Optional[dict] = None
+                    ) -> Dict[int, torch.Tensor]:
         pk = self._packed()
         imgs = list(x) if isinstance(x, (list, tuple)) else [x]
         B, _, H, W = imgs[0].shape
@@ -125,14 +126,21 @@
                 f3, u8 = ops.fpn_level(eighth, None, *pk["fpn8"], ca=64)
             else:
                 f3, u8 = ops.pointwise_split_mfma(eighth, *pk["fpn8_mfma"], cout=112, ca=64)
-            f2, u4 = ops.fpn_level(quarter, u8, *pk["fpn4"], ca=32)
-            f1, _ = ops.fpn_level(half, u4, *pk["fpn2"], ca=16)
-            return {3: f3, 2: f2, 1: f1}
+            if pending is not None:
+                pending.update(half=half, quarter=quarter, u8=u8)
+                return {3: f3}
+            return {3: f3, **self.finish_hip(dict(half=half, quarter=quarter, u8=u8))}
         out = {3: ops.conv2d(eighth, *pk["output1"], 64, 1)}
         top = ops.conv2d(quarter, *pk["inner1"], 64, 1, up=eighth)
         out[2] = ops.conv2d(top, *pk["output2"], 32, 1)
         out[1] = ops.fpn_tail(half, top, pk["inner2"][0], pk["inner2"][1], pk["output3"][0])
         return out
+
+    def finish_hip(self, pending: dict) -> Dict[int, torch.Tensor]:
+        pk = self._packed()
+        f2, u4 = ops.fpn_level(pending["quarter"], pending["u8"], *pk["fpn4"], ca=32)
+        f1, _ = ops.fpn_level(pending["half"], u4, *pk["fpn2"], ca=16)
+        return {2: f2, 1: f1}
 
     def forward(self, x: torch.Tensor) -> Dict[int, torch.Tensor]:
         half = self.conv4(self.conv3(self.conv2(self.conv1(self.conv0(x)))))
@@ -277,13 +285,14 @@
         return model
 
     def extract_features(self, images: List[torch.Tensor], stacked: Optional[dict] = None,
-                         image_table: Optional["ops.SourceTable"] = None) -> List[Dict[int, torch.Tensor]]:
+                         image_table: Optional["ops.SourceTable"] = None, pending: Optional[dict] = None
+                         ) -> List[Dict[int, torch.Tensor]]:
         same = all(im.shape == images[0].shape for im in images)
         B = images[0].shape[0]
         if image_table is not None and not (self.hip_feature_net and same and images[0].is_cuda and self.feature.f16_split):
             raise PmnError("image_table needs the HIP FeatureNet (f16_split) and same-size images on a ROCm device")
         if self.hip_feature_net and same and images[0].is_cuda:
-            f = self.feature.forward_hip(images, image_table=image_table)
+            f = self.feature.forward_hip(images, image_table=image_table, pending=pending)
             if stacked is not None:
                 stacked.update({("nhwc", s): t for s, t in f.items()})
             return [{s: t[i * B:(i + 1) * B].permute(0, 3, 1, 2) for s, t in f.items()} for i in range(len(images))]
@@ -296,6 +305,13 @@
                 stacked.update(f)
             return [{s: t[i * B:(i + 1) * B] for s, t in f.items()} for i in range(len(images))]
         return [self.feature(im) for im in images]
+
+    def finish_features(self, features: List[Dict[int, torch.Tensor]], stacked: dict, pending: dict) -> None:
+        f = self.feature.finish_hip(pending)
+        B = f[2].shape[0] // len(features)
+        stacked.update({("nhwc", s): t for s, t in f.items()})
+        for i, view in enumerate(features):
+            view.update({s: t[i * B:(i + 1) * B].permute(0, 3, 1, 2) for s, t in f.items()})
 
     def forward(self, images: List[torch.Tensor], intrinsics: torch.Tensor, extrinsics: torch.Tensor,
                 depth_min: torch.Tensor, depth_max: torch.Tensor, noise: Optional[torch.Tensor] = None,
@@ -313,8 +329,9 @@
         _, _, ref_height, ref_width = ref_image.size()
 
         stacked: Dict[int, torch.Tensor] = {}
+        pending: dict = {}
         if features is None:
-            features = self.extract_features(images, stacked, image_table)
+            features = self.extract_features(images, stacked, image_table, pending)
         elif features_nhwc is not None:
             stacked.update({("nhwc", st): t for st, t in features_nhwc.items()})
         ref_feature, src_features = features[0], features[1:]
@@ -331,7 +348,31 @@
         scale = 0.125
         depth_shift, vw_shift = 0, 0
         rel_all = ops.stage_projections(intrinsics, extrinsics, self.stages - 1, scale) if self.hip_projections else None
+
+
+        def stage_maps(stage):
+            if source_tables is not None:
+                return ref_nhwc_maps[stage], source_tables[stage]
+            if ("nhwc", stage) in stacked:
+                allv = stacked[("nhwc", stage)]
+            elif stage in stacked:
+                allv = stacked[("nhwc", stage)] = ops.nchw_to_nhwc(stacked[stage].contiguous())
+            else:
+                return None, None
+            return allv[:batch], allv[batch:].view(len(features) - 1, batch, *allv.shape[1:])
+
+        precomputed: Dict[int, dict] = {}
+        ops.plan_fork()
+        ops.plan_switch(1)
+        if pending:
+            self.finish_features(features, stacked, pending)
+        for stage in range(self.stages - 2, 0, -1):
+            precomputed[stage] = getattr(self, f"patchmatch_{stage}").prepare(features[0][stage], stage_maps(stage)[0])
+        ops.plan_switch(0)
         for stage in range(self.stages - 1, 0, -1):
+            if stage == self.stages - 2:
+                ops.plan_join()
+                pending.clear()
             if rel_all is None:
                 intrinsics_l = intrinsics.clone()
                 intrinsics_l[:, :, :2] *= scale
@@ -345,24 +386,13 @@
 
             dbg = [] if debug is not None else None
             pm: PatchMatch = getattr(self, f"patchmatch_{stage}")
-            ref_nhwc = src_nhwc = None
-            if ("nhwc", stage) in stacked:
-                allv = stacked[("nhwc", stage)]
-            elif stage in stacked:
-                allv = ops.nchw_to_nhwc(stacked[stage].contiguous())
-            else:
-                allv = None
-            if source_tables is not None:
-                ref_nhwc, src_nhwc = ref_nhwc_maps[stage], source_tables[stage]
-            elif allv is not None:
-                ref_nhwc = allv[:batch]
-                src_nhwc = allv[batch:].view(len(src_features), batch, *allv.shape[1:])
+            ref_nhwc, src_nhwc = stage_maps(stage)
             depths, score, view_weights = pm(
                 ref_feature=ref_feature[stage], src_features=[f[stage] for f in src_features], ref_proj=ref_proj,
                 src_projs=list(src_proj), depth_min=depth_min, depth_max=depth_max, depth=depth,
                 view_weights=view_weights, depth_shift=depth_shift, vw_shift=vw_shift,
                 noise=noise if stage == self.stages - 1 else None, debug=dbg, ref_nhwc=ref_nhwc, src_nhwc=src_nhwc,
-                rel_proj=None if rel_all is None else rel_all[self.stages - 1 - stage])
+                rel_proj=None if rel_all is None else rel_all[self.stages - 1 - stage], precomputed=precomputed.get(stage))
             if debug is not None:
                 debug[stage] = dbg
             depth_patchmatch[stage] = depths
diff --git a/patchmatchnet_amd/ops.py b/patchmatchnet_amd/ops.py
--- a/patchmatchnet_amd/ops.py
+++ b/patchmatchnet_amd/ops.py
@@ -1,6 +1,7 @@
 from __future__ import annotations
 
 import ctypes
+import threading
 from typing import List, Optional, Sequence, Tuple
 
 import numpy as np
@@ -111,6 +112,95 @@
 
 def _stream(t: torch.Tensor) -> int:
     return torch.cuda.current_stream(t.device).cuda_stream
+
+
+_RECORDING = threading.local()
+
+
+class PlanRegion:
+
+    def __init__(self, plan) -> None:
+        self.plan, self.open, self.branch, self.forked = plan, False, 0, False
+        self.held: List[torch.Tensor] = []
+        self.reads = {0: [], 1: []}
+        self.writes = {0: [], 1: []}
+        self.allocated = {0: [], 1: []}
+        self.held_bytes = 0
+
+
+def begin_plan_recording(plan) -> PlanRegion:
+    _RECORDING.region = PlanRegion(plan)
+    return _RECORDING.region
+
+
+def end_plan_recording() -> None:
+    _RECORDING.region = None
+
+
+def _region() -> Optional[PlanRegion]:
+    return getattr(_RECORDING, "region", None)
+
+
+def plan_fork() -> None:
+    r = _region()
+    if r is not None:
+        check(_lib.lib().pmn_plan_fork(r.plan), "pmn_plan_fork")
+        r.open, r.branch, r.forked = True, 0, True
+
+
+def plan_switch(branch: int) -> None:
+    r = _region()
+    if r is not None:
+        check(_lib.lib().pmn_plan_switch(r.plan, int(branch)), "pmn_plan_switch")
+        r.branch = int(branch)
+
+
+def plan_join() -> None:
+    r = _region()
+    if r is not None:
+        for b in (0, 1):
+            for rng in r.allocated[b]:
+                if not any(_ranges_overlap(rng, w) for w in r.writes[b]):
+                    raise PmnError("plan_join: a tensor allocated between fork and join is not among the outputs its branch's calls "
+                                   "declared (ops._note): the overlap check would not see it")
+        check_branch_overlap(r.reads[0], r.writes[0], r.reads[1], r.writes[1])
+        check(_lib.lib().pmn_plan_join(r.plan), "pmn_plan_join")
+        r.open, r.branch = False, 0
+        r.held.clear()
+
+
+def _range(t: torch.Tensor) -> Tuple[int, int]:
+    return (t.data_ptr(), t.numel() * t.element_size())
+
+
+def _ranges_overlap(a: Tuple[int, int], b: Tuple[int, int]) -> bool:
+    return a[1] > 0 and b[1] > 0 and a[0] < b[0] + b[1] and b[0] < a[0] + a[1]
+
+
+def check_branch_overlap(main_reads, main_writes, side_reads, side_writes) -> None:
+    for who, writes, others in (("main", main_writes, list(side_reads) + list(side_writes)),
+                                ("side", side_writes, list(main_reads) + list(main_writes))):
+        for w in writes:
+            for o in others:
+                if _ranges_overlap(w, o):
+                    raise PmnError(f"plan fork: the {who} branch writes [{w[0]:#x}, +{w[1]}) which the other branch touches at "
+                                   f"[{o[0]:#x}, +{o[1]}): the branches run concurrently on replay and must not share a buffer")
+
+
+def _hold(t, fresh: bool) -> None:
+    r = _region()
+    if r is not None and r.open and isinstance(t, torch.Tensor) and t.is_cuda:
+        r.held.append(t)
+        if fresh and t.numel():
+            r.allocated[r.branch].append(_range(t))
+            r.held_bytes += t.numel() * t.element_size()
+
+
+def _note(reads, writes) -> None:
+    r = _region()
+    if r is not None and r.open:
+        r.reads[r.branch] += [_range(t) for t in reads if t is not None]
+        r.writes[r.branch] += [_range(t) for t in writes if t is not None]
 
 
 def _host_f32(a: np.ndarray, n: int, name: str):
@@ -141,6 +231,7 @@
         _dev(out, "out")
         if tuple(out.shape) != (B, h, w, C):
             raise PmnError("nchw_to_nhwc: bad output shape")
+    _note((x,), (out,))
     with torch.cuda.device(x.device):
         check(_lib.lib().pmn_nchw_to_nhwc(x.data_ptr(), out.data_ptr(), B, C, h, w, _stream(x)), "pmn_nchw_to_nhwc")
     return out
@@ -206,6 +297,7 @@
     tab, tab_p = _host_i32(table, 2 * K, "table")
     _mlp_dev(mlp, "mlp")
     out = torch.empty((B, K, h, w), dtype=torch.float32, device=ref_nhwc.device)
+    _note((ref_nhwc, eval_offsets, mlp), (out,))
     with torch.cuda.device(ref_nhwc.device):
         check(_lib.lib().pmn_feature_weight(ref_nhwc.data_ptr(), eval_offsets.data_ptr(), tab_p, mlp.data_ptr(), B, C, G,
                                             K, h, w,
@@ -246,6 +338,7 @@
     D = D0 + K
     ds = torch.empty((B, D, h, w), dtype=torch.float32, device=dev)
     xn = torch.empty((B, h, w, D), dtype=torch.float32, device=dev).permute(0, 3, 1, 2)
+    _note((noise, depth if noise is None else None, depth_min, depth_max, propa_offsets), (ds, xn))
     with torch.cuda.device(dev):
         check(_lib.lib().pmn_init_hypotheses(_ptr(noise), _ptr(depth) if noise is None else None, depth_shift,
                                              depth_min.data_ptr(), depth_max.data_ptr(), num_sample,
@@ -307,6 +400,8 @@
             argmax = torch.empty((B, N, h, w), dtype=torch.int32, device=dev)
     cost = torch.empty((B, h, w, D), dtype=torch.float32, device=dev).permute(0, 3, 1, 2)
     sim = torch.empty((B, G, D, h, w), dtype=torch.float32, device=dev) if want_similarity else None
+    _note((ref_nhwc, src_nhwc if table is None else table.table, rel_proj, depth_sample, view_weights, similarity_mlp, pixelwise_mlp),
+          (cost, vw_out, argmax, sim))
     with torch.cuda.device(dev):
         if _TIMING is not None and _TIMING_ON:
             ev0, ev1 = torch.cuda.Event(enable_timing=True), torch.cuda.Event(enable_timing=True)
@@ -337,6 +432,7 @@
     tab, tab_p = _host_i32(table, 2 * K, "table")
     score = torch.empty((B, D, h, w), dtype=torch.float32, device=cost.device)
     depth = torch.empty((B, h, w), dtype=torch.float32, device=cost.device)
+    _note((cost, depth_sample, xnorm, feature_weight_, eval_offsets), (score, depth))
     with torch.cuda.device(cost.device):
         check(_lib.lib().pmn_aggregate_regress(cost.data_ptr(), depth_sample.data_ptr(), xnorm.data_ptr(),
                                                feature_weight_.data_ptr(), eval_offsets.data_ptr(), tab_p, K,
@@ -430,6 +526,7 @@
         if tuple(up.shape) != (N, Ho // 2, Wo // 2, cout) or Ho % 2 or Wo % 2:
             raise PmnError("conv2d: `up` must be [N,Ho/2,Wo/2,cout]")
         up_h, up_w = up.shape[1], up.shape[2]
+    _note((x, weights, shift, up), (out,))
     with torch.cuda.device(x.device):
         check(_lib.lib().pmn_conv2d(x.data_ptr(), weights.data_ptr(), shift.data_ptr(), _ptr(up), out.data_ptr(), N, H, W,
                                     cin, cout, K, stride, pad, dil, 1 if relu else 0, 1 if in_nchw else 0,
@@ -592,6 +689,7 @@
         raise PmnError("offset_heads_f16s: weights are not in pack_offset_heads_f16s layout for this input")
     out_a = torch.empty((N, ca, H, W), dtype=torch.float32, device=x.device)
     out_b = torch.empty((N, cout - ca, H, W), dtype=torch.float32, device=x.device) if ca < cout else None
+    _note((x, weights, shift), (out_a, out_b))
     with torch.cuda.device(x.device):
         check(_lib.lib().pmn_offset_heads_f16s(x.data_ptr(), weights.data_ptr(), shift.data_ptr(), out_a.data_ptr(), _ptr(out_b), N,
                                                H, W, cin, cout, ca, dil, _stream(x)), "pmn_offset_heads_f16s")
@@ -611,6 +709,7 @@
             raise PmnError("fpn_level: `u` must be [N,H/2,W/2,cout]")
     out_a = torch.empty((N, H, W, ca), dtype=torch.float32, device=x.device)
     out_b = torch.empty((N, H, W, cout - ca), dtype=torch.float32, device=x.device) if ca < cout else None
+    _note((x, u, w, b), (out_a, out_b))
     with torch.cuda.device(x.device):
         check(_lib.lib().pmn_fpn_level(x.data_ptr(), _ptr(u), w.data_ptr(), b.data_ptr(), out_a.data_ptr(), _ptr(out_b),
                                        N, H, W, cin, cout, ca, _stream(x)), "pmn_fpn_level")
diff --git a/patchmatchnet_amd/patchmatch.py b/patchmatchnet_amd/patchmatch.py
--- a/patchmatchnet_amd/patchmatch.py
+++ b/patchmatchnet_amd/patchmatch.py
@@ -227,19 +227,9 @@
             self._heads, self._heads_key = pk, key
         return self._heads
 
-    def forward(self, ref_feature: torch.Tensor, src_features: List[torch.Tensor], ref_proj: torch.Tensor,
-                src_projs: List[torch.Tensor], depth_min: torch.Tensor, depth_max: torch.Tensor, depth: torch.Tensor,
-                view_weights: torch.Tensor, depth_shift: int = 0, vw_shift: int = 0, noise: Optional[torch.Tensor] = None,
-                debug: Optional[list] = None, ref_nhwc: Optional[torch.Tensor] = None,
-                src_nhwc: Optional[torch.Tensor] = None, rel_proj: Optional[torch.Tensor] = None
-                ) -> Tuple[List[torch.Tensor], torch.Tensor, torch.Tensor]:
-        if len(src_features) != len(src_projs):
-            raise AssertionError("Patchmatch Evaluation: Different number of images and projection matrices")
+    def prepare(self, ref_feature: torch.Tensor, ref_nhwc: Optional[torch.Tensor] = None) -> dict:
         if not ref_feature.is_cuda:
             raise PmnError("patchmatchnet_amd.PatchMatch runs on a ROCm GPU only (no CPU fallback)")
-        device = ref_feature.device
-        batch, _, height, width = ref_feature.size()
-
         propagate_any = self.propagate_neighbors > 0 and not (self.stage == 1 and self.patchmatch_iteration == 1)
         if ref_nhwc is None:
             ref_nhwc = ops.nchw_to_nhwc(ref_feature.detach())
@@ -261,6 +251,26 @@
             ref_feature = ref_feature.contiguous()
             propa_offsets = self.propa_conv(ref_feature).contiguous() if propagate_any else None
             eval_offsets = self.eval_conv(ref_feature).contiguous()
+        feature_weight = self.feature_weight_net(ref_nhwc, eval_offsets, self._etable)
+        return dict(ref_nhwc=ref_nhwc, propa_offsets=propa_offsets, eval_offsets=eval_offsets, feature_weight=feature_weight)
+
+    def forward(self, ref_feature: torch.Tensor, src_features: List[torch.Tensor], ref_proj: torch.Tensor,
+                src_projs: List[torch.Tensor], depth_min: torch.Tensor, depth_max: torch.Tensor, depth: torch.Tensor,
+                view_weights: torch.Tensor, depth_shift: int = 0, vw_shift: int = 0, noise: Optional[torch.Tensor] = None,
+                debug: Optional[list] = None, ref_nhwc: Optional[torch.Tensor] = None,
+                src_nhwc: Optional[torch.Tensor] = None, rel_proj: Optional[torch.Tensor] = None,
+                precomputed: Optional[dict] = None) -> Tuple[List[torch.Tensor], torch.Tensor, torch.Tensor]:
+        if len(src_features) != len(src_projs):
+            raise AssertionError("Patchmatch Evaluation: Different number of images and projection matrices")
+        if not ref_feature.is_cuda:
+            raise PmnError("patchmatchnet_amd.PatchMatch runs on a ROCm GPU only (no CPU fallback)")
+        device = ref_feature.device
+        batch, _, height, width = ref_feature.size()
+
+        if precomputed is None:
+            precomputed = self.prepare(ref_feature, ref_nhwc)
+        ref_nhwc, propa_offsets = precomputed["ref_nhwc"], precomputed["propa_offsets"]
+        eval_offsets, feature_weight = precomputed["eval_offsets"], precomputed["feature_weight"]
         if rel_proj is None:
             rel_proj = ops.relative_projection(src_projs, ref_proj)
         if src_nhwc is None:
@@ -269,8 +279,6 @@
         rel_proj = rel_proj.contiguous()
         depth_min = depth_min.float().contiguous()
         depth_max = depth_max.float().contiguous()
-
-        feature_weight = self.feature_weight_net(ref_nhwc, eval_offsets, self._etable)
 
         depth_sample = depth
         cur_shift = depth_shift
```

Measured after the change: 401.9 (median of 6 runs). +4.5%, better.
